# QitaoZhao/ContextAware-PoseFormer

Hardware: AMD Instinct MI355X
Metric: frames/sec (higher is better)
Workload: dtype f32; 1 GPU; configs[1]: batch 64/GPU hrnet_32 256x256 image + 17 kpts -> 17x3, PoseFormer lifter embed 128 levels 4, fp32 tensors, fp32 accumulation; 3x3 stride-1 convs from batch 5: each operand as two fp16 pieces under exact power-of-two block scales (to 2^-23), three piece products on the 16-bit matrix pipe -- same measured distance to fp64 as the direct fp32 MFMA kernel; Inf / NaN / |x| >= 1.5e23 give NaN; frames_per_gpu=64, parallelism=dp1 (independent frames, no collective), plan_flags=0

## Files before the change

contextaware-poseformer_amd/capf/lib.py:

```python
import ctypes
import os
from ctypes import POINTER, byref, c_char_p, c_double, c_float, c_int, c_int32, c_int64, c_size_t, c_void_p

LIB_PATH = os.environ.get("CAPF_LIB") or os.path.join(os.path.dirname(os.path.abspath(__file__)), "libcapf.so")
HRNET, CPN50 = 0, 1
F32, BF16 = 0, 1
PLAN_NO_FUSED_LIFTER, PLAN_NO_WINOGRAD, PLAN_NO_ROW_HALO, PLAN_WINOGRAD_F23_ONLY, PLAN_NO_PWCHAIN, PLAN_NO_WS, PLAN_LIFTER_FP32, PLAN_NO_F32X3, PLAN_F32X3_EXACT, PLAN_NO_F32H2_GEMM, PLAN_NO_UPADD, PLAN_H2_PLANES, PLAN_NO_BNECK, PLAN_NO_BATCHED_REDUCE = 1, 2, 4, 8, 16, 32, 64, 128, 256, 512, 1024, 2048, 4096, 8192
PLAN_BF16_F32_STREAM = 32768
ABI_VERSION = 9

EXPORTS = [
    "capf_create", "capf_destroy", "capf_last_error", "capf_version", "capf_num_params", "capf_param_info",
    "capf_set_param", "capf_params_changed", "capf_lifter_params_changed", "capf_workspace_bytes", "capf_set_workspace", "capf_forward",
    "capf_backbone_forward", "capf_lifter_forward", "capf_set_debug", "capf_set_lanes", "capf_op_conv_group", "capf_affine_from_center_scale", "capf_warp_affine", "capf_op_schedule", "capf_forward_profile_launches", "capf_forward_profile_variants", "capf_tensor", "capf_forward_stats",
    "capf_num_ops", "capf_op_info", "capf_forward_profile", "capf_op_pack_conv", "capf_op_conv", "capf_op_linear",
    "capf_preprocess", "capf_fliptest_fuse", "capf_op_pack_conv_bf16", "capf_op_conv_bf16", "capf_op_conv_bf16_rh_width", "capf_op_pack_conv_bf16_rh", "capf_op_conv_bf16_rh", "capf_op_conv_bf16_group", "capf_forward_train", "capf_backward", "capf_grad_elems", "capf_grad_info", "capf_train_h2_matrices", "capf_mpjpe", "capf_adamw_step",
    "capf_pose_errors", "capf_segment_sums", "capf_keypoints_loss", "capf_train_generation", "capf_max_batch", "capf_op_bytes", "capf_op_linear_bf16", "capf_op_pack_conv_wino", "capf_op_conv_wino", "capf_op_conv_wino_group",
    "capf_op_bilinear_corners", "capf_mpjpe_nd", "capf_op_executed_flops",
    "capf_forward_prefix", "capf_op_describe", "capf_op_tensor",
    "capf_op_conv_bf16_ws_pack_elems", "capf_op_pack_conv_bf16_ws", "capf_op_conv_bf16_ws_group",
    "capf_op_conv_f32x3_pack_elems", "capf_op_pack_conv_f32x3", "capf_op_conv_f32x3_group",
    "capf_op_conv_f32h2_pack_elems", "capf_op_pack_conv_f32h2", "capf_op_conv_f32h2_group",
    "capf_abi_version", "capf_op_describe_sized",
    "capf_jpeg_info", "capf_jpeg_coefficients", "capf_jpeg_decode",
    "capf_jpeg_batch_info", "capf_jpeg_decode_batch", "capf_jpeg_coefficients_subseq",
    "capf_op_f32h2_gemm_pack_elems", "capf_op_pack_f32h2_gemm", "capf_op_conv_f32h2g", "capf_op_conv_f32h2g_group", "capf_op_linear_f32h2g", "capf_op_linear_ln_f32h2g", "capf_op_wgrad", "capf_op_conv_f32h2_tiles", "capf_op_conv_f32h2_planes", "capf_op_h2_planes",
    "capf_fliptest_fuse_swap", "capf_pck_counts",
]


class CapfError(RuntimeError):
    pass


class CapfConfig(ctypes.Structure):
    _fields_ = [
        ("backbone", c_int32), ("hr_channels", c_int32 * 4), ("hr_modules", c_int32 * 3), ("hr_blocks", c_int32),
        ("base_dim", c_int32), ("embed_dim_ratio", c_int32), ("levels", c_int32), ("num_joints", c_int32),
        ("num_heads", c_int32), ("deform_heads", c_int32), ("deform_samples", c_int32), ("context_blocks", c_int32),
        ("compute_dtype", c_int32), ("max_batch", c_int32), ("height", c_int32), ("width", c_int32),
        ("training", c_int32), ("plan_flags", c_int32), ("depth", c_int32),
    ]


class OpDesc(ctypes.Structure):
    _fields_ = [(k, c_int32) for k in ("kind", "backbone", "conv", "Cin", "H", "W", "Cout", "Ho", "Wo", "ks", "stride", "pad", "act",
                                       "in_dtype", "out_dtype", "mfma_bf16", "n_in")] + [("shift", c_int32 * 4)] + \
               [(k, c_int32) for k in ("relu", "p_weight", "p_bn_weight", "has_residual", "checkpoint", "rows_per_frame", "p_bias",
                                       "p_ln_weight", "p_ln_bias")] + [("eps", c_float), ("attn", c_int32 * 4), ("maps", (c_int64 * 4) * 3),
                                                                         ("up_H", c_int32), ("up_W", c_int32)]


class ConvDesc(ctypes.Structure):
    _fields_ = [("x", ctypes.c_void_p), ("w_packed", ctypes.c_void_p), ("bias", ctypes.c_void_p),
                ("residual", ctypes.c_void_p), ("y", ctypes.c_void_p)] + \
               [(k, ctypes.c_int32) for k in ("B", "H", "W", "Cin", "Cout", "ks", "stride", "act")]


_lib = None


def load_library():
    global _lib
    if _lib is not None:
        return _lib
    import torch
    if not os.path.exists(LIB_PATH):
        raise CapfError(f"{LIB_PATH} is missing: build it with `python __graft_entry__.py` "
                        "(or make -C contextaware-poseformer_amd/csrc); there is no fallback path")
    lib = ctypes.CDLL(LIB_PATH)
    abi = lib.capf_abi_version() if hasattr(lib, "capf_abi_version") else None
    if abi != ABI_VERSION:
        raise CapfError(f"{LIB_PATH} implements ABI revision {abi}, this binding expects {ABI_VERSION}: rebuild the library")
    H = c_void_p
    lib.capf_create.argtypes = [POINTER(CapfConfig), c_int, POINTER(H)]
    lib.capf_create.restype = c_int
    lib.capf_destroy.argtypes = [H]
    lib.capf_destroy.restype = None
    lib.capf_last_error.argtypes = [H]
    lib.capf_last_error.restype = c_char_p
    lib.capf_version.restype = c_char_p
    lib.capf_num_params.argtypes = [H]
    lib.capf_param_info.argtypes = [H, c_int, POINTER(c_char_p), POINTER(c_int64), POINTER(c_int), POINTER(c_int)]
    lib.capf_set_param.argtypes = [H, c_char_p, c_void_p, POINTER(c_int64), c_int]
    lib.capf_params_changed.argtypes = [H, c_void_p]
    lib.capf_lifter_params_changed.argtypes = [H, c_void_p]
    lib.capf_workspace_bytes.argtypes = [H, c_int]
    lib.capf_workspace_bytes.restype = c_size_t
    lib.capf_set_workspace.argtypes = [H, c_void_p, c_size_t]
    lib.capf_forward.argtypes = [H, c_void_p, c_void_p, c_void_p, c_void_p, c_int, c_void_p]
    lib.capf_backbone_forward.argtypes = [H, c_void_p, c_void_p, c_int]
    lib.capf_lifter_forward.argtypes = [H, c_void_p, c_void_p, c_void_p, c_int, c_void_p]
    lib.capf_set_debug.argtypes = [H, c_int]
    lib.capf_set_lanes.argtypes = [H, c_int]
    lib.capf_tensor.argtypes = [H, c_char_p, POINTER(c_void_p), POINTER(c_int64), POINTER(c_int)]
    lib.capf_forward_stats.argtypes = [H, c_int, POINTER(c_int64), POINTER(c_double)]
    lib.capf_forward_profile_variants.argtypes = [H, POINTER(c_int32), c_int]
    lib.capf_num_ops.argtypes = [H]
    lib.capf_op_info.argtypes = [H, c_int, c_int, POINTER(c_char_p), POINTER(c_char_p), POINTER(c_double)]
    lib.capf_op_bytes.argtypes = [H, c_int, c_int, POINTER(c_double)]
    lib.capf_op_executed_flops.argtypes = [H, c_int, c_int, POINTER(c_double)]
    lib.capf_forward_prefix.argtypes = [H, c_void_p, c_void_p, c_void_p, c_void_p, c_int, c_void_p, c_int]
    lib.capf_op_describe.argtypes = [H, c_int, POINTER(OpDesc)]
    lib.capf_op_describe_sized.argtypes = [H, c_int, c_void_p, c_size_t]
    lib.capf_op_tensor.argtypes = [H, c_int, c_int, POINTER(c_void_p)]
    lib.capf_forward_profile.argtypes = [H, c_void_p, c_void_p, c_void_p, c_void_p, c_int, c_void_p,
                                         POINTER(c_float), c_int]
    lib.capf_forward_profile_launches.argtypes = [H, c_void_p, c_void_p, c_void_p, c_void_p, c_int, c_void_p,
                                                  POINTER(c_float), POINTER(c_int32), c_int]
    P = c_void_p
    lib.capf_forward_train.argtypes = [H, P, P, P, P, c_int, P, P]
    lib.capf_backward.argtypes = [H, P, P, c_int, P, P]
    lib.capf_train_generation.argtypes = [H]
    lib.capf_train_generation.restype = c_int64
    lib.capf_max_batch.argtypes = [H]
    lib.capf_grad_elems.argtypes = [H]
    lib.capf_grad_elems.restype = c_int64
    lib.capf_grad_info.argtypes = [H, c_int, POINTER(c_int64)]
    lib.capf_train_h2_matrices.argtypes = [H]
    lib.capf_train_h2_matrices.restype = c_int
    lib.capf_mpjpe.argtypes = [P, P, P, c_int, P, P, c_float]
    lib.capf_mpjpe_nd.argtypes = [P, P, P, c_int, c_int, P, P, c_float]
    lib.capf_adamw_step.argtypes = [P, P, P, P, P, c_int64] + [c_float] * 5 + [c_int, c_float]
    lib.capf_op_bilinear_corners.argtypes = [P, P, c_int, c_int, c_int, c_int, P, P]
    lib.capf_op_pack_conv.argtypes = [P, P, P, P, P, P, c_float, P, P, c_int, c_int, c_int]
    lib.capf_op_conv.argtypes = [P, P, P, P, P, P] + [c_int] * 8
    lib.capf_op_linear.argtypes = [P, P, P, P, P, P] + [c_int] * 4
    lib.capf_preprocess.argtypes = [P, P, c_int, c_int, c_int, POINTER(c_float), POINTER(c_float), c_int, P, P, P, P, P, P, P]
    lib.capf_fliptest_fuse.argtypes = [P, P, c_int, P]
    lib.capf_op_pack_conv_bf16.argtypes = [P, P, P, P, P, P, c_float, P, P, c_int, c_int, c_int]
    lib.capf_op_conv_bf16.argtypes = [P, P, P, P, P, P] + [c_int] * 8
    lib.capf_op_conv_bf16_rh_width.argtypes = [c_int]
    lib.capf_op_pack_conv_bf16_rh.argtypes = [P, P, P, P, P, P, c_float, P, P, c_int, c_int]
    lib.capf_op_conv_bf16_rh.argtypes = [P, P, P, P, P, P] + [c_int] * 6
    lib.capf_op_conv_bf16_ws_pack_elems.argtypes = [c_int, c_int]
    lib.capf_op_conv_bf16_ws_pack_elems.restype = c_int64
    lib.capf_op_pack_conv_bf16_ws.argtypes = [P, P, P, P, P, P, c_float, P, P, c_int, c_int]
    lib.capf_op_conv_f32x3_pack_elems.argtypes = [c_int, c_int]
    lib.capf_op_conv_f32x3_pack_elems.restype = c_int64
    lib.capf_op_pack_conv_f32x3.argtypes = [P, P, P, P, P, P, c_float, P, P, c_int, c_int]
    lib.capf_op_conv_f32h2_pack_elems.argtypes = [c_int, c_int]
    lib.capf_op_conv_f32h2_pack_elems.restype = c_int64
    lib.capf_op_pack_conv_f32h2.argtypes = [P, P, P, P, P, P, c_float, P, P, c_int, c_int]
    lib.capf_op_f32h2_gemm_pack_elems.argtypes = [c_int, c_int]
    lib.capf_op_f32h2_gemm_pack_elems.restype = c_int64
    lib.capf_op_pack_f32h2_gemm.argtypes = [P, P, P, P, P, P, c_float, P, P, c_int, c_int, c_int, c_int]
    lib.capf_op_conv_f32h2g.argtypes = [P, P, P, P, P, P] + [c_int] * 8
    lib.capf_op_linear_f32h2g.argtypes = [P, P, P, P, P, P] + [c_int] * 4
    lib.capf_op_linear_ln_f32h2g.argtypes = [P, P, P, P, c_float, P, P, P, P] + [c_int] * 4
    lib.capf_op_wgrad.argtypes = [P, P, P, c_int, c_int, c_int, P, c_int]
    lib.capf_op_pack_conv_wino.argtypes = [P, P, P, P, P, P, c_float, P, P, c_int, c_int, c_int]
    lib.capf_op_conv_wino.argtypes = [P, P, P, P, P, P] + [c_int] * 7
    lib.capf_op_linear_bf16.argtypes = [P, P, P, P, P, P] + [c_int] * 4
    D = POINTER(ConvDesc)
    for name in ("capf_op_conv_group", "capf_op_conv_bf16_ws_group", "capf_op_conv_f32x3_group", "capf_op_conv_f32h2_group",
                 "capf_op_conv_f32h2g_group"):
        getattr(lib, name).argtypes = [P, c_int, D]
    lib.capf_op_conv_wino_group.argtypes = [P, c_int, D, c_int]
    lib.capf_op_conv_bf16_group.argtypes = [P, c_int, D, POINTER(c_void_p), POINTER(c_int32)]
    lib.capf_op_conv_f32h2_planes.argtypes = [P, D, P, P]
    lib.capf_op_conv_f32h2_tiles.argtypes = [c_int, c_int, c_int, POINTER(c_int)]
    lib.capf_pose_errors.argtypes = [P, P, P, c_int, c_int, P, P]
    lib.capf_segment_sums.argtypes = [P, P, P, P, c_int, c_int, P, P]
    lib.capf_keypoints_loss.argtypes = [P, c_int, P, P, P, c_int, c_int, c_float, P, P]
    lib.capf_fliptest_fuse_swap.argtypes = [P, P, c_int, c_int, POINTER(c_int32), P]
    lib.capf_pck_counts.argtypes = [P, P, P, c_int, c_int, c_int, c_double, P, c_int, P, P, P]
    _lib = lib
    return lib


PARAM_KINDS = {0: "conv_w", 1: "bn_w", 2: "bn_b", 3: "bn_mean", 4: "bn_var", 5: "bn_nbt", 6: "lin_w", 7: "lin_b",
               8: "ln_w", 9: "ln_b", 10: "raw"}


class Engine:

    def __init__(self, cfg: CapfConfig, device=None):
        self.lib = load_library()
        self.cfg = cfg
        self.h = c_void_p()
        rc = self.lib.capf_create(byref(cfg), -1 if device is None else int(device), byref(self.h))
        if rc != 0:
            raise CapfError(f"capf_create failed ({rc}): {self.lib.capf_last_error(None).decode()}")
        self.device = device
        self._ws = None
        self._ws_batch = 0
        self._bound = {}

    def close(self):
        if getattr(self, "h", None):
            self.lib.capf_destroy(self.h)
            self.h = None

    __del__ = close

    def _check(self, rc, what):
        if rc < 0:
            raise CapfError(f"{what} failed ({rc}): {self.lib.capf_last_error(self.h).decode()}")
        return rc

    def schema(self):
        out = []
        name, shape, nd, kind = c_char_p(), (c_int64 * 4)(), c_int(), c_int()
        for i in range(self.lib.capf_num_params(self.h)):
            self._check(self.lib.capf_param_info(self.h, i, byref(name), shape, byref(nd), byref(kind)), "param_info")
            out.append((name.value.decode(), tuple(shape[j] for j in range(nd.value)), PARAM_KINDS[kind.value]))
        return out

    def bind_state(self, named_tensors, stream=0):
        import torch
        for name, shape, kind in self.schema():
            if kind == "bn_nbt":
                continue
            t = named_tensors[name]
            if t.dtype != torch.float32 or not t.is_cuda or not t.is_contiguous():
                raise CapfError(f"{name}: need a contiguous fp32 CUDA tensor, got {t.dtype} {t.device}")
            if self._bound.get(name) == t.data_ptr():
                continue
            shp = (c_int64 * 4)(*(list(t.shape) + [0] * (4 - t.dim())))
            self._check(self.lib.capf_set_param(self.h, name.encode(), c_void_p(t.data_ptr()), shp, t.dim()),
                        f"set_param({name})")
            self._bound[name] = t.data_ptr()
        self.params_changed(stream)

    def params_changed(self, stream=0):
        self._check(self.lib.capf_params_changed(self.h, c_void_p(stream)), "params_changed")

    def lifter_params_changed(self, stream=0):
        self._check(self.lib.capf_lifter_params_changed(self.h, c_void_p(stream)), "lifter_params_changed")

    def workspace_bytes(self, batch):
        return self.lib.capf_workspace_bytes(self.h, batch)

    def ensure_workspace(self, batch):
        import torch
        if self._ws is None or batch > self._ws_batch:
            nbytes = self.workspace_bytes(batch)
            self._ws = torch.empty(nbytes // 4 + 64, dtype=torch.float32, device=f"cuda:{self.device}")
            self._ws_batch = batch
            self._check(self.lib.capf_set_workspace(self.h, c_void_p(self._ws.data_ptr()), nbytes), "set_workspace")

    def forward(self, images, k2d, kcrop, out, stream):
        B = images.shape[0]
        self.ensure_workspace(B)
# ... 43 lines not shown
        self.ensure_workspace(B)
        self._check(self.lib.capf_backbone_forward(self.h, c_void_p(stream), c_void_p(images.data_ptr()), B),
                    "backbone_forward")

    def lifter_forward(self, k2d, kcrop, out, stream):
        B = k2d.shape[0]
        self.ensure_workspace(B)
        self._check(self.lib.capf_lifter_forward(self.h, c_void_p(stream), c_void_p(k2d.data_ptr()),
                                                 c_void_p(kcrop.data_ptr()), B, c_void_p(out.data_ptr())),
                    "lifter_forward")

    def set_lanes(self, on):
        self._check(self.lib.capf_set_lanes(self.h, int(on)), "set_lanes")

    def set_debug(self, on):
        self._check(self.lib.capf_set_debug(self.h, int(on)), "set_debug")

    def tensor(self, name):
        import torch
        ptr, shape, nd = c_void_p(), (c_int64 * 4)(), c_int()
        rc = self._check(self.lib.capf_tensor(self.h, name.encode(), byref(ptr), shape, byref(nd)), f"tensor({name})")
        shp = [shape[i] for i in range(nd.value)]
        n = 1
        for s in shp:
            n *= s
        off = (ptr.value - self._ws.data_ptr()) // 4
        if rc == 2:
            return self._ws[off:off + (n + 1) // 2].view(torch.bfloat16)[:n].view(*shp).clone()
        flat = self._ws[off:off + n]
        if rc == 1:
            flat = flat.view(torch.int32)
        return flat.view(*shp).clone()

    def op_table(self, batch):
        name, kern, fl = c_char_p(), c_char_p(), c_double()
        out = []
        for i in range(self.lib.capf_num_ops(self.h)):
            self._check(self.lib.capf_op_info(self.h, i, batch, byref(name), byref(kern), byref(fl)), "op_info")
            out.append((name.value.decode(), kern.value.decode(), fl.value))
        return out

    def op_bytes(self, batch):
        b, out = c_double(), []
        for i in range(self.lib.capf_num_ops(self.h)):
            self._check(self.lib.capf_op_bytes(self.h, i, batch, byref(b)), "op_bytes")
            out.append(b.value)
        return out

    def op_executed_flops(self, batch):
        f, out = c_double(), []
        for i in range(self.lib.capf_num_ops(self.h)):
            self._check(self.lib.capf_op_executed_flops(self.h, i, batch, byref(f)), "op_executed_flops")
            out.append(f.value)
        return out

    def forward_prefix(self, images, n_ops, stream, k2d=None, kcrop=None, out=None):
        B = images.shape[0]
        self.ensure_workspace(B)
        self._prefix_images = images
        P = lambda t: c_void_p(t.data_ptr()) if t is not None else c_void_p(0)
        self._check(self.lib.capf_forward_prefix(self.h, c_void_p(stream), P(images), P(k2d), P(kcrop), B, P(out), int(n_ops)),
                    "forward_prefix")

    def op_describe(self, index):
        d = OpDesc()
        self._check(self.lib.capf_op_describe_sized(self.h, index, byref(d), ctypes.sizeof(d)), "op_describe")
        return d

    def op_tensor(self, index, slot, shape, dtype_code):
        import torch
        ptr = c_void_p()
        self._check(self.lib.capf_op_tensor(self.h, index, slot, byref(ptr)), f"op_tensor({index}, {slot})")
        n = 1
        for v in shape:
            n *= v
        img = getattr(self, "_prefix_images", None)
        if img is not None and ptr.value == img.data_ptr():
            return img.view(*shape)
        off = (ptr.value - self._ws.data_ptr()) // 4
        if dtype_code == 2:
            return self._ws[off:off + (n + 1) // 2].view(torch.bfloat16)[:n].view(*shape)
        return self._ws[off:off + n].view(*shape)

    def op_h2_planes(self, index, batch):
        import torch
        ptr, tp = c_void_p(), c_int(0)
        self.lib.capf_op_h2_planes.argtypes = [c_void_p, c_int, c_int, POINTER(c_void_p), POINTER(c_int)]
        role = self.lib.capf_op_h2_planes(self.h, index, batch, byref(ptr), byref(tp))
        if role <= 0:
            return 0, None, 0
        d = self.op_describe(index)
        C = d.Cout if role == 1 else d.Cin
        tiles = self.lib.capf_op_conv_f32h2_tiles(batch, d.H, d.W, None)
        off = (ptr.value - self._ws.data_ptr()) // 4
        return role, self._ws[off:off + tiles * (C // 16)].view(torch.int32).view(tiles, C // 16), tp.value

    def op_tensor_fp32(self, index, slot, shape, dtype_code):
        t = self.op_tensor(index, slot, shape, dtype_code)
        role, exps, tp = self.op_h2_planes(index, shape[0])
        if (role == 1 and slot == 5) or (role == 2 and slot == 0):
            return planes_to_fp32(t, exps, tp)
        return t

    def forward_profile(self, images, k2d, kcrop, out, stream):
        B = images.shape[0]
        self.ensure_workspace(B)
        n = self.lib.capf_num_ops(self.h)
        ms = (c_float * n)()
        self._check(self.lib.capf_forward_profile(self.h, c_void_p(stream), c_void_p(images.data_ptr()),
                                                  c_void_p(k2d.data_ptr()), c_void_p(kcrop.data_ptr()), B,
                                                  c_void_p(out.data_ptr()), ms, n), "forward_profile")
        return list(ms)

    def op_schedule(self):
        self.lib.capf_op_schedule.argtypes = [c_void_p, c_int, POINTER(c_int32), POINTER(c_int32), POINTER(c_int32),
                                              POINTER(c_int32), POINTER(c_int32)]
        out = []
        for i in range(self.lib.capf_num_ops(self.h)):
            rg, lv, ln = c_int32(), c_int32(), c_int32()
            rd, wr = (c_int32 * 5)(), (c_int32 * 6)()
            self._check(self.lib.capf_op_schedule(self.h, i, byref(rg), byref(lv), byref(ln), rd, wr), "op_schedule")
            out.append((rg.value, lv.value, ln.value, [v for v in rd if v != -1], [v for v in wr if v != -1]))
        return out

    def forward_profile_launches(self, images, k2d, kcrop, out, stream):
        B = images.shape[0]
        self.ensure_workspace(B)
        n = self.lib.capf_num_ops(self.h)
        ms = (c_float * n)()
        leader = (c_int32 * n)()
        self._check(self.lib.capf_forward_profile_launches(self.h, c_void_p(stream), c_void_p(images.data_ptr()),
                                                           c_void_p(k2d.data_ptr()), c_void_p(kcrop.data_ptr()), B,
                                                           c_void_p(out.data_ptr()), ms, leader, n), "forward_profile_launches")
        return list(ms), list(leader)

    def profile_variants(self):
        n = self.lib.capf_num_ops(self.h)
        v = (c_int32 * n)()
        self._check(self.lib.capf_forward_profile_variants(self.h, v, n), "forward_profile_variants")
        return list(v)

    def stats(self, batch):
        n, f = c_int64(), c_double()
        self._check(self.lib.capf_forward_stats(self.h, batch, byref(n), byref(f)), "forward_stats")
        return n.value, f.value


def _p(t):
    return c_void_p(t.data_ptr()) if t is not None else c_void_p(0)


def _stream(t):
    import torch
    return c_void_p(torch.cuda.current_stream(t.device).cuda_stream)


def _call(entry, *args):
    rc = getattr(load_library(), entry)(*args)
    if rc:
        raise CapfError(f"{entry} failed ({rc})")


def _out_hw(H, W, ks, stride):
    pad = ks // 2
    return (H + 2 * pad - ks) // stride + 1, (W + 2 * pad - ks) // stride + 1

# ... 57 lines not shown
    descs, outs = _conv_descs([(x, wp, bias, res, wp.shape[0], 3, 1, act) for x, wp, bias, act, res in problems])
    x0, wp0 = problems[0][:2]
    _call("capf_op_conv_wino_group", _stream(x0), len(problems), descs, _wino_variant(wp0, x0.shape[3]))
    return outs


def conv_nhwc_group(problems):
    descs, outs = _conv_descs([(x, wp, bias, res, wp.shape[0], ks, stride, act) for x, wp, bias, ks, stride, act, res in problems])
    _call("capf_op_conv_group", _stream(problems[0][0]), len(problems), descs)
    return outs


def pack_conv_bf16(w, bn=None, eps=1e-5):
    import torch
    co, ci, ks, _ = w.shape
    return _pack("capf_op_pack_conv_bf16", w, bn, eps, (co, (ks * ks * ci + 63) // 64 * 64), torch.bfloat16, co, ci, ks)


def conv_nhwc_bf16(x, wp, bias, ks, stride=1, act=0, residual=None):
    d = ConvDesc()
    y = _conv_out(d, x, wp, bias, residual, wp.shape[0], ks, stride, act, bf16=True)
    _call("capf_op_conv_bf16", _stream(x), d.x, d.w_packed, d.bias, d.residual, d.y, d.B, d.H, d.W, d.Cin, d.Cout, ks, stride, act)
    return y


def pack_conv_bf16_rh(w, bn=None, eps=1e-5):
    import torch
    co, ci, ks, _ = w.shape
    cw = load_library().capf_op_conv_bf16_rh_width(ci)
    if ks != 3 or not cw:
        raise CapfError(f"row-halo conv needs a 3x3 kernel and Cin % 32 == 0 (got ks={ks}, Cin={ci})")
    return _pack("capf_op_pack_conv_bf16_rh", w, bn, eps, (co, 9 * ci), torch.bfloat16, co, ci) + (cw,)


def conv_nhwc_bf16_rh(x, wp, bias, act=0, residual=None):
    d = ConvDesc()
    y = _conv_out(d, x, wp, bias, residual, wp.shape[0], act=act, bf16=True)
    _call("capf_op_conv_bf16_rh", _stream(x), d.x, d.w_packed, d.bias, d.residual, d.y, d.B, d.H, d.W, d.Cin, d.Cout, act)
    return y


def pack_conv_bf16_ws(w, bn=None, eps=1e-5):
    import torch
    co, ci, ks, _ = w.shape
    n = load_library().capf_op_conv_bf16_ws_pack_elems(co, ci)
    if ks != 3 or n <= 0 or co % 8:
        raise CapfError(f"2-D halo conv needs a 3x3 kernel, Cin % 16 == 0 and Cout % 8 == 0 (got ks={ks}, Cin={ci}, Cout={co})")
    return _pack("capf_op_pack_conv_bf16_ws", w, bn, eps, n, torch.bfloat16, co, ci)


def conv_nhwc_bf16_ws_group(problems):
    descs, outs = _conv_descs([(x, wp, bias, res, co, 3, 1, act) for x, wp, bias, act, res, co in problems], bf16=True)
    _call("capf_op_conv_bf16_ws_group", _stream(problems[0][0]), len(problems), descs)
    return outs


def pack_conv_f32x3(w, bn=None, eps=1e-5):
    import torch
    co, ci, ks, _ = w.shape
    n = load_library().capf_op_conv_f32x3_pack_elems(co, ci)
    if ks != 3 or n <= 0 or co % 4:
        raise CapfError(f"split-fp32 conv needs a 3x3 kernel, Cin % 16 == 0 and Cout % 4 == 0 (got ks={ks}, Cin={ci}, Cout={co})")
    return _pack("capf_op_pack_conv_f32x3", w, bn, eps, n, torch.bfloat16, co, ci)


def conv_nhwc_f32x3_group(problems):
    descs, outs = _conv_descs([(x, wp, bias, res, co, 3, 1, act) for x, wp, bias, act, res, co in problems])
    _call("capf_op_conv_f32x3_group", _stream(problems[0][0]), len(problems), descs)
    return outs


def pack_conv_f32h2(w, bn=None, eps=1e-5):
    import torch
    co, ci, ks, _ = w.shape
    n = load_library().capf_op_conv_f32h2_pack_elems(co, ci)
    if ks != 3 or n <= 0 or co % 4:
        raise CapfError(f"split-fp32 conv needs a 3x3 kernel, Cin % 16 == 0 and Cout % 4 == 0 (got ks={ks}, Cin={ci}, Cout={co})")
    return _pack("capf_op_pack_conv_f32h2", w, bn, eps, n, torch.int16, co, ci)


def conv_nhwc_f32h2_group(problems):
    descs, outs = _conv_descs([(x, wp, bias, res, co, 3, 1, act) for x, wp, bias, act, res, co in problems])
    _call("capf_op_conv_f32h2_group", _stream(problems[0][0]), len(problems), descs)
    return outs


def conv_nhwc_f32h2_planes(x, wp, bias, act, residual, cout, exps_in=None, planes_out=False):
    import torch
    d = ConvDesc()
    y = _conv_out(d, x, wp, bias, residual, cout, act=act)
    tiles = load_library().capf_op_conv_f32h2_tiles(d.B, d.H, d.W, None)
    eo = torch.zeros(tiles, cout // 16, device=x.device, dtype=torch.int32) if planes_out else None
    _call("capf_op_conv_f32h2_planes", _stream(x), byref(d), _p(exps_in), _p(eo))
    return (y, eo) if planes_out else y


def f32h2_tile_pixels(B, H, W):
    px = c_int(0)
    if load_library().capf_op_conv_f32h2_tiles(B, H, W, byref(px)) <= 0:
        raise CapfError("geometry not eligible for the two-fp16-piece tile")
    return px.value


def planes_to_fp32(planes, exps, tile_pixels):
    import torch
    B, H, W, C = planes.shape
    h = planes.contiguous().view(torch.float16).view(B * H * W, C // 16, 2, 16).float()
    tile = torch.arange(B * H * W, device=planes.device) // tile_pixels
    scale = torch.exp2((127 - exps[tile].to(torch.float64))).to(torch.float32)
    v = (h[:, :, 0, :] + h[:, :, 1, :]) * scale[:, :, None]
    return v.reshape(B, H, W, C)


def pack_f32h2_gemm(w, bn=None, eps=1e-5):
    import torch
    if w.dim() == 4:
        n, ci, ks, _ = w.shape
        k = ks * ks * ci
    else:
        (n, k), ci, ks = w.shape, 0, 0
    elems = load_library().capf_op_f32h2_gemm_pack_elems(n, k)
    return _pack("capf_op_pack_f32h2_gemm", w, bn, eps, elems, torch.float32, n, ci, ks, k, bias="zeros" if w.dim() == 4 else None)


def conv_nhwc_f32h2g(x, wp, bias, ks, stride=1, act=0, residual=None, cout=None):
    d = ConvDesc()
    y = _conv_out(d, x, wp, bias, residual, cout if cout is not None else bias.numel(), ks, stride, act)
    _call("capf_op_conv_f32h2g", _stream(x), d.x, d.w_packed, d.bias, d.residual, d.y, d.B, d.H, d.W, d.Cin, d.Cout, ks, stride, act)
    return y


def conv_nhwc_f32h2g_group(problems):
    descs, outs = _conv_descs([(x, wp, bias, res, co, ks, stride, act) for x, wp, bias, ks, stride, act, res, co in problems])
    _call("capf_op_conv_f32h2g_group", _stream(problems[0][0]), len(problems), descs)
    return outs


def _rows_out(x, n, dtype=None):
    import torch
    return torch.empty(x.shape[0], n, device=x.device, dtype=dtype or torch.float32)


def linear_ln_f32h2g(x, gamma, beta, eps, wp, bias, n, act=0, residual=None):
    (M, K), y = x.shape, _rows_out(x, n)
    _call("capf_op_linear_ln_f32h2g", _stream(x), _p(x), _p(gamma), _p(beta), float(eps), _p(wp), _p(bias), _p(residual), _p(y), M, n, K, act)
    return y


def linear_f32h2g(x, wp, bias, n, act=0, residual=None):
    (M, K), y = x.shape, _rows_out(x, n)
    _call("capf_op_linear_f32h2g", _stream(x), _p(x), _p(wp), _p(bias), _p(residual), _p(y), M, n, K, act)
    return y


def wgrad(dy, x, two_piece=True):
    import torch
    (M, N), K = dy.shape, x.shape[1]
    out = torch.empty(N * K + N, device=x.device, dtype=torch.float32)
    _call("capf_op_wgrad", _stream(x), _p(dy), _p(x), M, N, K, _p(out), 1 if two_piece else 0)
    return out[:N * K].view(N, K), out[N * K:]


def conv_nhwc_bf16_group(problems):
    descs, outs = _conv_descs([(x, wp, bias, res, wp.shape[0], ks, stride, act) for x, wp, bias, ks, stride, act, res, _ in problems], bf16=True)
    rh = (c_void_p * len(problems))(*(p[7].data_ptr() if p[7] is not None else None for p in problems))
    variant = c_int32(-1)
# ... 290 lines not shown
```

contextaware-poseformer_amd/csrc/engine.cpp:

```cpp
#include <stdio.h>
#include <string.h>

#include <algorithm>
#include <vector>

#include "engine.h"

namespace capf {

#define HIP_TRY(expr)                                                                      \
    do {                                                                                   \
        hipError_t _e = (expr);                                                            \
        if (_e != hipSuccess) {                                                            \
            err = std::string(#expr) + ": " + hipGetErrorString(_e);                       \
            return CAPF_ERR_HIP;                                                           \
        }                                                                                  \
    } while (0)

Engine::ConvSrc Engine::conv_src(const Pack& pk) const {
    return {params[pk.w[0]].ptr, params[pk.bn.g].ptr, params[pk.bn.b].ptr, params[pk.bn.m].ptr, params[pk.bn.v].ptr, 1e-5f};
}

int Engine::repack(hipStream_t s, bool lifter_only) {
    for (const Param& p : params) {
// ... 20 lines not shown
        float* B = pack_arena + pk.b_off;
        if (pk.kind == CONV_BN) {
            if (lifter_only) continue;
            const ConvSrc c = conv_src(pk);
            if (pk.bf16) {
                HIP_TRY(launch_pack_conv_bf16(c.w, c.g, c.b, c.m, c.v, c.eps, W, B, pk.N, pk.Cin, pk.ks, pk.Kpad, s));
                if (pk.rh) HIP_TRY(launch_pack_conv_bf16_rh(c.w, c.g, c.b, c.m, c.v, c.eps, pack_arena + pk.rh_off, B, pk.N, pk.Cin, bf16_rh_width(pk.Cin), s));
                if (pk.ws) HIP_TRY(launch_pack_conv_bf16_ws(c.w, c.g, c.b, c.m, c.v, c.eps, pack_arena + pk.ws_off, B, pk.N, pk.Cin, s));
            } else if (pk.wino) {
                if (!pk.wino_skip) HIP_TRY(launch_pack_conv_wino(c.w, c.g, c.b, c.m, c.v, c.eps, W, B, pk.N, pk.Cin, s, pk.Kpad == 18 * pk.Cin ? 43 : 23));
                HIP_TRY(launch_pack_conv(c.w, c.g, c.b, c.m, c.v, c.eps, pack_arena + pk.direct_off, B, pk.N, pk.Cin, pk.ks, pk.direct_Kpad, s));
                if (pk.x3)
                    HIP_TRY((plan.x3_h2 ? launch_pack_conv_f32h2 : launch_pack_conv_f32x3)(c.w, c.g, c.b, c.m, c.v, c.eps, pack_arena + pk.x3_off, B, pk.N, pk.Cin, s));
            } else {
                HIP_TRY(launch_pack_conv(c.w, c.g, c.b, c.m, c.v, c.eps, W, B, pk.N, pk.Cin, pk.ks, pk.Kpad, s));
            }
            continue;
        }
        int n0 = 0;
        for (int i = 0; i < pk.n_lin; ++i) {
            const int n = (int)params[pk.w[i]].shape[0];
            const float* w = params[pk.w[i]].ptr;
            if (pk.bf16)
                HIP_TRY(launch_pack_conv_bf16(w, nullptr, nullptr, nullptr, nullptr, 0.f, reinterpret_cast<unsigned short*>(W) + (size_t)n0 * pk.Kpad,
                                              nullptr, n, pk.K, 1, pk.Kpad, s));
            else if (pk.quad) HIP_TRY(launch_pack_linear_quad(w, W, n, pk.K, n0, pk.N, s));
            else HIP_TRY(launch_pack_linear(w, W + (size_t)n0 * pk.Kpad, n, pk.K, pk.Kpad, s));
            jobs.push_back(CopySegment{params[pk.b[i]].ptr, B + n0, n, 0});
            n0 += n;
        }
    }
    if (!jobs.empty()) {
        CopySegment* tab_dev = reinterpret_cast<CopySegment*>(pack_arena + bias_tab_off);
        const bool same = bias_tab_on_device && bias_tab.size() == jobs.size() &&
                          memcmp(bias_tab.data(), jobs.data(), jobs.size() * sizeof(CopySegment)) == 0;
        if (!same) {
            HIP_TRY(hipStreamSynchronize(s));
            bias_tab = jobs;
            HIP_TRY(hipMemcpyAsync(tab_dev, bias_tab.data(), bias_tab.size() * sizeof(CopySegment), hipMemcpyHostToDevice, s));
            bias_tab_on_device = true;
        }
        HIP_TRY(launch_copy_segments(tab_dev, (int)jobs.size(), s));
    }
    packed = true;
    return CAPF_OK;
}

int Engine::ensure_h2g_lifter(hipStream_t s) {
    if (!h2g_lifter_dirty) return CAPF_OK;
    for (const Pack& pk : packs) {
        if (!pk.h2g || pk.kind != LINEAR) continue;
        int n0 = 0;
        for (int i = 0; i < pk.n_lin; ++i) {
            const int n = (int)params[pk.w[i]].shape[0];
            HIP_TRY(launch_pack_f32h2_gemm_rows(params[pk.w[i]].ptr, pack_arena + pk.h2g_off, n0, n, pk.N, pk.K, pk.h2g_Kpad, s));
            n0 += n;
        }
        if (pk.chain) HIP_TRY(launch_res_chain_repack(pack_arena + pk.h2g_off, pack_arena + pk.chain_off, pk.N, pk.h2g_Kpad, s));
    }
    h2g_lifter_dirty = false;
    return CAPF_OK;
}

GemmArgs Engine::gemm_args(const Op& op, int batch, bool planes) const {
    auto ptr = [&](int buf) -> float* { return (buf >= 0 && ws) ? bptr(buf, batch) : nullptr; };
    const Pack& pk = packs[op.pack];
    GemmArgs a{};
    a.A = op.in[0] == -2 ? images : ptr(op.in[0]);
    if (pk.in_place) {
        a.Wp = params[pk.w[0]].ptr;
        a.bias = params[pk.b[0]].ptr;
    } else {
        a.Wp = pack_arena + pk.w_off;
        a.bias = pack_arena + pk.b_off;
    }
    a.res = op.res_param >= 0 ? params[op.res_param].ptr : ptr(op.aux);
    a.out = ptr(op.out);
    a.M = (int)(op.rows_per_frame * batch);
    a.N = op.N; a.K = op.K; a.Kpad = pk.Kpad;
    if (pk.rh) a.Wp2 = pack_arena + pk.rh_off;
    if (pk.ws || pk.x3) a.Wp3 = pack_arena + (pk.ws ? pk.ws_off : pk.x3_off);
    a.x3_h2 = pk.x3 && plan.x3_h2;
    if (a.x3_h2 && op.h2_utab >= 0 && utab_on_device) a.h2_utab = reinterpret_cast<const unsigned*>(pack_arena + utab_off) + op.h2_utab;
    if (pk.h2g && batch >= H2G_MIN_BATCH && !op.bf16 && !op.pw_pair && !(op.wino && wino_now(op, batch))) a.Wh2 = pack_arena + pk.h2g_off;
    if (op.wino && !wino_now(op, batch)) {
        a.Wp = pack_arena + pk.direct_off;
        a.Kpad = pk.direct_Kpad;
    } else if (op.wino && pk.wino_skip) {
        a.Wp = nullptr;
    }
    a.conv = op.conv;
    a.Cin = op.Cin; a.H = op.H; a.W = op.W; a.Ho = op.Ho; a.Wo = op.Wo;
    a.ks = op.ks; a.stride = op.stride; a.pad = op.pad;
    a.amap = op.amap; a.omap = op.omap; a.rmap = op.rmap;
    a.act = op.act;
    a.out_bf16 = op.out_bf16;
    a.f32s = op.f32s;
    a.out_f32 = op.st_f32;
    a.out_sh = op.sh >= 0 ? ptr(op.sh) : nullptr;
    if (planes && op.h2_role && a.x3_h2 && a.Wp3 && wino_now(op, batch)) {
        const GemmArgs peer = gemm_args(ops[op.h2_peer], batch, false);
        GemmArgs me = a;
        me.conv = op.conv; me.Cin = op.Cin; me.H = op.H; me.W = op.W; me.Ho = op.Ho; me.Wo = op.Wo; me.ks = op.ks; me.stride = op.stride; me.pad = op.pad;
        me.omap = op.omap; me.rmap = op.rmap; me.act = op.act;
        if (peer.x3_h2 && peer.Wp3 && wino_now(ops[op.h2_peer], batch) && gemm_f32x3_wanted(me) && gemm_f32x3_wanted(peer)) {
            int* e = reinterpret_cast<int*>(ptr(op.h2_exps));
            if (op.h2_role == 1) a.h2_eout = e; else a.h2_ein = e;
        }
    }
    if (op.conv && op.up_in >= 0) {
        a.up = ptr(op.up_in);
        a.up_H = op.up_H; a.up_W = op.up_W;
        a.up_sh = op.Ho > 1 ? (float)(op.up_H - 1) / (float)(op.Ho - 1) : 0.f;
        a.up_sw = op.Wo > 1 ? (float)(op.up_W - 1) / (float)(op.Wo - 1) : 0.f;
    }
    static const bool splitk_on = [] { const char* e = diag_env("CAPF_SPLITK"); return !e || atoi(e) != 0; }();
    if ((op.conv || (op.kind == OP_GEMM && op.ln.w < 0 && op.res_param < 0)) && !op.bf16 && split_ws && lanes != 1 && splitk_on) {
        a.split_ws = on_side_chain ? split_ws_side : split_ws;
        a.split_cnt = on_side_chain ? split_cnt_side : split_cnt;
        a.split_ws_elems = SPLIT_WS_ELEMS; a.split_cnt_elems = SPLIT_CNT_ELEMS;
    }
    if (op.ln.w >= 0) {
        a.ln_g = params[op.ln.w].ptr;
        a.ln_b = params[op.ln.b].ptr;
        a.ln_eps = op.eps;
    }
    return a;
}

Engine::FusedLaunch Engine::fused_at(int i, int batch, int last_op, bool bneck_only) const {
    const int n_all = (int)ops.size();
    if (i < 0 || i >= n_all) return {};
    const Op& o = ops[i];
    if (o.kind == OP_FORK) {
        if (!plan.use_bneck || !bf16() || o.fork.lanes != 2 || o.region < 0) return {};
        const int j = regions[o.region].second;
        if (j != i + 4 || j + 1 >= last_op || j + 1 >= n_all) return {};
        int c1 = -1, c2 = -1, ds = -1;
        for (int k = i + 1; k < j; ++k) {
            const Op& g = ops[k];
            if (g.kind != OP_GEMM || !g.conv || g.bf16 != 1) return {};
            if (g.lane == 1) ds = k; else if (c1 < 0) c1 = k; else c2 = k;
        }
        const int c3 = j + 1;
        if (c1 < 0 || c2 < 0 || ds < 0 || ops[c3].kind != OP_GEMM || !ops[c3].conv || ops[c3].bf16 != 1) return {};
        if (ops[c2].in[0] != ops[c1].out || ops[ds].in[0] != ops[c1].in[0] || ops[c3].in[0] != ops[c2].out || ops[c3].aux != ops[ds].out) return {};
        if (ops[c1].rows_per_frame * batch < 65536) return {};
        if (!bneck0_bf16_ok(gemm_args(ops[c1], batch), gemm_args(ops[c2], batch), gemm_args(ops[ds], batch), gemm_args(ops[c3], batch))) return {};
        return {Fusion::BNECK0, 4, {c1, c2, ds, c3}};
    }
    if (o.kind != OP_GEMM) return {};
    if (plan.use_bneck && bf16() && i + 2 < last_op && i + 2 < n_all) {
        const Op &c2 = ops[i + 1], &c3 = ops[i + 2];
        bool ok = o.bneck_c3 == i + 2 && c2.in[0] == o.out && c3.in[0] == c2.out && c3.aux == o.in[0] && o.aux < 0 && c2.aux < 0 &&
                  o.rows_per_frame * batch >= 65536;
        for (const Op* g : {&o, &c2, &c3})
            ok = ok && g->kind == OP_GEMM && g->conv && g->bf16 == 1 && g->region == o.region && g->lane == o.lane && g->up_in < 0;
        if (ok && bneck1_bf16_ok(gemm_args(o, batch), gemm_args(c2, batch), gemm_args(c3, batch))) return {Fusion::BNECK1, 3, {i, i + 1, i + 2}};
    }
    if (bneck_only || !plan.use_pwchain || i + 1 >= last_op || i + 1 >= n_all) return {};
    const Op& b = ops[i + 1];
    if (!o.conv || b.kind != OP_GEMM || !b.conv || o.bf16 != b.bf16 || o.bf16 > 1 || b.in[0] != o.out || b.region != o.region || b.lane != o.lane) return {};
    if (o.bf16 && (fused_leader(i, batch, true).n || fused_at(i + 1, batch, last_op, true).n)) return {};
    const GemmArgs ga = gemm_args(o, batch), gb = gemm_args(b, batch);
    if (!(o.bf16 ? gemm_bf16_pwchain_ok(ga, gb) : gemm_f32_pwchain_ok(ga, gb))) return {};
    return {Fusion::PWCHAIN, 2, {i, i + 1}};
// ... 168 lines not shown
        case OP_HEAD:
            HIP_TRY(launch_head(ptr(op.in[0]), params[op.ln.w].ptr, params[op.ln.b].ptr, op.eps, params[op.head.w].ptr,
                                params[op.head.b].ptr, out, (int)(op.rows_per_frame * batch), op.C, op.head.N, s));
            break;
        default: break;
    }
    return CAPF_OK;
}

int Engine::run_region_grouped(hipStream_t s, int batch, int region, LaunchLog* log, unsigned lane_mask) {
    auto mine = [&](const Op& op) { return ((lane_mask >> op.lane) & 1u) != 0; };
    auto groupable = [&](const Op& op, const GemmArgs& a) {
        if (op.kind != OP_GEMM) return false;
        switch (gemm_family(op, batch)) {
            case Family::BF16: return gemm_bf16_groupable(a);
            case Family::WINO: return gemm_wino_ok(a);
            case Family::F32: return gemm_f32_groupable(a);
            default: return false;
        }
    };
    for (const std::vector<int>& level : region_levels[region]) {
        for (Family pass : {Family::F32, Family::BF16, Family::WINO}) {
            GemmArgs group[MAXG];
            int members[MAXG];
            int n = 0;
            auto flush = [&]() -> int {
                if (n == 0) return CAPF_OK;
                if (log) HIP_TRY(log->mark(s, members, n));
                if (pass == Family::F32) HIP_TRY(launch_gemm_f32_group(group, n, s));
                else if (pass == Family::BF16) {
                    int v = -1;
                    HIP_TRY(launch_gemm_bf16_group(group, n, s, &v));
                    if (log && !log->op_variant.empty()) log->op_variant[members[0]] = v;
                }
                else HIP_TRY(launch_gemm_wino_group(group, n, s));
                n = 0;
                return CAPF_OK;
            };
            for (int oi : level) {
                const Op& op = ops[oi];
                if (op.kind != OP_GEMM || !mine(op) || gemm_family(op, batch) != pass) continue;
                const GemmArgs a = gemm_args(op, batch);
                if (!groupable(op, a)) continue;
                group[n] = a;
                members[n++] = oi;
                if (n == MAXG) { int rc = flush(); if (rc) return rc; }
            }
            int rc = flush();
            if (rc) return rc;
        }
        {
            FuseSumArgs fg[4];
            int fm[4], nf = 0;
            for (int oi : level) {
                const Op& op = ops[oi];
                if (op.kind != OP_FUSE || skipped(op) || !mine(op)) continue;
                if (nf > 0 && (op.bf16 != ops[fm[0]].bf16 || (op.C % 8 == 0) != (ops[fm[0]].C % 8 == 0))) continue;
                if (nf == 4) break;
                fg[nf] = fuse_args(op, batch);
                fm[nf++] = oi;
            }
            if (nf < 2) nf = 0;
            if (nf) {
                if (log) HIP_TRY(log->mark(s, fm, nf));
                HIP_TRY(launch_fuse_sum_group(fg, nf, s));
            }
            for (int oi : level) {
                const Op& op = ops[oi];
                if (!mine(op)) continue;
                if (op.kind == OP_GEMM && groupable(op, gemm_args(op, batch))) continue;
                if (skipped(op)) continue;
                bool done = false;
                for (int k = 0; k < nf; ++k) done |= fm[k] == oi;
                if (done) continue;
                if (log) HIP_TRY(log->mark(s, &oi, 1));
                int rc = exec_op(op, s, batch);
                if (rc) return rc;
            }
        }
    }
    return CAPF_OK;
}

int Engine::run(hipStream_t s, int batch, int first_op, int last_op, hipEvent_t* ev, LaunchLog* log) {
    hipStream_t main_stream = s;
    if (plan.use_h2g && (batch >= H2G_MIN_BATCH || has_res_chain) && last_op > n_backbone_ops && !bf16()) {
        const int rc = ensure_h2g_lifter(s);
        if (rc) return rc;
    }
    const bool grouped = (lanes == 2 || lanes == 3) && !ev;
    const bool par = lanes == 1 && !ev && !log && side[0];
    for (int oi = first_op; oi < last_op; ++oi) {
        const Op& op = ops[oi];
        s = (par && op.lane > 0) ? side[op.lane - 1] : main_stream;
        if (ev) HIP_TRY(hipEventRecord(ev[oi], s));
        if (const FusedLaunch f = ev ? FusedLaunch{} : fused_at(oi, batch, last_op); f.n) {
            const bool tap = debug || last_op < (int)ops.size();
            GemmArgs m[4];
            for (int k = 0; k < f.n; ++k) m[k] = gemm_args(ops[f.m[k]], batch);
            if (log) HIP_TRY(log->mark(s, f.m, f.n));
            if (f.kind == Fusion::BNECK0) HIP_TRY(launch_bneck0_bf16(m[0], m[1], m[2], m[3], tap, s));
            else if (f.kind == Fusion::BNECK1) HIP_TRY(launch_bneck1_bf16(m[0], m[1], m[2], tap, s));
            else if (op.bf16) HIP_TRY(launch_gemm_bf16_pwchain(m[0], m[1], s));
            else HIP_TRY(launch_gemm_f32_pwchain(m[0], m[1], s));
            oi = f.m[f.n - 1];
            continue;
        }
        switch (op.kind) {
            case OP_FORK: {
                if (grouped && regions[op.region].second <= last_op) {
                    const bool two = lanes == 3 && !log && side[0] && op.fork.lanes >= 2 && batch >= 16 && batch <= 256;
                    if (two) {
                        HIP_TRY(hipEventRecord(events[op.fork.first_event], main_stream));
                        HIP_TRY(hipStreamWaitEvent(side[0], events[op.fork.first_event], 0));
                        on_side_chain = true;
                        int rc = run_region_grouped(side[0], batch, op.region, nullptr, 0x6u);
                        on_side_chain = false;
                        if (rc) return rc;
                        rc = run_region_grouped(main_stream, batch, op.region, nullptr, ~0x6u);
                        if (rc) return rc;
                        HIP_TRY(hipEventRecord(events[op.fork.first_event + 1], side[0]));
                        HIP_TRY(hipStreamWaitEvent(main_stream, events[op.fork.first_event + 1], 0));
                        oi = regions[op.region].second;
                        break;
                    }
                    int rc = run_region_grouped(main_stream, batch, op.region, log);
                    if (rc) return rc;
                    oi = regions[op.region].second;
                } else if (par) {
                    HIP_TRY(hipEventRecord(events[op.fork.first_event], main_stream));
                    for (int l = 1; l < op.fork.lanes; ++l) HIP_TRY(hipStreamWaitEvent(side[l - 1], events[op.fork.first_event], 0));
                }
                break;
            }
            case OP_JOIN:
                if (par) {
                    for (int l = 1; l < op.fork.lanes; ++l) {
                        HIP_TRY(hipEventRecord(events[op.fork.first_event + l], side[l - 1]));
                        HIP_TRY(hipStreamWaitEvent(main_stream, events[op.fork.first_event + l], 0));
                    }
                }
                break;
            default: {
                if (skipped(op)) break;
                if (log) HIP_TRY(log->mark(s, &oi, 1));
                int rc = exec_op(op, s, batch);
                if (rc) return rc;
            }
        }
    }
    if (ev) HIP_TRY(hipEventRecord(ev[last_op], main_stream));
    if (log) HIP_TRY(log->mark(main_stream, nullptr, 0));
    return CAPF_OK;
}

}

using capf::Engine;

static std::string g_create_error;

extern "C" {

const char* capf_version(void) { return "capf 0.9 (gfx950)"; }
int capf_abi_version(void) { return CAPF_ABI_VERSION; }

const char* capf_last_error(const capf_handle* h) { return h ? h->e.err.c_str() : g_create_error.c_str(); }

int capf_create(const capf_config* cfg, int device, capf_handle** out) {
    if (!cfg || !out) {
        g_create_error = "null argument";
        return CAPF_ERR_INVALID;
    }
    capf_handle* h = new capf_handle();
    Engine& e = h->e;
    e.cfg = *cfg;
    e.device = device;
    e.lanes = 2;
    if (cfg->compute_dtype != CAPF_F32 && cfg->compute_dtype != CAPF_BF16) {
        g_create_error = "compute_dtype must be CAPF_F32 or CAPF_BF16";
        delete h;
        return CAPF_ERR_UNSUPPORTED;
    }
    if (cfg->plan_flags & ~(16383 | CAPF_PLAN_BF16_F32_STREAM)) {
        g_create_error = "unknown capf_plan_flag bits";
        delete h;
        return CAPF_ERR_INVALID;
    }
    if (cfg->max_batch <= 0) {
        g_create_error = "max_batch must be positive";
        delete h;
        return CAPF_ERR_INVALID;
    }
    if (!e.build()) {
        g_create_error = e.err;
        delete h;
        return CAPF_ERR_UNSUPPORTED;
    }
    if (device >= 0) {
        hipError_t r = hipSetDevice(device);
        if (r == hipSuccess && e.pack_elems) r = hipMalloc(reinterpret_cast<void**>(&e.pack_arena), e.pack_elems * sizeof(float));
        if (r == hipSuccess) r = hipMalloc(reinterpret_cast<void**>(&e.split_ws), Engine::SPLIT_WS_ELEMS * sizeof(float));
        if (r == hipSuccess) r = hipMalloc(reinterpret_cast<void**>(&e.split_cnt), Engine::SPLIT_CNT_ELEMS * sizeof(int));
        if (r == hipSuccess) r = hipMemset(e.split_cnt, 0, Engine::SPLIT_CNT_ELEMS * sizeof(int));
        if (r == hipSuccess) r = hipMalloc(reinterpret_cast<void**>(&e.split_ws_side), Engine::SPLIT_WS_ELEMS * sizeof(float));
        if (r == hipSuccess) r = hipMalloc(reinterpret_cast<void**>(&e.split_cnt_side), Engine::SPLIT_CNT_ELEMS * sizeof(int));
        if (r == hipSuccess) r = hipMemset(e.split_cnt_side, 0, Engine::SPLIT_CNT_ELEMS * sizeof(int));
        for (int i = 0; i < 3 && r == hipSuccess; ++i) r = hipStreamCreateWithFlags(&e.side[i], hipStreamNonBlocking);
        e.events.resize(e.n_events);
        for (auto& x : e.events)
            if (r == hipSuccess) r = hipEventCreateWithFlags(&x, hipEventDisableTiming);
        if (r != hipSuccess) {
            g_create_error = std::string("hip: ") + hipGetErrorString(r);
            delete h;
            return CAPF_ERR_HIP;
        }
    }
    *out = h;
    return CAPF_OK;
}

void capf_destroy(capf_handle* h) {
    if (!h) return;
    if (h->e.pack_arena) (void)hipFree(h->e.pack_arena);
    if (h->e.split_ws) (void)hipFree(h->e.split_ws);
    if (h->e.split_cnt) (void)hipFree(h->e.split_cnt);
    if (h->e.split_ws_side) (void)hipFree(h->e.split_ws_side);
    if (h->e.split_cnt_side) (void)hipFree(h->e.split_cnt_side);
    for (auto& x : h->e.events)
        if (x) (void)hipEventDestroy(x);
    for (auto& st : h->e.side)
        if (st) (void)hipStreamDestroy(st);
    delete h;
}

int capf_max_batch(const capf_handle* h) { return h ? (h->e.batch_limit < h->e.cfg.max_batch ? h->e.batch_limit : h->e.cfg.max_batch) : CAPF_ERR_INVALID; }

int capf_num_params(const capf_handle* h) { return h ? (int)h->e.params.size() : CAPF_ERR_INVALID; }

int capf_param_info(const capf_handle* h, int index, const char** name, int64_t shape[4], int* ndim, int* kind) {
    if (!h || index < 0 || index >= (int)h->e.params.size()) return CAPF_ERR_INVALID;
    const capf::Param& p = h->e.params[index];
    if (name) *name = p.name.c_str();
    if (shape) memcpy(shape, p.shape, sizeof(p.shape));
    if (ndim) *ndim = p.ndim;
    if (kind) *kind = p.kind;
    return CAPF_OK;
}

int capf_set_param(capf_handle* h, const char* name, const void* dev_ptr, const int64_t* shape, int ndim) {
    if (!h || !name) return CAPF_ERR_INVALID;
    Engine& e = h->e;
    auto it = e.param_index.find(name);
    if (it == e.param_index.end()) {
        e.err = std::string("unknown parameter: ") + name;
        return CAPF_ERR_INVALID;
    }
    capf::Param& p = e.params[it->second];
    bool ok = (ndim == p.ndim);
    for (int i = 0; ok && i < ndim; ++i) ok = (shape[i] == p.shape[i]);
    if (!ok) {
        e.err = std::string("shape mismatch for ") + name;
        return CAPF_ERR_INVALID;
    }
    p.ptr = static_cast<const float*>(dev_ptr);
    e.packed = false;
    return CAPF_OK;
// ... 327 lines not shown
}

int capf_op_linear(void* stream, const float* x, const float* w, const float* bias, const float* residual, float* y,
                   int M, int N, int K, int act) {
    if (K % 32 != 0) return CAPF_ERR_UNSUPPORTED;
    return hip_rc(capf::launch_gemm_f32(rows_args(&capf::GemmArgs::Wp, x, w, bias, residual, y, M, N, K, act), static_cast<hipStream_t>(stream)));
}

int capf_op_bilinear_corners(void* stream, const float* grid, int n, int H, int W, int border, int32_t* idx, float* frac) {
    if (!grid || !idx || !frac || n <= 0 || H <= 0 || W <= 0) return CAPF_ERR_INVALID;
    return capf::launch_bilinear_corners(grid, n, H, W, border, idx, frac, static_cast<hipStream_t>(stream)) == hipSuccess
               ? CAPF_OK : CAPF_ERR_HIP;
}

int capf_op_pack_conv_bf16(void* stream, const float* w, const float* gamma, const float* beta, const float* mean,
                           const float* var, float eps, void* wp, float* bias, int Cout, int Cin, int ks) {
    const int Kpad = (ks * ks * Cin + 63) / 64 * 64;
    return hip_rc(capf::launch_pack_conv_bf16(w, gamma, beta, mean, var, eps, wp, bias, Cout, Cin, ks, Kpad, static_cast<hipStream_t>(stream)));
}

int capf_op_conv_bf16(void* stream, const void* x, const void* wp, const float* bias, const void* residual, void* y, int B,
                      int H, int W, int Cin, int Cout, int ks, int stride, int act) {
    const capf::GemmArgs a = conv_args(conv_desc(x, wp, bias, residual, y, B, H, W, Cin, Cout, ks, stride, act), &capf::GemmArgs::Wp, 64);
    return hip_rc(capf::launch_gemm_bf16(a, static_cast<hipStream_t>(stream)), CAPF_ERR_UNSUPPORTED);
}

int capf_op_conv_bf16_rh_width(int Cin) {
    return capf::gemm_bf16_rh_cw(conv_args(conv_desc(nullptr, nullptr, nullptr, nullptr, nullptr, 1, 8, 8, Cin, 8, 3, 1, 0), &capf::GemmArgs::Wp, 1));
}

int capf_op_pack_conv_bf16_rh(void* stream, const float* w, const float* gamma, const float* beta, const float* mean,
                              const float* var, float eps, void* wp, float* bias, int Cout, int Cin) {
    const int cw = capf_op_conv_bf16_rh_width(Cin);
    if (!cw) return CAPF_ERR_UNSUPPORTED;
    return hip_rc(capf::launch_pack_conv_bf16_rh(w, gamma, beta, mean, var, eps, wp, bias, Cout, Cin, cw, static_cast<hipStream_t>(stream)));
}

int capf_op_conv_bf16_rh(void* stream, const void* x, const void* wp, const float* bias, const void* residual, void* y, int B,
                         int H, int W, int Cin, int Cout, int act) {
    const capf::GemmArgs a = conv_args(conv_desc(x, wp, bias, residual, y, B, H, W, Cin, Cout, 3, 1, act), &capf::GemmArgs::Wp, 1);
    return hip_rc(capf::launch_gemm_bf16_rh(a, static_cast<hipStream_t>(stream)), CAPF_ERR_UNSUPPORTED);
}

int64_t capf_op_conv_bf16_ws_pack_elems(int Cout, int Cin) { return Cin % 16 == 0 && Cout > 0 ? capf::bf16_ws_pack_elems(Cout, Cin) : 0; }

int capf_op_pack_conv_bf16_ws(void* stream, const float* w, const float* gamma, const float* beta, const float* mean,
                              const float* var, float eps, void* wp, float* bias, int Cout, int Cin) {
    if (!w || !wp || Cin % 16 != 0 || Cout % 8 != 0) return CAPF_ERR_UNSUPPORTED;
    return hip_rc(capf::launch_pack_conv_bf16_ws(w, gamma, beta, mean, var, eps, wp, bias, Cout, Cin, static_cast<hipStream_t>(stream)));
}

int capf_op_conv_bf16_ws_group(void* stream, int n, const capf_conv_desc* d) {
    return conv_group(stream, n, d, [](const capf_conv_desc& c, int, capf::GemmArgs& a) { return wp3_build(c, a, capf::gemm_bf16_ws_ok, 0); },
                      capf::launch_gemm_bf16_ws_group);
}

int64_t capf_op_conv_f32x3_pack_elems(int Cout, int Cin) { return Cin % 16 == 0 && Cout > 0 ? capf::f32x3_pack_elems(Cout, Cin) : 0; }

int capf_op_pack_conv_f32x3(void* stream, const float* w, const float* gamma, const float* beta, const float* mean, const float* var,
                            float eps, void* wp, float* bias, int Cout, int Cin) {
    if (!w || !wp || Cin % 16 != 0 || Cout % 4 != 0) return CAPF_ERR_UNSUPPORTED;
    return hip_rc(capf::launch_pack_conv_f32x3(w, gamma, beta, mean, var, eps, wp, bias, Cout, Cin, static_cast<hipStream_t>(stream)));
}

int capf_op_conv_f32x3_group(void* stream, int n, const capf_conv_desc* d) {
    return conv_group(stream, n, d, [](const capf_conv_desc& c, int, capf::GemmArgs& a) { return wp3_build(c, a, capf::gemm_f32x3_ok, 0); },
                      capf::launch_gemm_f32x3_group);
}

int64_t capf_op_conv_f32h2_pack_elems(int Cout, int Cin) { return Cin % 16 == 0 && Cout > 0 ? capf::f32h2_pack_elems(Cout, Cin) : 0; }

int capf_op_pack_conv_f32h2(void* stream, const float* w, const float* gamma, const float* beta, const float* mean, const float* var,
                            float eps, void* wp, float* bias, int Cout, int Cin) {
    if (!w || !wp || Cin % 16 != 0 || Cout % 4 != 0) return CAPF_ERR_UNSUPPORTED;
    return hip_rc(capf::launch_pack_conv_f32h2(w, gamma, beta, mean, var, eps, wp, bias, Cout, Cin, static_cast<hipStream_t>(stream)));
}

int capf_op_conv_f32h2_group(void* stream, int n, const capf_conv_desc* d) {
    return conv_group(stream, n, d, [](const capf_conv_desc& c, int, capf::GemmArgs& a) { return wp3_build(c, a, capf::gemm_f32x3_ok, 1); },
                      capf::launch_gemm_f32h2_group);
}

int capf_op_conv_f32h2_tiles(int B, int H, int W, int* tile_pixels) { return capf::f32h2_tiles_m(B, H, W, tile_pixels); }

int capf_op_conv_f32h2_planes(void* stream, const capf_conv_desc* d, const int32_t* exps_in, int32_t* exps_out) {
    if (!d || !is_3x3_s1(*d) || (exps_in && exps_out)) return CAPF_ERR_UNSUPPORTED;
    capf::GemmArgs g = conv_args(*d, &capf::GemmArgs::Wp3, 1);
    g.x3_h2 = 1; g.h2_ein = exps_in; g.h2_eout = exps_out;
    if (!capf::gemm_f32x3_ok(g)) return CAPF_ERR_UNSUPPORTED;
    const hipError_t e = capf::launch_gemm_f32h2_group(&g, 1, static_cast<hipStream_t>(stream));
    return hip_rc(e, e == hipErrorInvalidValue ? CAPF_ERR_UNSUPPORTED : CAPF_ERR_HIP);
}

int capf_op_conv_bf16_group(void* stream, int n, const capf_conv_desc* d, const void* const* w_rh, int32_t* variant) {
    return conv_group(stream, n, d, [w_rh](const capf_conv_desc& c, int i, capf::GemmArgs& a) {
        a = conv_args(c, &capf::GemmArgs::Wp, 64);
        a.Wp2 = w_rh ? static_cast<const float*>(w_rh[i]) : nullptr;
        return capf::gemm_bf16_groupable(a) ? CAPF_OK : CAPF_ERR_UNSUPPORTED;
    }, [variant](const capf::GemmArgs* g, int n, hipStream_t s) {
        int v = -1;
        const hipError_t e = capf::launch_gemm_bf16_group(g, n, s, &v);
        if (variant) *variant = v;
        return e;
    });
}

int capf_op_linear_bf16(void* stream, const void* x_bf16, const void* w_bf16, const float* bias, const float* residual, void* y,
                        int M, int N, int K, int gelu_bf16_out) {
    if (!x_bf16 || !w_bf16 || !y || K % 64 != 0) return CAPF_ERR_INVALID;
    return capf::launch_gemm_bf16_rows(x_bf16, w_bf16, bias, M, N, K, K, static_cast<float*>(y), capf::row_ld(N), residual,
                                       capf::row_ld(N), gelu_bf16_out, static_cast<hipStream_t>(stream)) == hipSuccess
               ? CAPF_OK : CAPF_ERR_UNSUPPORTED;
}

int capf_preprocess(void* stream, const uint8_t* images_bgr, int batch, int height, int width, const float mean[3],
                    const float* std3, int mode, float* images_out, const float* gt_in, float* gt_out, const float* k2d_in,
                    float* k2d_out, const float* kcrop_in, float* kcrop_out) {
    if (!images_bgr || !images_out || !k2d_in || !k2d_out || !kcrop_in || !kcrop_out || !mean || batch <= 0 || mode < 0 ||
        mode > 2 || (gt_in && !gt_out))
        return CAPF_ERR_INVALID;
    return capf::launch_preprocess(images_bgr, batch, height, width, mean, std3, mode, images_out, gt_in, gt_out, k2d_in,
                                   k2d_out, kcrop_in, kcrop_out, static_cast<hipStream_t>(stream)) == hipSuccess
               ? CAPF_OK : CAPF_ERR_HIP;
}

int capf_fliptest_fuse(void* stream, const float* pred2, int batch, float* out) {
    if (!pred2 || !out || batch <= 0) return CAPF_ERR_INVALID;
    return capf::launch_fliptest_fuse(pred2, batch, out, static_cast<hipStream_t>(stream)) == hipSuccess ? CAPF_OK : CAPF_ERR_HIP;
}

int capf_fliptest_fuse_swap(void* stream, const float* pred2, int batch, int joints, const int32_t* swap, float* out) {
    if (!pred2 || !out || !swap || batch <= 0 || joints <= 0 || joints > capf::FLIP_MAX_JOINTS) return CAPF_ERR_INVALID;
    for (int j = 0; j < joints; ++j)
        if (swap[j] < 0 || swap[j] >= joints || swap[swap[j]] != j) return CAPF_ERR_INVALID;
    return capf::launch_fliptest_fuse_swap(pred2, batch, joints, swap, out, static_cast<hipStream_t>(stream)) == hipSuccess ? CAPF_OK
                                                                                                                       : CAPF_ERR_HIP;
}

int capf_affine_from_center_scale(const double center[2], const double scale[2], int out_w, int out_h, double m[6]) {
    if (!center || !scale || !m || out_w <= 1 || out_h <= 1) return CAPF_ERR_INVALID;
    return capf::affine_from_center_scale(center, scale, out_w, out_h, m) ? CAPF_OK : CAPF_ERR_INVALID;
}

int capf_warp_affine(void* stream, const uint8_t* const* frames, const int32_t* dims, const double* m, int batch, int out_h,
                     int out_w, uint8_t* out) {
    if (!frames || !dims || !m || !out || batch <= 0 || out_h <= 0 || out_w <= 0) return CAPF_ERR_INVALID;
    return capf::launch_warp_affine_u8(frames, dims, m, out, batch, out_h, out_w, static_cast<hipStream_t>(stream)) == hipSuccess
               ? CAPF_OK : CAPF_ERR_HIP;
}

int capf_pose_errors(void* stream, const float* pred, const float* gt, int n, int joints, const int32_t* prev, float* err) {
    if (!pred || !gt || !err || n <= 0 || joints <= 0) return CAPF_ERR_INVALID;
    hipError_t r = capf::launch_pose_errors(pred, gt, n, joints, prev, err, static_cast<hipStream_t>(stream));
    return r == hipSuccess ? CAPF_OK : (r == hipErrorInvalidValue ? CAPF_ERR_UNSUPPORTED : CAPF_ERR_HIP);
}

int capf_segment_sums(void* stream, const float* err, const int32_t* segment, const int32_t* prev, int n, int n_segments,
                      double* sums, int32_t* counts) {
    if (!err || !sums || !counts || n <= 0 || n_segments <= 0 || (n_segments > 1 && !segment)) return CAPF_ERR_INVALID;
    return capf::launch_segment_sums(err, segment, prev, n, n_segments, sums, counts, static_cast<hipStream_t>(stream)) == hipSuccess
               ? CAPF_OK : CAPF_ERR_HIP;
}

int capf_pck_counts(void* stream, const float* pred, const float* gt, int n, int joints, int root, double to_mm, const int32_t* segment,
                    int n_segments, int32_t* counts, double* mpjpe_sums, int32_t* frames) {
    if (!counts || !mpjpe_sums || !frames || n < 0 || (n > 0 && (!pred || !gt)) || joints <= 0 || joints > 32 || root < 0 ||
// ... 171 lines not shown
    }
    const int act_dt = e.bf16() ? 2 : 0;
    d->in_dtype = d->out_dtype = (d->backbone ? act_dt : 0);
    d->H = op.H; d->W = op.W; d->Ho = op.Ho; d->Wo = op.Wo;
    if (op.kind == capf::OP_GEMM) {
        const capf::Pack& pk = e.packs[op.pack];
        d->conv = op.conv; d->Cin = op.conv ? op.Cin : op.K; d->Cout = op.N;
        d->ks = op.ks; d->stride = op.stride; d->pad = op.pad; d->act = op.act;
        d->has_residual = op.aux >= 0 || op.res_param >= 0;
        if (op.conv && op.up_in >= 0) { d->up_H = op.up_H; d->up_W = op.up_W; }
        d->mfma_bf16 = (op.bf16 || op.out_bf16) ? 1 : 0;
        if (op.conv) {
            d->in_dtype = op.in[0] == -2 ? 0 : (op.bf16 ? 2 : 0);
            d->out_dtype = op.st_f32 ? 0 : (op.bf16 || op.out_bf16) ? 2 : 0;
            d->p_weight = pk.w[0]; d->p_bn_weight = pk.bn.g;
        } else {
            d->in_dtype = op.bf16 == 2 ? 2 : 0;
            d->out_dtype = op.out_bf16 ? 2 : 0;
            d->p_weight = pk.n_lin == 1 ? pk.w[0] : -1;
            d->p_bias = pk.n_lin == 1 ? pk.b[0] : -1;
            d->p_ln_weight = op.ln.w; d->p_ln_bias = op.ln.b;
        }
    } else if (op.kind == capf::OP_LAYERNORM) {
        d->Cin = d->Cout = op.C;
        d->in_dtype = 0; d->out_dtype = op.out_bf16 ? 2 : 0;
        d->has_residual = op.aux >= 0;
        d->p_ln_weight = op.ln.w; d->p_ln_bias = op.ln.b;
        d->maps[1][0] = 1; d->maps[1][1] = op.C; d->maps[1][2] = 0; d->maps[1][3] = 0;
    } else if (op.kind == capf::OP_ATTENTION) {
        const capf::Attn& at = op.attn;
        d->attn[0] = at.groups; d->attn[1] = at.tokens; d->attn[2] = at.heads; d->attn[3] = at.head_dim;
        d->rows_per_frame = at.groups * at.tokens;
        d->Cin = 3 * at.heads * at.head_dim; d->Cout = at.heads * at.head_dim;
        d->in_dtype = 0; d->out_dtype = op.out_bf16 ? 2 : 0;
        d->maps[0][0] = 1; d->maps[0][1] = d->Cin; d->maps[1][0] = 1; d->maps[1][1] = d->Cout;
    } else {
        d->Cin = d->Cout = op.C;
        d->n_in = op.n_in; d->relu = op.relu;
        d->has_residual = op.kind == capf::OP_RESIZE && op.aux >= 0;
        for (int i = 0; i < 4; ++i) d->shift[i] = op.shift[i];
        if (op.kind == capf::OP_FUSE) { d->Ho = op.H; d->Wo = op.W; }
        if (op.kind == capf::OP_FUSE && d->backbone) d->in_dtype = d->out_dtype = op.bf16 ? 2 : 0;
    }
    d->checkpoint = (op.bneck_c3 >= 0 ? op.bneck_c3 : op.region >= 0 ? e.regions[op.region].second : index) + 1;
    return CAPF_OK;
}

int capf_op_describe_sized(const capf_handle* h, int index, void* desc, size_t desc_bytes) {
    if (!desc || desc_bytes == 0) return CAPF_ERR_INVALID;
    capf_op_desc full;
    const int rc = capf_op_describe(h, index, &full);
    if (rc != CAPF_OK) return rc;
    memset(desc, 0, desc_bytes);
    memcpy(desc, &full, desc_bytes < sizeof(full) ? desc_bytes : sizeof(full));
    return CAPF_OK;
}

int capf_op_tensor(const capf_handle* h, int index, int slot, const void** dev_ptr) {
    if (!h || !dev_ptr || index < 0 || index >= (int)h->e.ops.size() || slot < 0 || slot > 6) return CAPF_ERR_INVALID;
    const Engine& e = h->e;
    const capf::Op& op = e.ops[index];
    const auto r = op.reads();
    const int buf = slot == 1 && r[5] >= 0 ? r[5] : slot < 5 ? r[slot] : slot == 5 ? op.out : op.sh;
    if (buf == -2) { *dev_ptr = e.images; return CAPF_OK; }
    if (buf < 0 || !e.ws || e.last_batch <= 0) return CAPF_ERR_INVALID;
    *dev_ptr = e.bptr(buf, e.last_batch);
    return CAPF_OK;
}

int capf_op_h2_planes(const capf_handle* h, int index, int batch, const void** exps, int32_t* tile_pixels) {
    if (!h || index < 0 || index >= (int)h->e.ops.size() || batch <= 0) return CAPF_ERR_INVALID;
    const Engine& e = h->e;
    const capf::Op& op = e.ops[index];
    if (!op.h2_role || !e.ws) return 0;
    const capf::GemmArgs a = e.gemm_args(op, batch);
    if (!a.h2_ein && !a.h2_eout) return 0;
    if (exps) *exps = a.h2_ein ? static_cast<const void*>(a.h2_ein) : static_cast<const void*>(a.h2_eout);
    int tp = 0;
    capf::f32h2_tiles_m(batch, op.H, op.W, &tp);
    if (tile_pixels) *tile_pixels = tp;
    return op.h2_role;
}

int capf_forward_profile(capf_handle* h, void* stream, const float* images_nhwc, const float* k2d, float* kcrop_inout,
                         int batch, float* out, float* op_ms, int n_ops) {
    if (!h || !images_nhwc || !k2d || !kcrop_inout || !out || !op_ms) return CAPF_ERR_INVALID;
    Engine& e = h->e;
    const int n = (int)e.ops.size();
    if (n_ops < n) return CAPF_ERR_INVALID;
    int rc = check_run(e, batch);
    if (rc) return rc;
    e.images = images_nhwc; e.k2d = k2d; e.kcrop = kcrop_inout; e.out = out;
    e.last_batch = batch;
    e.invalidate_train();
    std::vector<hipEvent_t> ev(n + 1);
    for (auto& x : ev)
        if (hipEventCreate(&x) != hipSuccess) return CAPF_ERR_HIP;
    hipStream_t s = static_cast<hipStream_t>(stream);
    rc = e.run(s, batch, 0, n, ev.data());
    if (rc == CAPF_OK && hipStreamSynchronize(s) != hipSuccess) rc = CAPF_ERR_HIP;
    for (int i = 0; i < n && rc == CAPF_OK; ++i)
        if (hipEventElapsedTime(&op_ms[i], ev[i], ev[i + 1]) != hipSuccess) rc = CAPF_ERR_HIP;
    for (auto& x : ev) (void)hipEventDestroy(x);
    return rc;
}

int capf_forward_profile_launches(capf_handle* h, void* stream, const float* images_nhwc, const float* k2d,
                                  float* kcrop_inout, int batch, float* out, float* op_ms, int32_t* op_leader, int n_ops) {
    if (!h || !images_nhwc || !k2d || !kcrop_inout || !out || !op_ms || !op_leader) return CAPF_ERR_INVALID;
    Engine& e = h->e;
    const int n = (int)e.ops.size();
    if (n_ops < n) return CAPF_ERR_INVALID;
    int rc = check_run(e, batch);
    if (rc) return rc;
    e.images = images_nhwc; e.k2d = k2d; e.kcrop = kcrop_inout; e.out = out;
    e.last_batch = batch;
    e.invalidate_train();
    capf::LaunchLog log;
    log.op_leader.assign(n, -1);
    log.op_variant.assign(n, -1);
    hipStream_t s = static_cast<hipStream_t>(stream);
    rc = e.run(s, batch, 0, n, nullptr, &log);
    e.last_variants = log.op_variant;
    if (rc == CAPF_OK && hipStreamSynchronize(s) != hipSuccess) rc = CAPF_ERR_HIP;
    for (int i = 0; i < n; ++i) { op_ms[i] = 0.f; op_leader[i] = log.op_leader[i]; }
    for (size_t k = 0; k < log.leader.size() && rc == CAPF_OK; ++k)
        if (hipEventElapsedTime(&op_ms[log.leader[k]], log.ev[k], log.ev[k + 1]) != hipSuccess) rc = CAPF_ERR_HIP;
    return rc;
}

int capf_forward_profile_variants(const capf_handle* h, int32_t* op_variant, int n_ops) {
    if (!h || !op_variant || n_ops < (int)h->e.last_variants.size()) return CAPF_ERR_INVALID;
    for (size_t i = 0; i < h->e.last_variants.size(); ++i) op_variant[i] = h->e.last_variants[i];
    return CAPF_OK;
}

int capf_forward_stats(const capf_handle* h, int batch, int64_t* launches, double* flops) {
    if (!h) return CAPF_ERR_INVALID;
    int64_t n = 0;
    double f = 0.0;
    for (const capf::Op& op : h->e.ops) {
        if (op.debug_only) continue;
        if (op.kind == capf::OP_FORK || op.kind == capf::OP_JOIN) continue;
        ++n;
        f += op.flops_per_frame * batch;
    }
    if (launches) *launches = n;
    if (flops) *flops = f;
    return CAPF_OK;
}

}
```

contextaware-poseformer_amd/csrc/engine.h:

```cpp
#pragma once
#include <hip/hip_runtime.h>
#include <stdint.h>

#include <array>
#include <map>
#include <string>
#include <vector>

#include "capf.h"
#include "kernels.h"

namespace capf {

struct Param {
    std::string name;
    int64_t shape[4] = {0, 0, 0, 0};
    int ndim = 0;
    int kind = 0;
    const float* ptr = nullptr;
    int64_t numel() const {
        int64_t n = 1;
        for (int i = 0; i < ndim; ++i) n *= shape[i];
        return n;
    }
};

struct Buffer {
    size_t elems = 0;
    size_t offset = 0;
    int def_op = -1;
    int last_op = -1;
    std::string tag;
};

struct Tensor {
    int buf = -1;
    int H = 0, W = 0, C = 0;
};

struct BnRef { int g = -1, b = -1, m = -1, v = -1; };

enum PackKind { CONV_BN = 0, LINEAR = 1 };
struct Pack {
    PackKind kind = CONV_BN;
    int w[4] = {-1, -1, -1, -1}, b[4] = {-1, -1, -1, -1};
    int n_lin = 0;
    BnRef bn;
    int N = 0, K = 0, Cin = 0, ks = 1;
    size_t w_off = 0, b_off = 0;
    int Kpad = 0;
    bool in_place = false;
    bool bf16 = false;
    bool quad = false;
    bool wino = false;
    bool wino_skip = false;
    size_t direct_off = 0; int direct_Kpad = 0;
    bool rh = false; size_t rh_off = 0; int rh_Kpad = 0;
    bool ws = false; size_t ws_off = 0;
    bool x3 = false; size_t x3_off = 0;
    bool h2g = false; size_t h2g_off = 0; int h2g_Kpad = 0;
    bool chain = false; size_t chain_off = 0;
};

struct LinearRef { int w = -1, b = -1, N = 0, K = 0; };
struct LnRef { int w = -1, b = -1; };
struct LifterMlp { LnRef norm2; LinearRef fc1, fc2; };
struct LifterAtt { LnRef norm1; LinearRef qkv, proj; LifterMlp mlp; };
struct LifterCtx {
    LnRef norm1;
    LinearRef aw, so, embed_proj[4];
    LifterMlp mlp;
    int ao_pack = -1;
    int tap_pos = -1, tap_idx = -1;
};
struct LifterSchema {
    int pos = -1;
    LinearRef coord, feat_embed[4];
    LifterAtt res[8], joint[8];
    LifterCtx ctx[4];
    LnRef head_ln;
    LinearRef head;
};

// ... 38 lines not shown
    int lvlH[4] = {0, 0, 0, 0}, lvlW[4] = {0, 0, 0, 0}, lvlC[4] = {0, 0, 0, 0};
    int idx_lvl[4] = {-1, -1, -1, -1};
    int tap_pos = -1, tap_idx = -1;
    int pq[4] = {-1, -1, -1, -1};
    int pb[4] = {-1, -1, -1, -1};
    double flops_per_frame = 0.0;
    int bf16 = 0;
    int wino = 0;
    int pw_pair = 0;
    int x3_lo = 0, x3_hi = -1;
    int out_bf16 = 0;
    int h2_exps = -1, h2_role = 0, h2_peer = -1;
    long h2_utab = -1;
    int f32s = 0, st_f32 = 0, sh = -1;
    int feat_bf16 = 0;
    int bneck_c3 = -1;
    int lane = 0;
    int region = -1;
};

struct NamedTensor {
    int buf;
    int64_t shape[4];
    int ndim;
    int is_int;
};

struct TrainLayout {
    struct Mlp { size_t xh2, rs2, y2, hp, hg; };
    struct Ctx { size_t xh1, rs1, y1, ao, U[4]; Mlp mlp; };
    struct Att { size_t xh1, rs1, y1, qkv, o; Mlp mlp; };
    size_t X, S[4];
    Ctx ctx[4];
    Att res[8], joint[8];
    size_t xhh, rsh, yh;
    size_t dX, gA, gB, gC, cat, dU[4], tA, tB, wT, slabs, red;
    size_t h2w, h2max;
    size_t wpad;
    size_t slabs_elems = 0, red_elems = 0;
    size_t red_cap = 0;
    size_t slab_cap = 0;
    size_t total;
};

struct LaunchLog {
    std::vector<hipEvent_t> ev;
    std::vector<int> leader;
    std::vector<int> op_leader;
    std::vector<int> op_variant;
    hipError_t mark(hipStream_t s, const int* members, int n) {
        hipEvent_t e;
        hipError_t r = hipEventCreate(&e);
        if (r != hipSuccess) return r;
        ev.push_back(e);
        if (n > 0) {
            leader.push_back(members[0]);
            for (int i = 0; i < n; ++i) op_leader[members[i]] = members[0];
        }
        return hipEventRecord(e, s);
    }
    ~LaunchLog() {
        for (hipEvent_t e : ev) (void)hipEventDestroy(e);
    }
};

struct Engine {
    capf_config cfg{};
    int device = -1;
    std::string err;

    struct PlanSwitches {
        bool fused_lifter = true;
        bool use_wino = true;
        bool wino_f43 = true;
        bool wino_f43_cpn = false;
        int wino_f43_min_hw = 0, wino_f43_max_hw = 1 << 30;
        int wino_min_batch = 24;
        bool use_rh = true;
        bool use_ws = true;
        bool use_x3 = true;
        bool x3_h2 = true;
        bool use_h2g = true;
        bool use_h2_planes = false;
        bool use_pwchain = true;
        bool use_bneck = true;
        bool use_upadd = true;
        bool batch_reduce = true;
        bool f32_stream = false;
    } plan;
    bool set_plan_switches();
    static constexpr int H2G_MIN_BATCH = 5;

    std::vector<Param> params;
    std::map<std::string, int> param_index;
    std::vector<Buffer> bufs;
    std::vector<Pack> packs;
    std::vector<Op> ops;
    int n_backbone_ops = 0;
    int cur_lane = 0, cur_region = -1, n_regions = 0, n_events = 0;
    std::vector<std::pair<int, int>> regions;
    std::vector<std::vector<std::vector<int>>> region_levels;
    std::map<std::string, NamedTensor> named;
    size_t ws_elems_per_frame = 0;
    size_t pack_elems = 0;
    size_t bias_tab_off = 0;
    bool has_res_chain = false;
    std::vector<unsigned> utab_host;
    size_t utab_off = 0;
    int batch_limit = 0;
    int feat_buf[4] = {-1, -1, -1, -1}, feat_H[4] = {0, 0, 0, 0}, feat_W[4] = {0, 0, 0, 0}, feat_C[4] = {0, 0, 0, 0};
    LifterSchema lifter;
    std::vector<long> grad_off;
    long grad_elems = 0;

    int add_param(const std::string& name, int kind, std::initializer_list<int64_t> shape);
    int new_buffer(size_t elems, const std::string& tag);
    Tensor conv_bn(const std::string& conv, const std::string& bn, const Tensor& x, int Cout, int ks, int stride,
                   int act, const Tensor* residual);
    void build_hrnet(Tensor img, Tensor feats[4]);
    void build_cpn(Tensor img, Tensor feats[4]);
    void build_lifter(const Tensor feats[4]);
    bool build();
    void assign_offsets();
    void schedule_regions();
    bool bf16() const { return cfg.compute_dtype == CAPF_BF16; }
    bool maps_bf16() const { return bf16() && !plan.f32_stream; }
    int depth() const { return cfg.depth > 0 ? cfg.depth : cfg.levels; }
    bool plan_f32_stream(const Tensor feats[4]);
    size_t act_elems(size_t n) const { return bf16() ? (n + 1) / 2 : n; }
    void use(int buf);
    void push(Op op);
    void fork(int n);
    void set_lane(int l) { cur_lane = l; }
    void join();

    float* pack_arena = nullptr;
    std::vector<CopySegment> bias_tab;
    bool bias_tab_on_device = false;
    bool utab_on_device = false;
    float* split_ws = nullptr;
    int* split_cnt = nullptr;
    float* split_ws_side = nullptr;
    int* split_cnt_side = nullptr;
    bool on_side_chain = false;
    static constexpr long SPLIT_WS_ELEMS = 4L << 20;
    static constexpr int SPLIT_CNT_ELEMS = 16384;
    float* ws = nullptr;
    size_t ws_bytes = 0;
    bool packed = false;
    bool h2g_lifter_dirty = true;
    bool debug = false;
    int lanes = 3;
    hipStream_t side[3] = {nullptr, nullptr, nullptr};
    std::vector<hipEvent_t> events;
    std::vector<int> last_variants;
    int last_batch = 0;
    const float* images = nullptr;
    const float* k2d = nullptr;
    float* kcrop = nullptr;
    float* out = nullptr;

    float* bptr(int buf, int batch) const { return ws + bufs[buf].offset * (size_t)batch; }
    struct ConvSrc { const float *w, *g, *b, *m, *v; float eps; };
    ConvSrc conv_src(const Pack& pk) const;
    int repack(hipStream_t s, bool lifter_only = false);
    int ensure_h2g_lifter(hipStream_t s);
    int run(hipStream_t s, int batch, int first_op, int last_op, hipEvent_t* ev = nullptr, LaunchLog* log = nullptr);
    int exec_op(const Op& op, hipStream_t s, int batch);
    bool skipped(const Op& op) const { return op.debug_only && !debug; }
    FuseSumArgs fuse_args(const Op& op, int batch) const;
    bool wino_now(const Op& op, int batch) const {
        return op.wino && ((batch >= op.x3_lo && batch <= op.x3_hi) || (batch >= plan.wino_min_batch && !packs[op.pack].wino_skip));
    }
    enum class Family { NONE = -1, F32, BF16, WINO, BF16_ROWS };
    struct OpRoute { Family family; const char* kernel; double flops; };
    Family gemm_family(const Op& op, int batch) const;
    OpRoute op_route(const Op& op, int batch) const;
    enum class Fusion { NONE, BNECK0, BNECK1, PWCHAIN };
    struct FusedLaunch { Fusion kind = Fusion::NONE; int n = 0; int m[4] = {-1, -1, -1, -1}; };
    FusedLaunch fused_at(int i, int batch, int last_op, bool bneck_only = false) const;
    FusedLaunch fused_leader(int i, int batch, bool bneck_only = false) const;
    int run_region_grouped(hipStream_t s, int batch, int region, LaunchLog* log, unsigned lane_mask = ~0u);
    GemmArgs gemm_args(const Op& op, int batch, bool planes = true) const;

    int train_batch = 0;
    int64_t train_generation = 0;
    void invalidate_train() { train_batch = 0; ++train_generation; t_h2_base = nullptr; }
    void train_layout(int B, TrainLayout& L) const;
    size_t train_elems(int B) const;
    int forward_train(hipStream_t s, int B, const float* masks);
    int backward(hipStream_t s, int B, const float* dOut, float* flat_grad, const float* masks);
    int t_gemm(hipStream_t s, const float* A, RowMap amap, int M, int N, int K, const float* W, int Kpad, const float* bias,
               float* out, RowMap omap, const float* res, RowMap rmap, int act, const float* rscale, int rs_div, const float* Wh2 = nullptr);
    struct H2TrainSpec { int param, pack; int N, K, ld; bool fwd, bwd; };
    std::vector<H2TrainSpec> t_h2_specs;
    std::vector<H2TrainW> t_h2_tab;
    std::map<const float*, int> t_h2_index;
    size_t t_h2_tab_off = 0;
    size_t t_h2_elems = 0, t_h2_max_elems = 0;
    int t_h2_tiles = 0;
    bool t_h2_on_device = false;
    SlabBatch t_slab_jobs{};
    size_t t_slab_cur = 0;
    float* t_slab_take(hipStream_t s, float* area, size_t cap, size_t elems, int* rc);
    int t_slab_defer(hipStream_t s, const float* slabs, int nslab, long n, float* dst);
    int t_slab_flush(hipStream_t s);
    ColFinalBatch t_col_jobs{};
    size_t t_col_cur = 0;
    int t_colreduce(hipStream_t s, const TrainLayout& L, float* tw, const float* A, RowMap amap, const float* Bm, RowMap bmap, int bmode,
                    int rows, int C, float* dst, long dst_stride, float* dst2, size_t cap_elems);
    int t_col_flush(hipStream_t s);
    float* t_h2_base = nullptr;
    void t_h2_plan();
    int t_h2_prepare(hipStream_t s, const TrainLayout& L, float* tw, int B);
    const float* t_h2_pack(const float* W, bool transposed) const;
    int t_linear_bwd(hipStream_t s, const TrainLayout& L, float* tw, const float* dY, RowMap dymap, int rows, int N, int K,
                     const float* Xin, RowMap xmap, const float* W, float* dX, RowMap dxmap, bool acc_dx, float* gW, float* gb);
};

}

struct capf_handle {
// ... 3 lines not shown
```

contextaware-poseformer_amd/csrc/igemm_f32h2_ws.hip:

```cpp
#include "igemm_f32h2_ws_tile.h"
#include "kernels.h"

namespace capf {

long f32h2_pack_elems(int Cout, int Cin) { return h2_pack_elems(Cout, Cin); }

static bool h2_from_args(const GemmArgs& a, H2Problem* q) {
    if (a.out_bf16 || !ws_args_ok(a, 3, 4.0, WS_MAX_P)) return false;
    if (!h2_plan(a.M / (a.H * a.W), a.H, a.W, a.Cin, a.N, 32, q)) return false;
    static const long wide_min = [] { const char* e = diag_env("CAPF_H2_WIDE_MIN_TILES"); return e ? atol(e) : 512L; }();
    if (a.N % 64 == 0 && (long)q->g.tiles_m * (a.N / 64) >= wide_min) { q->g.NS = 64; q->g.NSL = a.N / 64; }
    q->x = a.A;
    q->g.wp = reinterpret_cast<const unsigned short*>(a.Wp3);
    q->winv = reinterpret_cast<const float*>(q->g.wp + h2_piece_elems(a.N, a.Cin));
    q->g.bias = a.bias;
    q->res = a.res ? a.res + a.rmap.off : nullptr;
    q->y = a.out + a.omap.off;
    q->g.ldy = (int)a.omap.S1;
    q->g.ldr = a.res ? (int)a.rmap.S1 : (int)a.omap.S1;
    q->g.relu = a.act == ACT_RELU;
    q->ein = a.h2_ein;
    q->eout = a.h2_eout;
    q->utab = a.h2_utab;
    if (a.h2_eout && (a.res || a.N % 16 != 0 || a.omap.S1 != a.N)) return false;
    if (a.h2_ein && a.Cin % 16 != 0) return false;
    return true;
}

bool gemm_f32h2_ok(const GemmArgs& a) {
    H2Problem q;
    return h2_from_args(a, &q);
}
int f32h2_tiles_m(int B, int H, int W, int* tile_pixels) {
    H2Problem q;
    if (!h2_plan(B, H, W, 16, 16, 32, &q)) return 0;
    if (tile_pixels) *tile_pixels = q.g.P;
    return q.g.tiles_m;
}
bool f32h2_unit_table(int H, int W, int Cin, unsigned* out) { return h2_unit_table(H, W, Cin, out); }
bool f32h2_shape_ok(int B, int H, int W, int Cin, int Cout) {
    H2Problem q;
    return h2_plan(B, H, W, Cin, Cout, 32, &q);
}

struct H2GroupArgs {
    H2Problem g[MAXG];
    GroupLayout lay;
    int n;
};
static_assert(sizeof(H2GroupArgs) == MAXG * sizeof(H2Problem) + (2 * MAXG + 2) * sizeof(int), "kernel argument layout");

template <int TN, bool PIN = false, bool POUT = false>
__global__ __launch_bounds__(256, TN == 1 ? 3 : 2) void igemm_f32h2_group_ws_kernel(H2GroupArgs ga) {
#if defined(__HIP_DEVICE_COMPILE__)
    extern __shared__ __attribute__((aligned(16))) unsigned char h2_lds[];
    const GroupSlot t = group_slot(ga.lay, ga.n, blockIdx.x);
    if (!t.live) return;
    igemm_f32h2_ws_tile<TN, PIN, POUT>(ga.g[t.pi], t.bid, h2_lds);
#endif
}

template <int TN, bool PIN = false, bool POUT = false>
static hipError_t h2_launch(const H2Problem* list, int n, hipStream_t s) {
    int tiles[MAXG], order[MAXG];
    double cost[MAXG];
    for (int i = 0; i < n; ++i) { tiles[i] = list[i].g.tiles_m * list[i].g.NSL; cost[i] = list[i].g.C; }
    H2GroupArgs ga{};
    ga.n = n;
    const int start = group_layout(ga.lay, n, tiles, cost, order);
    for (int i = 0; i < n; ++i) ga.g[i] = list[order[i]];
    static DynLdsAttr attr;
    const hipError_t e = attr.ensure(reinterpret_cast<const void*>(&igemm_f32h2_group_ws_kernel<TN, PIN, POUT>), h2_lds_bytes(32 * TN));
    if (e != hipSuccess) return e;
    hipLaunchKernelGGL((igemm_f32h2_group_ws_kernel<TN, PIN, POUT>), dim3(start), dim3(256), h2_lds_bytes(32 * TN), s, ga);
    return hipGetLastError();
}

hipError_t launch_gemm_f32h2_group(const GemmArgs* list, int n, hipStream_t s) {
    if (n <= 0) return hipSuccess;
    if (n > MAXG) return hipErrorInvalidValue;
    H2Problem cls[2][3][MAXG];
    int cnt[2][3] = {{0, 0, 0}, {0, 0, 0}};
    for (int i = 0; i < n; ++i) {
        H2Problem q;
        if (!list[i].Wp3 || !list[i].x3_h2 || !h2_from_args(list[i], &q)) return hipErrorInvalidValue;
        if (q.ein && q.eout) return hipErrorInvalidValue;
        const int w = q.g.NS == 64 ? 1 : 0, k = q.ein ? 1 : (q.eout ? 2 : 0);
        cls[w][k][cnt[w][k]++] = q;
    }
    hipError_t e = hipSuccess;
    if (cnt[1][0] && e == hipSuccess) e = h2_launch<2>(cls[1][0], cnt[1][0], s);
    if (cnt[1][1] && e == hipSuccess) e = h2_launch<2, true, false>(cls[1][1], cnt[1][1], s);
    if (cnt[1][2] && e == hipSuccess) e = h2_launch<2, false, true>(cls[1][2], cnt[1][2], s);
    if (cnt[0][0] && e == hipSuccess) e = h2_launch<1>(cls[0][0], cnt[0][0], s);
    if (cnt[0][1] && e == hipSuccess) e = h2_launch<1, true, false>(cls[0][1], cnt[0][1], s);
    if (cnt[0][2] && e == hipSuccess) e = h2_launch<1, false, true>(cls[0][2], cnt[0][2], s);
    return e;
}

const char* gemm_f32h2_kernel_name(const GemmArgs&) { return "igemm_f32h2_group_ws"; }

__global__ void pack_conv_f32h2_kernel(const float* __restrict__ w, const float* __restrict__ gamma, const float* __restrict__ beta,
                                       const float* __restrict__ mean, const float* __restrict__ var, float eps,
                                       unsigned short* __restrict__ Wp, const float* __restrict__ winv, float* __restrict__ bias,
                                       int Cout, int Cin, long total) {
    const int ncc = Cin / 16;
    for (long i = blockIdx.x * (long)blockDim.x + threadIdx.x; i < total; i += (long)gridDim.x * blockDim.x) {
        const WsPackIdx d = ws_pack_decode(i, 32, ncc);
        float v = bn_fold_w3x3(w, gamma, beta, mean, var, eps, bias, Cout, Cin, d.ng, d.c, d.tap, d.first);
        if (d.ng < Cout) v *= __uint_as_float(0x7F000000u - __float_as_uint(winv[d.ng]));
        const long piece = 9L * 32 * 16;
        const long base = ((long)(d.sl * ncc + d.cc) * 2) * piece + ((long)d.tap * 32 + d.n) * 16 + d.qp * 8 + d.e;
        const _Float16 p0 = (_Float16)v;
        const _Float16 p1 = (_Float16)(v - (float)p0);
        Wp[base] = __builtin_bit_cast(unsigned short, p0);
        Wp[base + piece] = __builtin_bit_cast(unsigned short, p1);
    }
}

hipError_t launch_pack_conv_f32h2(const float* w, const float* gamma, const float* beta, const float* mean, const float* var, float eps,
                                  void* Wp_f16, float* bias, int Cout, int Cin, hipStream_t s) {
    if (Cin % 16 != 0 || Cout <= 0) return hipErrorInvalidValue;
    unsigned short* Wp = static_cast<unsigned short*>(Wp_f16);
    float* winv = reinterpret_cast<float*>(Wp + h2_piece_elems(Cout, Cin));
    const int npad = ((Cout + 31) / 32) * 32;
    const hipError_t e = launch_f32h2_wscale(w, gamma, var, eps, winv, npad, Cout, Cin * 9, s);
    if (e != hipSuccess) return e;
    const long total = h2_piece_elems(Cout, Cin) / 2;
    hipLaunchKernelGGL(pack_conv_f32h2_kernel, dim3(grid_1d(total)), dim3(256), 0, s, w, gamma, beta, mean, var, eps, Wp,
                       winv, bias, Cout, Cin, total);
    return hipGetLastError();
}

}
```

contextaware-poseformer_amd/csrc/igemm_f32h2_ws_tile.h:

```cpp
#pragma once
#ifndef H2_EXPERIMENT
#define H2_EXPERIMENT 0
#endif
#include <algorithm>

#include "igemm_bf16_ws_tile.h"

namespace capf {

static constexpr int H2_HP = WS_MAX_PP * 16 + 64;
static constexpr int H2_A_BYTES = 4 * H2_HP;
static constexpr int H2_AUX_BYTES = 16 + 2 * 64 * 4 + 4 * 64 * 4 + 16;
inline constexpr int h2_w_bytes(int NS) { return 2 * 9 * NS * 32; }
inline constexpr int h2_lds_bytes(int NS) { return H2_A_BYTES + h2_w_bytes(NS) + H2_AUX_BYTES; }

struct H2Problem {
    WsProblem g;
    const float* x;
    const float* res;
    float* y;
    const float* winv;
    const int* ein;
    int* eout;
    const unsigned* utab;
};
static constexpr int H2_NAU = 7;

inline long h2_piece_elems(int N, int C) { return (long)((N + 31) / 32) * (C / 16) * 2 * 9 * 32 * 16; }
inline long h2_pack_elems(int N, int C) { return h2_piece_elems(N, C) + 2L * ((N + 31) / 32) * 32; }

inline bool h2_plan(int B, int H, int W, int C, int N, int NS, H2Problem* q) {
    if (B <= 0 || H <= 0 || W <= 0 || N % 4 != 0 || (NS != 32 && NS != 64)) return false;
    if ((double)H * W * C * 4.0 * (WS_MAX_P / (H * W) + 2) >= 2.0e9 || (double)WS_MAX_P * N * 4.0 >= 2.0e9) return false;
    if (!ws_plan(B, H, W, C, (N + 7) & ~7, &q->g, true)) return false;
    q->g.N = N;
    q->g.ldy = q->g.ldr = N;
    q->g.NS = NS;
    q->g.NSL = (N + NS - 1) / NS;
    q->utab = nullptr;
    return true;
}

inline bool h2_unit_table(int H, int W, int C, unsigned* out) {
    H2Problem q;
    if (!h2_plan(1, H, W, C, 32, 32, &q)) return false;
    const WsProblem& p = q.g;
    if (p.G != 1 && p.RGPI != 1) return false;
    const int n_units = 4 * p.PP;
    for (int j = 0; j < H2_NAU; ++j)
        for (int tid = 0; tid < 256; ++tid) {
            const int qi = std::min(j * 256 + tid, n_units - 1);
            const int px = qi >> 2, qt = qi & 3;
            const int g = px / p.SEGP, rem = px - g * p.SEGP;
            const int rr = rem / p.PW, ww = rem - rr * p.PW;
            const int col = ww - 1;
            const long off = ((((long)g * p.H + rr - 1) * p.W + col) * p.C + qt * 4) * 4;
            if (off >= (1L << 31) || off < -(1L << 31)) return false;
            out[j * 256 + tid] = ((unsigned)(int)off & ~15u) | (col >= 0 && col < p.W ? 1u : 0u) | (rr == 0 ? 2u : 0u) | (rr == p.RH + 1 ? 4u : 0u);
        }
    return true;
}

inline __host__ __device__ int h2_scale_exp(int mbits) {
    const int sb = 268 - (mbits >> 23);
    return sb < 64 ? 64 : (sb > 190 ? 190 : sb);
}

#if defined(__HIP_DEVICE_COMPILE__)

typedef _Float16 ws_f16x8 __attribute__((ext_vector_type(8)));
typedef unsigned ws_u32x2 __attribute__((ext_vector_type(2)));

__device__ __forceinline__ void h2_split2(float x, float y, float s, unsigned& p1, unsigned& p2) {
    typedef _Float16 h2_t __attribute__((ext_vector_type(2)));
    typedef float f2_t __attribute__((ext_vector_type(2)));
    const f2_t v = f2_t{x, y} * s;
    const h2_t a = __builtin_convertvector(v, h2_t);
    const f2_t r = v - __builtin_convertvector(a, f2_t);
    const h2_t b = __builtin_convertvector(r, h2_t);
    p1 = __builtin_bit_cast(unsigned, a);
    p2 = __builtin_bit_cast(unsigned, b);
}

__device__ __forceinline__ unsigned h2_pk_mul(unsigned a, unsigned b) {
    typedef _Float16 h2_t __attribute__((ext_vector_type(2)));
    const h2_t r = __builtin_bit_cast(h2_t, a) * __builtin_bit_cast(h2_t, b);
    return __builtin_bit_cast(unsigned, r);
}

__device__ __forceinline__ int h2_wave_max(float v) {
    int x = __float_as_int(v);
    x = max(x, __builtin_amdgcn_update_dpp(0, x, 0xB1, 0xF, 0xF, true));
    x = max(x, __builtin_amdgcn_update_dpp(0, x, 0x4E, 0xF, 0xF, true));
    x = max(x, __builtin_amdgcn_update_dpp(0, x, 0x141, 0xF, 0xF, true));
    x = max(x, __builtin_amdgcn_update_dpp(0, x, 0x140, 0xF, 0xF, true));
    return max(max(__builtin_amdgcn_readlane(x, 0), __builtin_amdgcn_readlane(x, 16)),
               max(__builtin_amdgcn_readlane(x, 32), __builtin_amdgcn_readlane(x, 48)));
}

template <int TN, bool PIN = false, bool POUT = false>
__device__ __forceinline__ void igemm_f32h2_ws_tile(const H2Problem& q, const int bid, unsigned char* __restrict__ lds) {
    constexpr int NS = 32 * TN;
    constexpr int WP_BYTES = 9 * 32 * 32;
    constexpr int WS_BYTES = 2 * WP_BYTES;
    constexpr int W2_BYTES = TN * WS_BYTES;
    constexpr int NWI = W2_BYTES / 1024;
    constexpr int NWS = (NWI + 3) / 4;
    constexpr int NAU = H2_NAU;
    constexpr unsigned OOB = 0x80000000u;
    const WsProblem& p = q.g;
    const int tid = threadIdx.x, lane = tid & 63;
    const int wave = __builtin_amdgcn_readfirstlane(tid >> 6);
    const int frow = lane & 31, fhalf = lane >> 5;
    const int NCC = p.C >> 4;
    const int tm = bid / p.NSL, slice = bid - tm * p.NSL;

    const int b_first = ws_div(tm * p.G, p.d_rgpi);
    const ws_rsrc_t rs_x = __builtin_amdgcn_make_buffer_rsrc((void*)(q.x + (size_t)b_first * p.H * p.W * p.C), 0, 0x7FFFFF00u, 0x00020000);
    constexpr int HP = H2_HP;
    unsigned a_voff[NAU], a_lds[NAU];
    [[maybe_unused]] unsigned a_cls = 0;
    const int n_units = 4 * p.PP;
    const bool tab_ok = !(H2_EXPERIMENT & 128) && !PIN && q.utab != nullptr && (p.G == 1 || (p.RGPI == 1 && (tm + 1) * p.G <= p.RG));
    if (tab_ok) {
        const int k = tm * p.G - b_first * p.RGPI;
        const unsigned kill = (k == 0 ? 2u : 0u) | (k == p.RGPI - 1 ? 4u : 0u);
        const int base = k * p.RH * p.W * p.C * 4;
#pragma unroll
        for (int j = 0; j < NAU; ++j) {
            const unsigned t = q.utab[j * 256 + tid];
            const int qi = min(j * 256 + tid, n_units - 1);
            const int px = qi >> 2, qt = qi & 3;
            a_lds[j] = (unsigned)((qt >> 1) * HP + px * 16 + (qt & 1) * 8);
            a_voff[j] = ((t & 1u) && !(t & kill)) ? (unsigned)((int)(t & ~15u) + base) : OOB;
        }
    } else {
        const int q0 = tm * p.G;
#pragma unroll
        for (int j = 0; j < NAU; ++j) {
            const int qi = min(j * 256 + tid, n_units - 1);
            const int px = qi >> 2, qt = qi & 3;
            a_lds[j] = PIN ? (unsigned)((2 * (qt >> 1) + (qt & 1)) * HP + px * 16)
                           : (unsigned)((qt >> 1) * HP + px * 16 + (qt & 1) * 8);
#if (H2_EXPERIMENT & 64)
            a_voff[j] = (unsigned)(qi * 16 + q0);
            continue;
#endif
            const int g = ws_div(px, p.d_segp), rem = px - g * p.SEGP;
            const int rr = ws_div(rem, p.d_pw), ww = rem - rr * p.PW;
            if (PIN) a_cls |= (rr == 0 ? 1u : (rr == p.RH + 1 ? 2u : 0u)) << (2 * j);
            const int sg = q0 + g;
            const int b = ws_div(sg, p.d_rgpi);
            const int h = (sg - b * p.RGPI) * p.RH + rr - 1, col = ww - 1;
            const bool ok = sg < p.RG && h >= 0 && h < p.H && col >= 0 && col < p.W;
            a_voff[j] = ok ? (unsigned)(((((b - b_first) * p.H + h) * p.W + col) * p.C + qt * 4) * 4) : OOB;
        }
    }
    ws_f32x4 ar[NAU];
    auto load_a = [&](int cc) {
#pragma unroll
        for (int j = 0; j < NAU; ++j)
            ar[j] = __builtin_bit_cast(ws_f32x4, __builtin_amdgcn_raw_buffer_load_b128(rs_x, a_voff[j], (unsigned)cc * 64u, 0));
    };
    int* const aux = reinterpret_cast<int*>(lds + H2_A_BYTES + W2_BYTES);
    float* const aux_w = reinterpret_cast<float*>(aux + 4);
    float* const aux_b = aux_w + 64;
    int* const aux_px = reinterpret_cast<int*>(aux_b + 64) + wave * 64;
    [[maybe_unused]] int* const aux_o = reinterpret_cast<int*>(aux_b + 64) + 4 * 64;
    [[maybe_unused]] int e_nb[3] = {190, 190, 190};
    [[maybe_unused]] const int* e_row[3] = {nullptr, nullptr, nullptr};
    if constexpr (PIN) {
        e_row[0] = q.ein + (size_t)tm * NCC;
        if (p.G == 1 && p.RH < p.H) {
            const int k = tm - ws_div(tm, p.d_rgpi) * p.RGPI;
            if (k > 0) e_row[1] = q.ein + (size_t)(tm - 1) * NCC;
            if (k + 1 < p.RGPI) e_row[2] = q.ein + (size_t)(tm + 1) * NCC;
        }
    }
    [[maybe_unused]] int e_raw[3] = {190, 190, 190};
    auto load_e = [&](int cc) {
        if constexpr (PIN) {
#pragma unroll
            for (int k = 0; k < 3; ++k) e_raw[k] = e_row[k] ? e_row[k][cc] : 190;
        }
    };
    auto use_e = [&]() {
        if constexpr (PIN) {
#pragma unroll
            for (int k = 0; k < 3; ++k) e_nb[k] = __builtin_amdgcn_readfirstlane(e_raw[k]);
        }
    };
    [[maybe_unused]] unsigned has_cls[3] = {0, 0, 0};
    if constexpr (PIN) {
#pragma unroll
        for (int j = 0; j < NAU; ++j) {
            const unsigned c = (a_cls >> (2 * j)) & 3;
#pragma unroll
            for (int k = 0; k < 3; ++k) has_cls[k] |= (__builtin_amdgcn_ballot_w64(c == (unsigned)k) != 0 ? 1u : 0u) << j;
        }
    }
    auto store_planes = [&](int sn) {
        const unsigned moved = (e_nb[0] != sn ? has_cls[0] : 0u) | ((e_nb[1] != sn && e_nb[1] != 190) ? has_cls[1] : 0u) |
                               ((e_nb[2] != sn && e_nb[2] != 190) ? has_cls[2] : 0u);
#pragma unroll
        for (int j = 0; j < NAU; ++j) {
            const ws_u32x4 src = __builtin_bit_cast(ws_u32x4, ar[j]);
            unsigned w0 = src[0], w1 = src[1], w2 = src[2], w3 = src[3];
            if ((moved >> j) & 1) {
                const int cls = (a_cls >> (2 * j)) & 3;
                const int en = cls == 0 ? e_nb[0] : (cls == 1 ? e_nb[1] : e_nb[2]);
                const int r = en == 190 ? 0 : sn - en;
                const int r1 = r >= -14 ? r : -14, r2 = r - r1;
                const unsigned hb = (unsigned)(15 + r1) << 10, mb = hb | (hb << 16);
                w0 = h2_pk_mul(w0, mb); w1 = h2_pk_mul(w1, mb); w2 = h2_pk_mul(w2, mb); w3 = h2_pk_mul(w3, mb);
                if (__builtin_amdgcn_ballot_w64(r2 < 0)) {
                    const unsigned gb = r2 >= -14 ? (unsigned)(15 + r2) << 10 : (r2 >= -24 ? 1u << (24 + r2) : 0u), nb = gb | (gb << 16);
                    w0 = h2_pk_mul(w0, nb); w1 = h2_pk_mul(w1, nb); w2 = h2_pk_mul(w2, nb); w3 = h2_pk_mul(w3, nb);
                }
            }
            *reinterpret_cast<ws_u32x4*>(lds + a_lds[j]) = ws_u32x4{w0, w1, w2, w3};
        }
    };
    auto publish_max = [&]() {
        if constexpr (PIN) return;
#if (H2_EXPERIMENT & 1)
        return;
#endif
        float m = 0.f;
#pragma unroll
        for (int j = 0; j < NAU; ++j)
#pragma unroll
            for (int e = 0; e < 4; ++e) m = fmaxf(m, fabsf(ar[j][e]));
        const int wm = h2_wave_max(m);
        if (lane == 0) aux[wave] = wm;
    };
    auto block_scale_exp = [&]() -> int {
        if constexpr (PIN) return min(e_nb[0], min(e_nb[1], e_nb[2]));
#if (H2_EXPERIMENT & 1)
        return 127;
#endif
        const ws_u32x4 v = *reinterpret_cast<const ws_u32x4*>(aux);
        const int m = max(max((int)v[0], (int)v[1]), max((int)v[2], (int)v[3]));
        return __builtin_amdgcn_readfirstlane(h2_scale_exp(m));
    };
    auto split_a = [&](float s) {
        if constexpr (PIN) { store_planes(__float_as_int(s) >> 23); return; }
#pragma unroll
        for (int j = 0; j < NAU; ++j) {
            ws_u32x2 u1, u2;
#if (H2_EXPERIMENT & 1)
            u1[0] = __float_as_uint(ar[j][0]); u1[1] = __float_as_uint(ar[j][1]); u2[0] = __float_as_uint(ar[j][2]); u2[1] = __float_as_uint(ar[j][3]);
            *reinterpret_cast<ws_u32x2*>(lds + a_lds[j]) = u1;
            *reinterpret_cast<ws_u32x2*>(lds + 2 * HP + a_lds[j]) = u2;
            continue;
#endif
#pragma unroll
            for (int k = 0; k < 2; ++k) {
                unsigned s1, s2;
                h2_split2(ar[j][2 * k], ar[j][2 * k + 1], s, s1, s2);
                u1[k] = s1; u2[k] = s2;
            }
            *reinterpret_cast<ws_u32x2*>(lds + a_lds[j]) = u1;
            *reinterpret_cast<ws_u32x2*>(lds + 2 * HP + a_lds[j]) = u2;
        }
    };
    const unsigned w_voff = (unsigned)lane * 16u;
    const int nsl32 = (p.N + 31) >> 5;
    const ws_rsrc_t rs_w = __builtin_amdgcn_make_buffer_rsrc((void*)(p.wp + (size_t)slice * TN * NCC * (WS_BYTES / 2)), 0,
                                                             (unsigned)(nsl32 - slice * TN) * (unsigned)NCC * (unsigned)WS_BYTES, 0x00020000);
    auto fire_w = [&](int cc) {
#pragma unroll
        for (int i = 0; i < NWS; ++i) {
            const int k = min(i * 4 + wave, NWI - 1);
            const int j = k / 18, rem = k - j * 18;
            __builtin_amdgcn_raw_ptr_buffer_load_lds(rs_w, (ws_lptr_t)(lds + H2_A_BYTES + k * 1024), 16, w_voff,
                                                     (unsigned)(j * NCC + cc) * (unsigned)WS_BYTES + (unsigned)rem * 1024u, 0, 0);
        }
    };
    load_a(0);
    load_e(0);
    if (POUT && tid < 4) aux_o[tid] = 0;
    if (tid < NS) {
        const int n = slice * NS + tid;
        aux_w[tid] = n < ((p.N + 31) & ~31) ? q.winv[n] : 1.f;
        aux_b[tid] = (p.bias && n < p.N) ? p.bias[n] : 0.f;
    }

    int pl_i[2];
    {
        const int in_g1 = (frow >= 4 && frow < 12) || (frow >= 16 && frow < 20) || frow >= 28;
        const int pos = in_g1 ? (frow < 12 ? frow - 4 : (frow < 20 ? frow - 8 : frow - 16))
                              : (frow < 4 ? frow : (frow < 16 ? frow - 8 : frow - 12));
        if ((p.W & 15) == 0) {
#pragma unroll
            for (int i = 0; i < 2; ++i) pl_i[i] = ((2 * wave + i) * 2 + in_g1) * 16 + pos;
        } else {
            unsigned short* tab = reinterpret_cast<unsigned short*>(lds);
            unsigned short* ovf = tab + 256;
            int* cnt = reinterpret_cast<int*>(lds + 1024);
            if (tid < 18) cnt[tid] = 0;
            asm volatile("s_waitcnt lgkmcnt(0)" ::: "memory");
            __builtin_amdgcn_s_barrier();
            if (tid < p.P) {
                const int g = ws_div(tid, p.d_rhw), rem = tid - g * p.RHW;
                const int r = ws_div(rem, p.d_w), w = rem - r * p.W;
                const int c = ((g * (p.RH + 2) + r) * p.PW + w) & 15;
                const int rank = atomicAdd(&cnt[c], 1);
                if (rank < 16) tab[rank * 16 + c] = (unsigned short)tid;
                else ovf[atomicAdd(&cnt[16], 1)] = (unsigned short)tid;
            }
            asm volatile("s_waitcnt lgkmcnt(0)" ::: "memory");
            __builtin_amdgcn_s_barrier();
            if ((tid >> 4) >= cnt[tid & 15]) {
                const int e = atomicAdd(&cnt[17], 1);
                tab[tid] = e < cnt[16] ? ovf[e] : (unsigned short)0xFFFFu;
            }
            asm volatile("s_waitcnt lgkmcnt(0)" ::: "memory");
            __builtin_amdgcn_s_barrier();
#pragma unroll
            for (int i = 0; i < 2; ++i) pl_i[i] = tab[((2 * wave + i) * 2 + in_g1) * 16 + pos];
            asm volatile("s_waitcnt lgkmcnt(0)" ::: "memory");
            __builtin_amdgcn_s_barrier();
        }
    }
    fire_w(0);
    unsigned a_addr[2][3];
#pragma unroll
    for (int i = 0; i < 2; ++i) {
        int pl = pl_i[i];
        if (pl >= p.P) { pl = 0; pl_i[i] = 0x7FFF; }
        const int g = ws_div(pl, p.d_rhw), rem = pl - g * p.RHW;
        const int r = ws_div(rem, p.d_w), w = rem - r * p.W;
        const int pix0 = (g * (p.RH + 2) + r) * p.PW + w;
#pragma unroll
        for (int kh = 0; kh < 3; ++kh) a_addr[i][kh] = (unsigned)((pix0 + kh * p.PW) * 16 + fhalf * HP);
    }
    const unsigned b_addr = (unsigned)(H2_A_BYTES + frow * 32 + ((fhalf ^ ((frow >> 3) & 1)) << 4));
    if (fhalf == 0) { aux_px[frow] = pl_i[0]; aux_px[32 + frow] = pl_i[1]; }

    const int Mi = (int)p.M;
    const int gp0 = tm * p.G * p.RHW;
    const ws_rsrc_t rs_res = __builtin_amdgcn_make_buffer_rsrc(q.res ? (void*)(q.res + (size_t)gp0 * p.ldr) : (void*)q.y, 0, q.res ? 0x7FFFFF00u : 0u,
                                                               0x00020000);
    const ws_rsrc_t rs_out = __builtin_amdgcn_make_buffer_rsrc((void*)(q.y + (size_t)gp0 * p.ldy), 0, 0x7FFFFF00u, 0x00020000);
    constexpr int PW_[3] = {0, 1, 0};
    constexpr int PA_[3] = {1, 0, 0};

    publish_max();
    asm volatile("s_waitcnt lgkmcnt(0)" ::: "memory");
    __builtin_amdgcn_s_barrier();
    use_e();
    int sb = block_scale_exp();
    int smin = sb;
    split_a(__int_as_float(sb << 23));

    ws_f32x16 acc[2][TN];
#pragma unroll
    for (int i = 0; i < 2; ++i)
#pragma unroll
        for (int j = 0; j < TN; ++j)
#pragma unroll
            for (int e = 0; e < 16; ++e) acc[i][j][e] = 0.f;
    asm volatile("s_waitcnt vmcnt(0) lgkmcnt(0)" ::: "memory");
    if (NCC > 1) { load_a(1); load_e(1); }
    __builtin_amdgcn_s_barrier();

    const int er = lane >> 2, ec = (lane & 3) * 8;
    auto row_off = [&](int pl, int j, int q, int ld) -> unsigned {
        const int n = slice * NS + j * 32 + ec + 4 * q;
        const int gp = gp0 + pl;
        return (pl < p.P && gp < Mi && n < p.N) ? (unsigned)(pl * ld + n) * 4u : OOB;
    };
    ws_f32x4 rr[2][TN][4];
    ws_f16x8 af[2][2][2], bfr[2][2][TN];
    for (int cc = 0; cc < NCC; ++cc) {
        if (cc == NCC - 1 && !(H2_EXPERIMENT & 32) && !POUT) {
#pragma unroll
            for (int i = 0; i < 2; ++i)
#pragma unroll
                for (int h = 0; h < 2; ++h) {
                    const int pl = aux_px[i * 32 + h * 16 + er];
#pragma unroll
                    for (int j = 0; j < TN; ++j)
#pragma unroll
                        for (int q = 0; q < 2; ++q)
                            rr[i][j][h * 2 + q] = __builtin_bit_cast(ws_f32x4, __builtin_amdgcn_raw_buffer_load_b128(rs_res, row_off(pl, j, q, p.ldr), 0, 0));
                }
        }
        auto read_frags = [&](int t, int buf) {
            if ((H2_EXPERIMENT & 16) && (t > 0 || cc > 0)) return;
#pragma unroll
            for (int o = 0; o < 2; ++o) {
                const int pw = PW_[o], pa = PA_[o];
#pragma unroll
                for (int j = 0; j < TN; ++j)
                    bfr[buf][pw][j] = __builtin_bit_cast(ws_f16x8, *reinterpret_cast<const ws_f32x4*>(lds + b_addr + j * WS_BYTES + pw * WP_BYTES + t * 1024));
#pragma unroll
                for (int i = 0; i < 2; ++i)
                    af[buf][pa][i] = __builtin_bit_cast(ws_f16x8, *reinterpret_cast<const ws_f32x4*>(lds + pa * 2 * HP + (t % 3) * 16 + a_addr[i][t / 3]));
            }
        };
        read_frags(0, 0);
        __builtin_amdgcn_sched_barrier(0);
#pragma unroll
        for (int t = 0; t < 9; ++t) {
            if (t < 8) read_frags(t + 1, (t + 1) & 1);
#pragma unroll
            for (int k = 0; k < 3; ++k)
#pragma unroll
                for (int j = 0; j < TN; ++j)
#pragma unroll
                    for (int i = 0; i < 2; ++i)
                        if (!(H2_EXPERIMENT & 8)) acc[i][j] = __builtin_amdgcn_mfma_f32_32x32x16_f16(bfr[t & 1][PW_[k]][j], af[t & 1][PA_[k]][i], acc[i][j], 0, 0, 0);
                        else acc[i][j][0] += (float)bfr[t & 1][PW_[k]][j][0] + (float)af[t & 1][PA_[k]][i][0];
            if (t < 8) {
#pragma unroll
                for (int x = 0; x < 4 + 2 * TN; ++x) {
                    __builtin_amdgcn_sched_group_barrier(0x008, 1, 0);
                    __builtin_amdgcn_sched_group_barrier(0x100, 1, 0);
                }
                if (6 * TN > 4 + 2 * TN) __builtin_amdgcn_sched_group_barrier(0x008, 6 * TN - (4 + 2 * TN), 0);
            }
            __builtin_amdgcn_sched_barrier(0);
        }
        if (cc + 1 < NCC) {
            publish_max();
            asm volatile("s_waitcnt lgkmcnt(0)" ::: "memory");
            __builtin_amdgcn_s_barrier();
            if (!(H2_EXPERIMENT & 2)) fire_w(cc + 1);
            use_e();
            const int sn = min(block_scale_exp(), smin + 80);
            smin = min(smin, sn);
            if (sn != sb) {
                const float f = __int_as_float((127 + sn - sb) << 23);
#pragma unroll
                for (int i = 0; i < 2; ++i)
#pragma unroll
                    for (int j = 0; j < TN; ++j)
#pragma unroll
                        for (int e = 0; e < 16; ++e) acc[i][j][e] *= f;
                sb = sn;
            }
            split_a(__int_as_float(sb << 23));
            asm volatile("s_waitcnt vmcnt(0) lgkmcnt(0)" ::: "memory");
            if (cc + 2 < NCC && !(H2_EXPERIMENT & 4)) { load_a(cc + 2); load_e(cc + 2); }
            __builtin_amdgcn_s_barrier();
        }
    }

    if (H2_EXPERIMENT & 32) {
        float t = 0.f;
#pragma unroll
        for (int i = 0; i < 2; ++i)
#pragma unroll
            for (int j = 0; j < TN; ++j)
#pragma unroll
                for (int e = 0; e < 16; ++e) t += acc[i][j][e];
        if (t == 1234.5678f) q.y[tid] = t;
        return;
    }
    const float inv_s = __int_as_float((254 - sb) << 23);
    if constexpr (POUT) {
#pragma unroll
        for (int j = 0; j < TN; ++j) {
            float m[2] = {0.f, 0.f};
#pragma unroll
            for (int g = 0; g < 4; ++g) {
                const ws_f32x4 wv = *reinterpret_cast<const ws_f32x4*>(aux_w + j * 32 + 8 * g + 4 * fhalf);
                const ws_f32x4 bv = *reinterpret_cast<const ws_f32x4*>(aux_b + j * 32 + 8 * g + 4 * fhalf);
#pragma unroll
                for (int i = 0; i < 2; ++i)
#pragma unroll
                    for (int e = 0; e < 4; ++e) {
                        const float t = fmaf(acc[i][j][4 * g + e], wv[e] * inv_s, bv[e]);
                        m[g >> 1] = fmaxf(m[g >> 1], p.relu ? fmaxf(t, 0.f) : fabsf(t));
                    }
            }
            const int w0 = h2_wave_max(m[0]), w1 = h2_wave_max(m[1]);
            if (lane == 0) { atomicMax(&aux_o[2 * j], w0); atomicMax(&aux_o[2 * j + 1], w1); }
        }
    }
    asm volatile("s_waitcnt lgkmcnt(0)" ::: "memory");
    __builtin_amdgcn_s_barrier();
    constexpr int EPS = 36;
    float* ep = reinterpret_cast<float*>(lds) + wave * (32 * EPS);
    [[maybe_unused]] const int hi_chunk = (lane >> 1) & 1;
    if constexpr (POUT) {
        const int nck = p.N >> 4;
        if (tid < 2 * TN && slice * 2 * TN + tid < nck) q.eout[(size_t)tm * nck + slice * 2 * TN + tid] = h2_scale_exp(aux_o[tid]);
    }
#pragma unroll
    for (int j = 0; j < TN; ++j) {
        ws_f32x4 wv[2], bv[2];
#pragma unroll
        for (int q = 0; q < 2; ++q) {
            wv[q] = *reinterpret_cast<const ws_f32x4*>(aux_w + j * 32 + ec + 4 * q);
            bv[q] = *reinterpret_cast<const ws_f32x4*>(aux_b + j * 32 + ec + 4 * q);
#pragma unroll
            for (int e = 0; e < 4; ++e) wv[q][e] *= inv_s;
        }
#pragma unroll
        for (int i = 0; i < 2; ++i) {
            __builtin_amdgcn_wave_barrier();
#pragma unroll
            for (int g = 0; g < 4; ++g)
                *reinterpret_cast<ws_f32x4*>(&ep[frow * EPS + 8 * g + 4 * fhalf]) =
                    ws_f32x4{acc[i][j][4 * g], acc[i][j][4 * g + 1], acc[i][j][4 * g + 2], acc[i][j][4 * g + 3]};
            __builtin_amdgcn_wave_barrier();
#pragma unroll
            for (int h = 0; h < 2; ++h) {
                const int row = h * 16 + er;
                const int pl = aux_px[i * 32 + row];
                [[maybe_unused]] ws_f32x4 ov[2];
#pragma unroll
                for (int q = 0; q < 2; ++q) {
                    const ws_f32x4 x = *reinterpret_cast<const ws_f32x4*>(&ep[row * EPS + ec + 4 * q]);
                    ws_f32x4 o;
#pragma unroll
                    for (int e = 0; e < 4; ++e) {
                        const float t = POUT ? fmaf(x[e], wv[q][e], bv[q][e]) : fmaf(x[e], wv[q][e], bv[q][e] + rr[i][j][h * 2 + q][e]);
                        o[e] = p.relu ? fmaxf(t, 0.f) : t;
                    }
                    if constexpr (POUT) ov[q] = o;
                    else __builtin_amdgcn_raw_buffer_store_b128(__builtin_bit_cast(ws_u32x4, o), rs_out, row_off(pl, j, q, p.ldy), 0, 0);
                }
                if constexpr (POUT) {
                    const float sc = __int_as_float(h2_scale_exp(aux_o[2 * j + hi_chunk]) << 23);
                    ws_u32x4 p0, p1;
#pragma unroll
                    for (int qq = 0; qq < 2; ++qq)
#pragma unroll
                        for (int k = 0; k < 2; ++k) {
                            unsigned s1, s2;
                            h2_split2(ov[qq][2 * k], ov[qq][2 * k + 1], sc, s1, s2);
                            p0[2 * qq + k] = s1; p1[2 * qq + k] = s2;
                        }
                    const int n = slice * NS + j * 32 + ec;
                    const bool ok = pl < p.P && gp0 + pl < Mi && n < p.N;
                    const unsigned off = ok ? (unsigned)(pl * p.ldy + (n & ~15)) * 4u + (unsigned)(n & 15) * 2u : OOB;
                    __builtin_amdgcn_raw_buffer_store_b128(p0, rs_out, off, 0, 0);
                    __builtin_amdgcn_raw_buffer_store_b128(p1, rs_out, ok ? off + 32u : OOB, 0, 0);
                }
            }
        }
    }
}

#endif

}
```

contextaware-poseformer_amd/csrc/kernels.h:

```cpp
#pragma once
#include <hip/hip_runtime.h>
#include <stdint.h>

#include <stdlib.h>

namespace capf {

inline const char* diag_env(const char* name) {
#ifdef CAPF_DIAG
    return getenv(name);
#else
    (void)name;
    return nullptr;
#endif
}

__host__ __device__ __forceinline__ unsigned pack_bf16x2(float lo, float hi) {
#if defined(__HIP_DEVICE_COMPILE__)
    typedef __bf16 bf16x2_t __attribute__((ext_vector_type(2)));
    typedef float f32x2_t __attribute__((ext_vector_type(2)));
    return __builtin_bit_cast(unsigned, __builtin_convertvector(f32x2_t{lo, hi}, bf16x2_t));
#else
    (void)lo; (void)hi;
    return 0u;
#endif
}
__host__ __device__ __forceinline__ unsigned short to_bf16(float f) { return (unsigned short)(pack_bf16x2(f, 0.f) & 0xFFFFu); }

struct BilinearCorner {
    int x0, y0;
    float wx1, wy1;
};
#if defined(__HIPCC__)
template <bool BORDER>
__device__ __forceinline__ BilinearCorner bilinear_corner(float gx, float gy, int H, int W) {
    float x = ((gx + 1.0f) / 2.0f) * (float)(W - 1);
    float y = ((gy + 1.0f) / 2.0f) * (float)(H - 1);
    if (BORDER) {
        x = fminf((float)(W - 1), fmaxf(x, 0.0f));
        y = fminf((float)(H - 1), fmaxf(y, 0.0f));
    }
    const float xf = floorf(x), yf = floorf(y);
    BilinearCorner c;
    c.x0 = (int)xf;
    c.y0 = (int)yf;
    c.wx1 = x - xf;
    c.wy1 = y - yf;
    return c;
}
#endif

struct RowMap {
    int G;
    long S1, S2, off;
};
inline RowMap row_ld(long ld, long off = 0) { return RowMap{1, ld, 0, off}; }

enum Act { ACT_NONE = 0, ACT_RELU = 1, ACT_GELU = 2 };

struct FastDiv {
    unsigned mul, shift;
};
FastDiv make_fastdiv(unsigned d);

struct DynLdsAttr {
    unsigned long long seen = 0;
    hipError_t ensure(const void* kernel, int bytes) {
        int dev = 0;
        hipError_t e = hipGetDevice(&dev);
        if (e != hipSuccess) return e;
        if (dev >= 0 && dev < 64 && ((seen >> dev) & 1ull)) return hipSuccess;
        e = hipFuncSetAttribute(kernel, hipFuncAttributeMaxDynamicSharedMemorySize, bytes);
        if (e == hipSuccess && dev >= 0 && dev < 64) seen |= 1ull << dev;
        return e;
    }
};

struct GemmArgs {
    const float* A;
    const float* Wp;
    const float* Wp2;
    const float* Wp3;
    int x3_h2;
    const float* Wh2;
    const float* bias;
    const float* res;
    float* out;
    int M, N, K, Kpad;
    int conv;
    int Cin, H, W, Ho, Wo, ks, stride, pad;
    RowMap amap, omap, rmap;
    int act;
    FastDiv fd_hw, fd_wo;
    unsigned long long spread;
    const float* rscale;
    int rs_div;
    int splits, cps;
    long split_stride;
    int out_bf16;
    float* split_ws;
    int* split_cnt;
    long split_ws_elems;
    int split_cnt_elems;
    const float* ln_g;
    const float* ln_b;
    float ln_eps;
    const void* up;
    int up_H, up_W;
    float up_sh, up_sw;
    const int* h2_ein;
    int* h2_eout;
    const unsigned* h2_utab;
    int f32s;
    int out_f32;
    void* out_sh;
};

struct ResBlockW {
    const float *ln1_g, *ln1_b, *wqkv, *bqkv, *wproj, *bproj, *ln2_g, *ln2_b, *wfc1, *bfc1, *wfc2, *bfc2;
};
bool res_chain_ok(int dim, int tokens, int heads, int nblk);
hipError_t launch_res_chain_repack(const float* h2g_pack, float* chain_pack, int N, int K, hipStream_t s);
hipError_t launch_res_chain(float* X, int rows, int tokens, int heads, float eps, const ResBlockW* blk, int nblk, hipStream_t s);
hipError_t launch_mlp_chain(float* X, RowMap rows_map, int rows, float eps, const ResBlockW& blk, hipStream_t s);

inline int grid_1d(long total, int cap = 4096) {
    const long want = (total + 255) / 256;
    return (int)(want < cap ? want : cap);
}

#if defined(__HIPCC__)
__device__ __forceinline__ float bn_scale(const float* __restrict__ gamma, const float* __restrict__ var, float eps, int n) {
    return gamma ? gamma[n] / sqrtf(var[n] + eps) : 1.f;
}
__device__ __forceinline__ float bn_bias(const float* __restrict__ gamma, const float* __restrict__ beta, const float* __restrict__ mean, float sc, int n) {
    return gamma ? beta[n] - mean[n] * sc : 0.f;
}
__device__ __forceinline__ float bn_fold_w3x3(const float* __restrict__ w, const float* __restrict__ gamma, const float* __restrict__ beta,
                                              const float* __restrict__ mean, const float* __restrict__ var, float eps, float* __restrict__ bias,
                                              int Cout, int Cin, int ng, int c, int tap, bool first) {
    if (ng >= Cout) return 0.f;
    const float sc = bn_scale(gamma, var, eps, ng);
    if (bias && first) bias[ng] = bn_bias(gamma, beta, mean, sc, ng);
    return w[(((long)ng * Cin + c) * 3 + tap / 3) * 3 + tap % 3] * sc;
}
#endif

hipError_t launch_gemm_f32(const GemmArgs& a, hipStream_t s);
static constexpr int MAXG = 8;

struct GroupLayout {
    int start[MAXG + 1];
    int tiles[MAXG];
};
inline void group_order(int n, const double* cost, int* order) {
    for (int i = 0; i < n; ++i) {
        int j = i;
        for (; j > 0 && cost[i] > cost[order[j - 1]]; --j) order[j] = order[j - 1];
        order[j] = i;
    }
}
inline int group_fill(GroupLayout& lay, int n, const int* tiles) {
    int start = 0;
    for (int i = 0; i < MAXG; ++i) {
        lay.start[i] = start;
        lay.tiles[i] = i < n ? tiles[i] : 0;
        start += (lay.tiles[i] + 7) & ~7;
    }
    lay.start[MAXG] = start;
    return start;
}
inline int group_layout(GroupLayout& lay, int n, const int* tiles, const double* cost, int* order) {
    group_order(n, cost, order);
    int sorted[MAXG];
    for (int i = 0; i < n; ++i) sorted[i] = tiles[order[i]];
    return group_fill(lay, n, sorted);
}
#if defined(__HIPCC__)
struct GroupSlot { int pi, bid; bool live; };
__device__ __forceinline__ GroupSlot group_slot(const GroupLayout& lay, int n, int b) {
    int pi = 0;
    while (pi + 1 < n && b >= lay.start[pi + 1]) ++pi;
    const int l = b - lay.start[pi];
    const int per_xcd = (lay.start[pi + 1] - lay.start[pi]) >> 3;
    const int bid = (l & 7) * per_xcd + (l >> 3);
    return GroupSlot{pi, bid, bid < lay.tiles[pi]};
}
#endif

inline bool ws_args_ok(const GemmArgs& a, int align_mask, double elem_bytes, long rows) {
    if (!a.conv || a.ks != 3 || a.stride != 1 || a.pad != 1 || a.Ho != a.H || a.Wo != a.W || a.act == ACT_GELU || a.rscale ||
        a.omap.G != 1 || (a.res && a.rmap.G != 1) || a.M <= 0 || a.H <= 0 || a.W <= 0 || a.M % (a.H * a.W) != 0)
        return false;
    if ((a.omap.S1 & align_mask) || (a.omap.off & align_mask) || (a.res && ((a.rmap.S1 & align_mask) || (a.rmap.off & align_mask)))) return false;
    return (double)rows * (double)a.omap.S1 * elem_bytes < 2.0e9 && (!a.res || (double)rows * (double)a.rmap.S1 * elem_bytes < 2.0e9);
}
bool gemm_f32_groupable(const GemmArgs& a);
bool gemm_f32_rows_splitk(const GemmArgs& a);
hipError_t launch_gemm_f32_group(const GemmArgs* list, int n, hipStream_t s);
enum class F32Path { PW, H2G, SPLITK_GROUP, ROWS_SPLITK, STEM_BF16, STEM_STREAM, SMALLC, TILE };
struct F32Route { F32Path path; int tile; };
F32Route gemm_f32_route(const GemmArgs& a);
const char* gemm_f32_kernel_name(const GemmArgs& a);
bool gemm_f32_pw_ok(const GemmArgs& a);
hipError_t launch_gemm_f32_pw(const GemmArgs& a, hipStream_t s);
const char* gemm_f32_pw_kernel_name();
bool gemm_f32_pwchain_ok(const GemmArgs& a, const GemmArgs& b);
hipError_t launch_gemm_f32_pwchain(const GemmArgs& a, const GemmArgs& b, hipStream_t s);
const char* gemm_f32_pwchain_kernel_name();
bool bneck0_bf16_ok(const GemmArgs& c1, const GemmArgs& c2, const GemmArgs& ds, const GemmArgs& c3);
hipError_t launch_bneck0_bf16(const GemmArgs& c1, const GemmArgs& c2, const GemmArgs& ds, const GemmArgs& c3, bool tap, hipStream_t s);
const char* bneck0_bf16_kernel_name();
bool bneck1_bf16_ok(const GemmArgs& c1, const GemmArgs& c2, const GemmArgs& c3);
hipError_t launch_bneck1_bf16(const GemmArgs& c1, const GemmArgs& c2, const GemmArgs& c3, bool tap, hipStream_t s);
const char* bneck1_bf16_kernel_name();
bool gemm_bf16_pwchain_ok(const GemmArgs& a, const GemmArgs& b);
hipError_t launch_gemm_bf16_pwchain(const GemmArgs& a, const GemmArgs& b, hipStream_t s);
const char* gemm_bf16_pwchain_kernel_name();

bool gemm_wino_ok(const GemmArgs& a);
hipError_t launch_gemm_wino(const GemmArgs& a, hipStream_t s);
hipError_t launch_gemm_wino_group(const GemmArgs* list, int n, hipStream_t s);
enum class WinoPath { X3, F43_GROUP, WINO };
WinoPath gemm_wino_route(const GemmArgs& a);
const char* gemm_wino_kernel_name(const GemmArgs& a);
hipError_t launch_pack_conv_wino(const float* w, const float* gamma, const float* beta, const float* mean, const float* var,
                                 float eps, float* Wp, float* bias, int Cout, int Cin, hipStream_t s, int variant = 23);

hipError_t launch_pack_conv(const float* w, const float* gamma, const float* beta, const float* mean,
                            const float* var, float eps, float* Wp, float* bias, int Cout, int Cin,
                            int ks, int Kpad, hipStream_t s);
hipError_t launch_pack_conv_bf16(const float* w, const float* gamma, const float* beta, const float* mean,
                                 const float* var, float eps, void* Wp_bf16, float* bias, int Cout, int Cin, int ks,
                                 int Kpad, hipStream_t s);
hipError_t launch_gemm_bf16(const GemmArgs& a, hipStream_t s);
int f32h2_tiles_m(int B, int H, int W, int* tile_pixels = nullptr);
bool gemm_bf16_groupable(const GemmArgs& a);
bool gemm_bf16_upadd_ok(const GemmArgs& a);
hipError_t launch_gemm_bf16_group(const GemmArgs* list, int n, hipStream_t s, int* variant = nullptr);
enum class Bf16Path { WS, RH, T128x32, T128x64, T64x64, T128x128 };
struct Bf16Route { Bf16Path path; bool pp; };
Bf16Route gemm_bf16_route(const GemmArgs& a);
const char* gemm_bf16_kernel_name(const GemmArgs& a);
int bf16_rh_width(int Cin);
int gemm_bf16_rh_cw(const GemmArgs& a);
hipError_t launch_gemm_bf16_rh(const GemmArgs& a, hipStream_t s);
hipError_t launch_pack_conv_bf16_rh(const float* w, const float* gamma, const float* beta, const float* mean, const float* var,
                                    float eps, void* Wp_bf16, float* bias, int Cout, int Cin, int CW, hipStream_t s);
bool gemm_bf16_ws_ok(const GemmArgs& a);
int gemm_bf16_ws_tiles(const GemmArgs& a);
bool gemm_bf16_ws_wanted(const GemmArgs& a);
long bf16_ws_pack_elems(int Cout, int Cin);
hipError_t launch_gemm_bf16_ws(const GemmArgs& a, hipStream_t s);
hipError_t launch_gemm_bf16_ws_group(const GemmArgs* list, int n, hipStream_t s);
const char* gemm_bf16_ws_kernel_name(const GemmArgs& a);
hipError_t launch_pack_conv_bf16_ws(const float* w, const float* gamma, const float* beta, const float* mean, const float* var,
                                    float eps, void* Wp_bf16, float* bias, int Cout, int Cin, hipStream_t s);

bool gemm_f32x3_ok(const GemmArgs& a);
bool gemm_f32x3_wanted(const GemmArgs& a);
bool f32x3_takes(int B, int H, int W, int Cin, int Cout, bool h2);
long f32x3_pack_elems(int Cout, int Cin);
hipError_t launch_gemm_f32x3(const GemmArgs& a, hipStream_t s);
hipError_t launch_gemm_f32x3_group(const GemmArgs* list, int n, hipStream_t s);
const char* gemm_f32x3_kernel_name(const GemmArgs& a);
hipError_t launch_pack_conv_f32x3(const float* w, const float* gamma, const float* beta, const float* mean, const float* var, float eps,
                                  void* Wp_bf16, float* bias, int Cout, int Cin, hipStream_t s);
long f32h2_pack_elems(int Cout, int Cin);
hipError_t launch_gemm_f32h2_group(const GemmArgs* list, int n, hipStream_t s);
bool gemm_f32h2_ok(const GemmArgs& a);
static constexpr int F32H2_UNIT_TABLE_WORDS = 7 * 256;
bool f32h2_unit_table(int H, int W, int Cin, unsigned* out);
bool f32h2_shape_ok(int B, int H, int W, int Cin, int Cout);
const char* gemm_f32h2_kernel_name(const GemmArgs& a);
hipError_t launch_pack_conv_f32h2(const float* w, const float* gamma, const float* beta, const float* mean, const float* var, float eps,
                                  void* Wp_f16, float* bias, int Cout, int Cin, hipStream_t s);
long f32h2_gemm_pack_elems(int N, int Kpad);
hipError_t launch_f32h2_wscale(const float* w, const float* gamma, const float* var, float eps, float* winv, int rows, int N, int K, hipStream_t s);
bool gemm_f32h2g_ok(const GemmArgs& a);
hipError_t launch_gemm_f32h2g(const GemmArgs& a, hipStream_t s);
hipError_t launch_gemm_f32h2g_group(const GemmArgs* list, int n, hipStream_t s);
const char* gemm_f32h2g_kernel_name(const GemmArgs& a, bool grouped);
hipError_t launch_pack_f32h2_gemm(const float* w, const float* gamma, const float* beta, const float* mean, const float* var, float eps,
                                  float* Wp, float* bias, int N, int Cin, int ks, int K, int Kpad, hipStream_t s);
hipError_t launch_pack_f32h2_gemm_rows(const float* w, float* Wp, int n0, int n, int Ntot, int K, int Kpad, hipStream_t s);
struct H2TrainW {
    const float* w;
    long fwd_off, bwd_off;
    int N, K, ld, tile_start, max_off, pad_;
};
hipError_t launch_pack_f32h2_train(const H2TrainW* tab_dev, int n, int tiles, float* base, int* maxima, long maxima_elems, hipStream_t s);
bool gemm_bf16_smallc_ok(const GemmArgs& a);
hipError_t launch_gemm_bf16_smallc(const GemmArgs& a, hipStream_t s);
const char* gemm_bf16_smallc_kernel_name(const GemmArgs& a);
hipError_t launch_pack_linear(const float* w, float* Wp, int N, int K, int Kpad, hipStream_t s);
hipError_t launch_pack_linear_quad(const float* w, float* Wq, int N, int K, int n0, int Ntot, hipStream_t s);
hipError_t launch_gemm_bf16_rows(const void* A_bf16, const void* W_bf16, const float* bias, int M, int N, int K, int Kpad,
                                 float* out, RowMap omap, const float* res, RowMap rmap, int gelu_bf16_out, hipStream_t s);
const char* gemm_bf16_rows_kernel_name(int M, int N);

struct FuseSumArgs {
    const float* in[4];
    int shift[4];
    int n_in;
    float* out;
    int B, H, W, C;
    int relu;
    int bf16;
    void* out_sh;
};
hipError_t launch_fuse_sum(const FuseSumArgs& a, hipStream_t s);
hipError_t launch_fuse_sum_group(const FuseSumArgs* a, int n, hipStream_t s);

hipError_t launch_maxpool3x3s2(const float* in, float* out, int B, int H, int W, int C, int Ho, int Wo,
                               hipStream_t s, int bf16 = 0);
hipError_t launch_bilinear_resize(const float* in, float* out, int B, int H, int W, int C, int Ho, int Wo,
                                  hipStream_t s, int bf16 = 0, const float* add = nullptr);

struct CopySegment {
    const float* src;
    float* dst;
    int n, pad;
};
hipError_t launch_copy_segments(const CopySegment* table_dev, int n, hipStream_t s);

hipError_t launch_prep_embed(float* kcrop, const float* k2d, const float* w, const float* bias,
                             const float* pos, float* X, int B, int J, int L1, int C, hipStream_t s);
hipError_t launch_sample_ref(const float* feat, const float* ref, float* S, int* idx, int B, int J, int H,
                             int W, int C, hipStream_t s, int feat_bf16 = 0);
hipError_t launch_layernorm(const float* in, RowMap imap, const float* add, RowMap amap, const float* g,
                            const float* b, float eps, float* out, int rows, int C, hipStream_t s, int out_bf16 = 0);
struct DeformArgs {
    const float* feat[4];
    int H[4], W[4], C[4];
    float* U[4];
    const float* AO;
    const float* ref;
    int B, J, L, NH, NS;
    int feat_bf16;
    int ld_ao;
    const float* dU[4];
    float* cpos;
    int* cidx;
};
hipError_t launch_deform_sample(const DeformArgs& a, hipStream_t s);
hipError_t launch_bilinear_corners(const float* grid, int n, int H, int W, int border, int* idx, float* frac, hipStream_t s);
struct EmbedArgs {
    float* kcrop;
    const float* k2d;
    const float* cw; const float* cb;
    const float* pos;
    const float* feat[4]; int H[4], W[4], Cl[4];
    const float* fw[4]; const float* fb[4];
    float* sampled[4];
    int* idx[4];
    float* X;
// ... 95 lines not shown
```

contextaware-poseformer_amd/csrc/plan.cpp:

```cpp
#include <limits.h>
#include <stdlib.h>

#include <algorithm>
#include <map>
#include <tuple>

#include "engine.h"

namespace capf {

static const int EXT_IMAGES = -2;

static size_t round64(size_t n) { return (n + 63) / 64 * 64; }
static int round32(int n) { return (n + 31) / 32 * 32; }
static int round64(int n) { return (n + 63) / 64 * 64; }

int Engine::add_param(const std::string& name, int kind, std::initializer_list<int64_t> shape) {
    auto it = param_index.find(name);
    if (it != param_index.end()) return it->second;
    Param p;
    p.name = name;
    p.kind = kind;
    p.ndim = (int)shape.size();
    int i = 0;
// ... 867 lines not shown
void Engine::assign_offsets() {
    struct Live { size_t off, size; int last; };
    std::vector<int> order(bufs.size());
    for (size_t i = 0; i < bufs.size(); ++i) order[i] = (int)i;
    std::stable_sort(order.begin(), order.end(), [&](int a, int b) { return bufs[a].def_op < bufs[b].def_op; });
    for (Buffer& b : bufs)
        for (const auto& rg : regions) {
            const bool touches = b.def_op <= rg.second && b.last_op >= rg.first;
            if (touches && b.last_op < rg.second) b.last_op = rg.second;
            if (touches && b.def_op > rg.first) b.def_op = rg.first;
        }
    std::stable_sort(order.begin(), order.end(), [&](int a, int b) { return bufs[a].def_op < bufs[b].def_op; });
    std::vector<Live> live;
    size_t top = 0;
    for (int id : order) {
        Buffer& b = bufs[id];
        live.erase(std::remove_if(live.begin(), live.end(), [&](const Live& l) { return l.last < b.def_op; }), live.end());
        std::sort(live.begin(), live.end(), [](const Live& x, const Live& y) { return x.off < y.off; });
        size_t off = 0;
        for (const Live& l : live) {
            if (off + b.elems <= l.off) break;
            off = std::max(off, l.off + l.size);
        }
        b.offset = off;
        live.push_back(Live{off, b.elems, b.last_op});
        top = std::max(top, off + b.elems);
    }
    ws_elems_per_frame = top;
}

void Engine::schedule_regions() {
    region_levels.assign(regions.size(), {});
    for (size_t r = 0; r < regions.size(); ++r) {
        const int lo = regions[r].first + 1, hi = regions[r].second;
        std::vector<int> level(hi - lo, 0);
        auto has = [](const auto& slots, int b) { return std::find(slots.begin(), slots.end(), b) != slots.end(); };
        auto reads = [&](const Op& o, int b) { return has(o.reads(), b); };
        auto writes = [&](const Op& o, int b) { return has(o.writes(), b); };
        auto touched = [&](const Op& o) {
            std::vector<int> v;
            for (int b : o.reads()) if (b >= 0) v.push_back(b);
            for (int b : o.writes()) if (b >= 0) v.push_back(b);
            return v;
        };
        int max_level = 0;
        for (int i = lo; i < hi; ++i) {
            const Op& oi = ops[i];
            for (int j = lo; j < i; ++j) {
                const Op& oj = ops[j];
                bool dep = false;
                for (int b : touched(oi))
                    if ((writes(oj, b)) || (reads(oj, b) && writes(oi, b))) { dep = true; break; }
                if (dep) level[i - lo] = std::max(level[i - lo], level[j - lo] + 1);
            }
            max_level = std::max(max_level, level[i - lo]);
        }
        for (int i = lo; i < hi; ++i) {
            const Op& oi = ops[i];
            if (oi.kind != OP_FUSE || oi.debug_only) continue;
            bool sink = true;
            for (int j = i + 1; j < hi && sink; ++j) {
                const Op& oj = ops[j];
                for (int b : touched(oj))
                    if (writes(oi, b) || (reads(oi, b) && writes(oj, b))) { sink = false; break; }
            }
            if (sink) level[i - lo] = max_level;
        }
        region_levels[r].assign(max_level + 1, {});
        for (int i = lo; i < hi; ++i) region_levels[r][level[i - lo]].push_back(i);
    }
}

bool Engine::set_plan_switches() {
    PlanSwitches& p = plan;
    if (cfg.plan_flags & CAPF_PLAN_NO_FUSED_LIFTER) p.fused_lifter = false;
    if (cfg.plan_flags & CAPF_PLAN_NO_WINOGRAD) p.use_wino = false;
    if (cfg.plan_flags & CAPF_PLAN_NO_ROW_HALO) p.use_rh = false;
    if (cfg.plan_flags & CAPF_PLAN_WINOGRAD_F23_ONLY) p.wino_f43 = false;
    if (cfg.plan_flags & CAPF_PLAN_NO_PWCHAIN) p.use_pwchain = false;
    if (cfg.plan_flags & CAPF_PLAN_NO_UPADD) p.use_upadd = false;
    if (cfg.plan_flags & CAPF_PLAN_NO_BNECK) p.use_bneck = false;
    if (cfg.plan_flags & CAPF_PLAN_NO_BATCHED_REDUCE) p.batch_reduce = false;
    if (cfg.plan_flags & CAPF_PLAN_H2_PLANES) p.use_h2_planes = true;
    if (cfg.plan_flags & CAPF_PLAN_NO_WS) p.use_ws = false;
    if (cfg.plan_flags & CAPF_PLAN_NO_F32X3) p.use_x3 = false;
    if (cfg.plan_flags & CAPF_PLAN_F32X3_EXACT) p.x3_h2 = false;
    if (cfg.plan_flags & CAPF_PLAN_NO_F32H2_GEMM) p.use_h2g = false;
    if (cfg.plan_flags & CAPF_PLAN_BF16_F32_STREAM) {
        if (!bf16()) { err = "CAPF_PLAN_BF16_F32_STREAM needs compute_dtype = CAPF_BF16"; return false; }
        if (cfg.backbone != CAPF_HRNET) { err = "CAPF_PLAN_BF16_F32_STREAM is an HRNet plan (CPN50 is not supported)"; return false; }
        if (cfg.plan_flags != CAPF_PLAN_BF16_F32_STREAM) { err = "CAPF_PLAN_BF16_F32_STREAM cannot be combined with other plan flags"; return false; }
        p.f32_stream = true;
        p.use_bneck = false;
        p.use_pwchain = false;
    }
    if (const char* fz = diag_env("CAPF_LIFTER_FUSED")) p.fused_lifter = atoi(fz) != 0;
    if (const char* wz = diag_env("CAPF_WINO")) p.use_wino = atoi(wz) != 0;
    if (const char* rz = diag_env("CAPF_BF16_RH")) p.use_rh = atoi(rz) != 0;
    if (const char* wb = diag_env("CAPF_WINO_MIN_BATCH")) p.wino_min_batch = atoi(wb);
    if (const char* wf = diag_env("CAPF_WINO_F43")) p.wino_f43 = atoi(wf) != 0;
    if (const char* wf = diag_env("CAPF_WINO_F43_MINHW")) p.wino_f43_min_hw = atoi(wf);
    if (const char* wf = diag_env("CAPF_WINO_F43_CPN")) p.wino_f43_cpn = atoi(wf) != 0;
    if (const char* wf = diag_env("CAPF_WINO_F43_MAXHW")) p.wino_f43_max_hw = atoi(wf);
    if (cfg.embed_dim_ratio > 256) p.fused_lifter = false;
    if (cfg.backbone == CAPF_HRNET && cfg.hr_channels[3] > 512) p.fused_lifter = false;
    return true;
}

bool Engine::build() {
    if (cfg.height % 32 != 0 || cfg.width % 32 != 0) {
        err = "height and width must be multiples of 32";
        return false;
    }
    if (cfg.levels != 4 || cfg.num_joints <= 0 || cfg.embed_dim_ratio % (4 * cfg.num_heads) != 0 ||
        cfg.embed_dim_ratio % (4 * cfg.deform_heads) != 0 || cfg.deform_samples != 4 || cfg.deform_heads != 4) {
        err = "unsupported lifter configuration (levels must be 4, 4x4 deformable sampling, embed_dim_ratio % 32 == 0)";
        return false;
    }
    if (cfg.depth != 0 && cfg.depth != cfg.levels) {
        const bool mpi_width = (cfg.base_dim == 32 && cfg.embed_dim_ratio == 64) || (cfg.base_dim == 48 && cfg.embed_dim_ratio == 96);
        if (cfg.depth < 1 || cfg.depth > 8 || cfg.context_blocks || (cfg.training && !mpi_width)) {
            err = cfg.context_blocks ? "depth != levels: 1..8 blocks per group, only for the variant without context blocks (ContextPose_mpi) and only for "
                                       "inference plans"
                  : (cfg.depth < 1 || cfg.depth > 8) ? "depth != levels: 1..8 blocks per group (the variant without context blocks, ContextPose_mpi)"
                  : "depth != levels with training = 1: only at the ContextPose_mpi widths (embed_dim_ratio 64 over base_dim 32, 96 over 48); "
                    "other widths train at depth == levels";
            return false;
        }
    }
    if (!set_plan_switches()) return false;
    Tensor img{EXT_IMAGES, cfg.height, cfg.width, 3};
    Tensor feats[4];
    if (cfg.backbone == CAPF_HRNET) {
        for (int i = 0; i < 4; ++i)
            if (cfg.hr_channels[i] <= 0 || cfg.hr_channels[i] % 4 != 0) {
                err = "HRNet branch widths must be positive multiples of 4";
                return false;
            }
        build_hrnet(img, feats);
        if (plan.f32_stream && !plan_f32_stream(feats)) return false;
    } else if (cfg.backbone == CAPF_CPN50) {
        build_cpn(img, feats);
    } else {
        err = "unknown backbone";
        return false;
    }
    for (int l = 0; l < 4; ++l) {
        name_tensor(*this, "feat" + std::to_string(l), feats[l].buf, {-1, feats[l].H, feats[l].W, feats[l].C}, maps_bf16() ? 2 : 0);
        const int expect = cfg.backbone == CAPF_CPN50 ? cfg.base_dim : cfg.base_dim << l;
        if (feats[l].C != expect) {
            err = "poseformer.base_dim does not match the backbone's context-map widths";
            return false;
        }
    }
    n_backbone_ops = (int)ops.size();
    for (int l = 0; l < 4; ++l) {
        feat_buf[l] = feats[l].buf; feat_H[l] = feats[l].H; feat_W[l] = feats[l].W; feat_C[l] = feats[l].C;
    }
    build_lifter(feats);
    grad_off.assign(params.size(), -1);
    grad_elems = 0;
    for (size_t i = 0; i < params.size(); ++i)
        if (params[i].name.rfind("volume_net.", 0) == 0) {
            grad_off[i] = grad_elems;
            grad_elems += params[i].numel();
        }
// ... 15 lines not shown
        if (a.kind != OP_GEMM || b.kind != OP_GEMM || !a.conv || !b.conv || a.bf16 || b.bf16) continue;
        if (a.ks != 1 || b.ks != 1 || a.stride != 1 || b.stride != 1 || a.Cin != 64 || a.N != 256 || b.Cin != 256 || b.N != 64) continue;
        if (b.in[0] != a.out || b.region != a.region || b.lane != a.lane || a.aux < 0 || b.aux >= 0) continue;
        a.pw_pair = b.pw_pair = 1;
    }
    for (Op& op : ops) {
        if (op.kind != OP_GEMM || !op.wino || !packs[op.pack].x3) continue;
        const double cap = plan.x3_h2 ? 2.0e9 / ((double)op.H * op.W) : 2.0e9 / ((double)op.H * op.W * (double)std::max(op.Cin, op.N) * 4.0);
        int hi = (int)std::min(1.0e6, cap);
        while (hi >= 1 && hi > (int)cap - 4 && !f32x3_takes(hi, op.H, op.W, op.Cin, op.N, plan.x3_h2)) --hi;
        if (hi < 1 || !f32x3_takes(hi, op.H, op.W, op.Cin, op.N, plan.x3_h2)) continue;
        int lo = 1, top = hi;
        while (lo < top) {
            const int mid = lo + (top - lo) / 2;
            if (f32x3_takes(mid, op.H, op.W, op.Cin, op.N, plan.x3_h2)) top = mid; else lo = mid + 1;
        }
        op.x3_lo = lo; op.x3_hi = hi;
        if (lo <= plan.wino_min_batch && hi >= cfg.max_batch) packs[op.pack].wino_skip = true;
    }
    utab_host.clear();
    if (plan.x3_h2 && plan.use_x3) {
        std::map<std::tuple<int, int, int>, long> seen;
        for (Op& op : ops) {
            if (op.kind != OP_GEMM || !op.wino || !packs[op.pack].x3 || op.x3_hi < op.x3_lo) continue;
            const auto key = std::make_tuple(op.H, op.W, op.Cin);
            auto it = seen.find(key);
            if (it == seen.end()) {
                std::vector<unsigned> t(F32H2_UNIT_TABLE_WORDS);
                long at = -1;
                if (f32h2_unit_table(op.H, op.W, op.Cin, t.data())) {
                    at = (long)utab_host.size();
                    utab_host.insert(utab_host.end(), t.begin(), t.end());
                }
                it = seen.emplace(key, at).first;
            }
            op.h2_utab = it->second;
        }
    }
    size_t off = 0;
    for (Pack& pk : packs) {
        if (pk.in_place) continue;
        pk.w_off = off;
        off += pk.wino_skip ? 64 : round64(pk.bf16 ? ((size_t)pk.N * pk.Kpad + 1) / 2 : (size_t)pk.N * pk.Kpad);
        if (pk.wino) {
            pk.direct_off = off;
            off += round64((size_t)pk.N * pk.direct_Kpad);
        }
        if (pk.rh) {
            pk.rh_off = off;
            off += round64(((size_t)pk.N * pk.rh_Kpad + 1) / 2);
        }
        if (pk.ws) {
            pk.ws_off = off;
            off += round64(((size_t)bf16_ws_pack_elems(pk.N, pk.Cin) + 1) / 2);
        }
        if (pk.x3) {
            pk.x3_off = off;
            off += round64(((size_t)(plan.x3_h2 ? f32h2_pack_elems(pk.N, pk.Cin) : f32x3_pack_elems(pk.N, pk.Cin)) + 1) / 2);
        }
        pk.b_off = off;
        off += round64((size_t)pk.N);
    }
    for (Pack& pk : packs)
        if (pk.h2g) {
            pk.h2g_off = off;
            off += round64((size_t)f32h2_gemm_pack_elems(pk.N, pk.h2g_Kpad));
            if (pk.chain) {
                pk.chain_off = off;
                off += round64((size_t)f32h2_gemm_pack_elems(pk.N, pk.h2g_Kpad));
            }
        }
    {
        size_t nseg = 0;
        for (const Pack& pk : packs)
            if (pk.kind == LINEAR && !pk.in_place) nseg += (size_t)pk.n_lin;
        bias_tab_off = off;
        off += round64(nseg * (sizeof(CopySegment) / sizeof(float)));
    }
    t_h2_plan();
    t_h2_tab_off = off;
    off += round64(t_h2_specs.size() * (sizeof(H2TrainW) / sizeof(float)) + 16);
    utab_off = off;
    off += round64(utab_host.size() + 16);
    pack_elems = off;
    return true;
}

}
```

include/capf.h:

```cpp
#ifndef CAPF_H
#define CAPF_H

#include <stddef.h>
#include <stdint.h>

#ifdef __cplusplus
extern "C" {
#endif
#pragma GCC visibility push(default)

typedef struct capf_handle capf_handle;

enum capf_status {
    CAPF_OK = 0,
    CAPF_ERR_INVALID = -1,
    CAPF_ERR_UNSUPPORTED = -2,
    CAPF_ERR_HIP = -3,
    CAPF_ERR_STATE = -4
};

enum capf_backbone { CAPF_HRNET = 0, CAPF_CPN50 = 1 };
enum capf_dtype { CAPF_F32 = 0, CAPF_BF16 = 1 };

enum capf_param_kind {
    CAPF_P_CONV_W = 0,
    CAPF_P_BN_W = 1, CAPF_P_BN_B = 2, CAPF_P_BN_MEAN = 3, CAPF_P_BN_VAR = 4, CAPF_P_BN_NBT = 5,
    CAPF_P_LIN_W = 6, CAPF_P_LIN_B = 7,
    CAPF_P_LN_W = 8, CAPF_P_LN_B = 9,
    CAPF_P_RAW = 10
};

typedef struct capf_config {
    int32_t backbone;
    int32_t hr_channels[4];
    int32_t hr_modules[3];
    int32_t hr_blocks;
    int32_t base_dim;
    int32_t embed_dim_ratio;
    int32_t levels;
    int32_t num_joints;
    int32_t num_heads;
    int32_t deform_heads;
    int32_t deform_samples;
    int32_t context_blocks;
    int32_t compute_dtype;
    int32_t max_batch;
    int32_t height, width;
    int32_t training;
    int32_t plan_flags;
    int32_t depth;
} capf_config;

enum capf_plan_flag {
    CAPF_PLAN_NO_FUSED_LIFTER = 1,
    CAPF_PLAN_NO_WINOGRAD = 2,
    CAPF_PLAN_NO_ROW_HALO = 4,
    CAPF_PLAN_WINOGRAD_F23_ONLY = 8,
    CAPF_PLAN_NO_PWCHAIN = 16,
    CAPF_PLAN_NO_WS = 32,
    CAPF_PLAN_LIFTER_FP32 = 64,
    CAPF_PLAN_NO_F32X3 = 128,
    CAPF_PLAN_NO_F32H2_GEMM = 512,
    CAPF_PLAN_NO_UPADD = 1024,
    CAPF_PLAN_H2_PLANES = 2048,
    CAPF_PLAN_NO_BNECK = 4096,
    CAPF_PLAN_NO_BATCHED_REDUCE = 8192,
    CAPF_PLAN_BF16_F32_STREAM = 32768,
    CAPF_PLAN_F32X3_EXACT = 256
};

int capf_create(const capf_config* cfg, int device, capf_handle** out);
void capf_destroy(capf_handle* h);
int capf_max_batch(const capf_handle* h);
const char* capf_last_error(const capf_handle* h);
const char* capf_version(void);
#define CAPF_ABI_VERSION 9
int capf_abi_version(void);

int capf_num_params(const capf_handle* h);
int capf_param_info(const capf_handle* h, int index, const char** name, int64_t shape[4],
                    int* ndim, int* kind);

int capf_set_param(capf_handle* h, const char* name, const void* dev_ptr, const int64_t* shape,
                   int ndim);

int capf_params_changed(capf_handle* h, void* stream);

int capf_lifter_params_changed(capf_handle* h, void* stream);

size_t capf_workspace_bytes(const capf_handle* h, int batch);
int capf_set_workspace(capf_handle* h, void* dev_ptr, size_t bytes);

int capf_forward(capf_handle* h, void* stream, const float* images_nhwc, const float* k2d,
                 float* kcrop_inout, int batch, float* out);

int capf_backbone_forward(capf_handle* h, void* stream, const float* images_nhwc, int batch);

int capf_forward_train(capf_handle* h, void* stream, const float* images_nhwc, const float* k2d,
                       float* kcrop_inout, int batch, float* out, const float* drop_masks);
int capf_backward(capf_handle* h, void* stream, const float* grad_out, int batch, float* flat_grad,
                  const float* drop_masks);
int64_t capf_train_generation(const capf_handle* h);
int64_t capf_grad_elems(const capf_handle* h);
int capf_grad_info(const capf_handle* h, int param_index, int64_t* offset);
int capf_train_h2_matrices(const capf_handle* h);
int capf_mpjpe(void* stream, const float* pred, const float* gt, int rows, float* loss, float* dpred,
               float grad_scale);
int capf_mpjpe_nd(void* stream, const float* pred, const float* gt, int rows, int dim, float* loss, float* dpred,
                  float grad_scale);
int capf_adamw_step(void* stream, float* params, const float* grads, float* exp_avg, float* exp_avg_sq,
                    int64_t n, float lr, float beta1, float beta2, float eps, float weight_decay, int step,
                    float grad_scale);

int capf_lifter_forward(capf_handle* h, void* stream, const float* k2d, float* kcrop_inout, int batch,
                        float* out);

int capf_set_lanes(capf_handle* h, int on);

int capf_set_debug(capf_handle* h, int on);

int capf_tensor(const capf_handle* h, const char* name, const void** dev_ptr, int64_t shape[4],
                int* ndim);

int capf_forward_profile_variants(const capf_handle* h, int32_t* op_variant, int n_ops);
int capf_forward_stats(const capf_handle* h, int batch, int64_t* launches, double* flops);

int capf_op_pack_conv(void* stream, const float* w_oihw, const float* gamma, const float* beta,
                      const float* mean, const float* var, float eps, float* w_packed, float* bias,
                      int Cout, int Cin, int ks);
int capf_op_conv(void* stream, const float* x_nhwc, const float* w_packed, const float* bias,
                 const float* residual, float* y_nhwc, int B, int H, int W, int Cin, int Cout, int ks,
                 int stride, int act);
typedef struct capf_conv_desc {
    const float* x;
    const float* w_packed;
    const float* bias;
    const float* residual;
    float* y;
    int32_t B, H, W, Cin, Cout, ks, stride, act;
} capf_conv_desc;
int capf_op_conv_group(void* stream, int n, const capf_conv_desc* convs);
int capf_op_pack_conv_wino(void* stream, const float* w, const float* gamma, const float* beta, const float* mean,
                           const float* var, float eps, float* wp, float* bias, int Cout, int Cin, int variant);
int capf_op_conv_wino(void* stream, const float* x, const float* wp, const float* bias, const float* residual, float* y, int B,
                      int H, int W, int Cin, int Cout, int act, int variant);
int capf_op_conv_wino_group(void* stream, int n, const capf_conv_desc* d, int variant);
int capf_op_linear(void* stream, const float* x, const float* w, const float* bias, const float* residual,
                   float* y, int M, int N, int K, int act);
int capf_op_bilinear_corners(void* stream, const float* grid, int n, int H, int W, int border, int32_t* idx, float* frac);
int capf_op_pack_conv_bf16(void* stream, const float* w_oihw, const float* gamma, const float* beta,
                           const float* mean, const float* var, float eps, void* w_packed_bf16, float* bias,
                           int Cout, int Cin, int ks);
int capf_op_conv_bf16(void* stream, const void* x_nhwc_bf16, const void* w_packed_bf16, const float* bias,
                      const void* residual_bf16, void* y_nhwc_bf16, int B, int H, int W, int Cin, int Cout,
                      int ks, int stride, int act);

int capf_op_conv_bf16_rh_width(int Cin);
int capf_op_pack_conv_bf16_rh(void* stream, const float* w_oihw, const float* gamma, const float* beta, const float* mean,
                              const float* var, float eps, void* w_packed_bf16, float* bias, int Cout, int Cin);
int capf_op_conv_bf16_rh(void* stream, const void* x_nhwc_bf16, const void* w_packed_bf16, const float* bias,
                         const void* residual_bf16, void* y_nhwc_bf16, int B, int H, int W, int Cin, int Cout, int act);

int64_t capf_op_conv_bf16_ws_pack_elems(int Cout, int Cin);
int capf_op_pack_conv_bf16_ws(void* stream, const float* w_oihw, const float* gamma, const float* beta, const float* mean,
                              const float* var, float eps, void* w_packed_bf16, float* bias, int Cout, int Cin);
int capf_op_conv_bf16_ws_group(void* stream, int n, const capf_conv_desc* convs);

int64_t capf_op_conv_f32x3_pack_elems(int Cout, int Cin);
int capf_op_pack_conv_f32x3(void* stream, const float* w_oihw, const float* gamma, const float* beta, const float* mean,
                            const float* var, float eps, void* w_packed_bf16, float* bias, int Cout, int Cin);
int capf_op_conv_f32x3_group(void* stream, int n, const capf_conv_desc* convs);

int64_t capf_op_conv_f32h2_pack_elems(int Cout, int Cin);
int capf_op_pack_conv_f32h2(void* stream, const float* w_oihw, const float* gamma, const float* beta, const float* mean,
                            const float* var, float eps, void* w_packed_f16, float* bias, int Cout, int Cin);
int capf_op_conv_f32h2_group(void* stream, int n, const capf_conv_desc* convs);

int capf_op_conv_f32h2_tiles(int B, int H, int W, int* tile_pixels);
int capf_op_conv_f32h2_planes(void* stream, const capf_conv_desc* conv, const int32_t* exps_in, int32_t* exps_out);

int64_t capf_op_f32h2_gemm_pack_elems(int N, int K);
int capf_op_pack_f32h2_gemm(void* stream, const float* w, const float* gamma, const float* beta, const float* mean, const float* var,
                            float eps, float* w_packed, float* bias, int N, int Cin, int ks, int K);
int capf_op_conv_f32h2g(void* stream, const float* x_nhwc, const float* w_packed, const float* bias, const float* residual, float* y,
                        int B, int H, int W, int Cin, int Cout, int ks, int stride, int act);
int capf_op_conv_f32h2g_group(void* stream, int n, const capf_conv_desc* convs);
int capf_op_linear_f32h2g(void* stream, const float* x, const float* w_packed, const float* bias, const float* residual, float* y,
                          int M, int N, int K, int act);
int capf_op_wgrad(void* stream, const float* dY, const float* X, int M, int N, int K, float* dw_db, int two_piece);
int capf_op_linear_ln_f32h2g(void* stream, const float* x, const float* ln_gamma, const float* ln_beta, float eps, const float* w_packed,
                             const float* bias, const float* residual, float* y, int M, int N, int K, int act);

int capf_op_conv_bf16_group(void* stream, int n, const capf_conv_desc* convs, const void* const* w_row_halo, int32_t* variant);

int capf_op_linear_bf16(void* stream, const void* x_bf16, const void* w_bf16, const float* bias, const float* residual, void* y,
                        int M, int N, int K, int gelu_bf16_out);

int capf_preprocess(void* stream, const uint8_t* images_bgr, int batch, int height, int width, const float mean[3],
                    const float* std3, int mode, float* images_out, const float* gt_in, float* gt_out,
                    const float* k2d_in, float* k2d_out, const float* kcrop_in, float* kcrop_out);
int capf_fliptest_fuse(void* stream, const float* pred2, int batch, float* out);
int capf_fliptest_fuse_swap(void* stream, const float* pred2, int batch, int joints, const int32_t* swap, float* out);

int capf_pose_errors(void* stream, const float* pred, const float* gt, int n, int joints, const int32_t* prev, float* err);
int capf_segment_sums(void* stream, const float* err, const int32_t* segment, const int32_t* prev, int n, int n_segments,
                      double* sums, int32_t* counts);
int capf_keypoints_loss(void* stream, int mode, const float* pred, const float* gt, const float* validity, int rows, int dim,
                        float threshold, float* loss, float* dpred);
int capf_pck_counts(void* stream, const float* pred, const float* gt, int n, int joints, int root, double to_mm, const int32_t* segment,
                    int n_segments, int32_t* counts, double* mpjpe_sums, int32_t* frames);

int capf_jpeg_info(const uint8_t* data, size_t n_bytes, int32_t* width, int32_t* height, int32_t* components, int32_t* h_samp,
                   int32_t* v_samp, size_t* scratch_bytes);
int capf_jpeg_coefficients(const uint8_t* data, size_t n_bytes, int16_t* coef, size_t coef_elems);
int capf_jpeg_decode(void* stream, const uint8_t* data, size_t n_bytes, uint8_t* out_bgr, size_t out_pitch_bytes, void* scratch,
                     size_t scratch_bytes);
int capf_jpeg_batch_info(int n, const uint8_t* const* data, const size_t* n_bytes, int subseq_bytes, int32_t* info, size_t* scratch_bytes);
int capf_jpeg_decode_batch(void* stream, int n, const uint8_t* const* data, const size_t* n_bytes, uint8_t* const* out_bgr,
                           const size_t* out_pitch_bytes, int16_t* coef_out, void* scratch, size_t scratch_bytes, int32_t* status,
                           int subseq_bytes);
int capf_jpeg_coefficients_subseq(const uint8_t* data, size_t n_bytes, int16_t* coef, size_t coef_elems, int subseq_bytes);
int capf_affine_from_center_scale(const double center[2], const double scale[2], int out_w, int out_h, double m[6]);
int capf_warp_affine(void* stream, const uint8_t* const* frames, const int32_t* dims, const double* m, int batch,
                     int out_h, int out_w, uint8_t* out);

int capf_num_ops(const capf_handle* h);
int capf_op_info(const capf_handle* h, int index, int batch, const char** name, const char** kernel,
                 double* flops);
int capf_op_executed_flops(const capf_handle* h, int index, int batch, double* flops);
int capf_op_bytes(const capf_handle* h, int index, int batch, double* bytes);
int capf_op_schedule(const capf_handle* h, int index, int32_t* region, int32_t* level, int32_t* lane,
                     int32_t reads[5], int32_t writes[6]);
typedef struct capf_op_desc {
    int32_t kind;
    int32_t backbone;
    int32_t conv;
    int32_t Cin, H, W, Cout, Ho, Wo, ks, stride, pad, act;
    int32_t in_dtype, out_dtype;
    int32_t mfma_bf16;
    int32_t n_in, shift[4], relu;
    int32_t p_weight, p_bn_weight;
    int32_t has_residual;
    int32_t checkpoint;
    int32_t rows_per_frame;
    int32_t p_bias, p_ln_weight, p_ln_bias;
    float eps;
    int32_t attn[4];
    int64_t maps[3][4];
    int32_t up_H, up_W;
} capf_op_desc;
int capf_forward_prefix(capf_handle* h, void* stream, const float* images_nhwc, const float* k2d, float* kcrop_inout,
                        int batch, float* out, int n_ops);
int capf_op_describe(const capf_handle* h, int index, capf_op_desc* desc);
int capf_op_describe_sized(const capf_handle* h, int index, void* desc, size_t desc_bytes);
int capf_op_tensor(const capf_handle* h, int index, int slot, const void** dev_ptr);
int capf_op_h2_planes(const capf_handle* h, int index, int batch, const void** exps, int32_t* tile_pixels);

int capf_forward_profile(capf_handle* h, void* stream, const float* images_nhwc, const float* k2d,
                         float* kcrop_inout, int batch, float* out, float* op_ms, int n_ops);
int capf_forward_profile_launches(capf_handle* h, void* stream, const float* images_nhwc, const float* k2d,
                                  float* kcrop_inout, int batch, float* out, float* op_ms, int32_t* op_leader,
                                  int n_ops);

#pragma GCC visibility pop
#ifdef __cplusplus
}
#endif
#endif
```

Baseline: 9855 frames/s.

## Run grouped fp16-split 3x3 convs as persistent workgroups walking precomputed tile lists

Grouped split-fp16 3x3 conv launches on 32-channel tiles now use a persistent walking kernel by default. Each workgroup reads a host-built, per-batch list of (problem, tile) entries from the pack arena. While it writes the current tile's epilogue, it prefetches the next tile's weights and activations, so the loads overlap and the per-tile workgroup startup cost goes away. In exchange it adds host-side list planning, cached per batch size and copied to the device once, plus a more complex kernel control flow, with a plan flag to fall back to one workgroup per tile.

```diff
diff --git a/contextaware-poseformer_amd/capf/lib.py b/contextaware-poseformer_amd/capf/lib.py
--- a/contextaware-poseformer_amd/capf/lib.py
+++ b/contextaware-poseformer_amd/capf/lib.py
@@ -7,6 +7,7 @@
 F32, BF16 = 0, 1
 PLAN_NO_FUSED_LIFTER, PLAN_NO_WINOGRAD, PLAN_NO_ROW_HALO, PLAN_WINOGRAD_F23_ONLY, PLAN_NO_PWCHAIN, PLAN_NO_WS, PLAN_LIFTER_FP32, PLAN_NO_F32X3, PLAN_F32X3_EXACT, PLAN_NO_F32H2_GEMM, PLAN_NO_UPADD, PLAN_H2_PLANES, PLAN_NO_BNECK, PLAN_NO_BATCHED_REDUCE = 1, 2, 4, 8, 16, 32, 64, 128, 256, 512, 1024, 2048, 4096, 8192
 PLAN_BF16_F32_STREAM = 32768
+PLAN_H2_PER_TILE_GRID = 65536
 ABI_VERSION = 9
 
 EXPORTS = [
@@ -25,6 +26,7 @@
     "capf_jpeg_info", "capf_jpeg_coefficients", "capf_jpeg_decode",
     "capf_jpeg_batch_info", "capf_jpeg_decode_batch", "capf_jpeg_coefficients_subseq",
     "capf_op_f32h2_gemm_pack_elems", "capf_op_pack_f32h2_gemm", "capf_op_conv_f32h2g", "capf_op_conv_f32h2g_group", "capf_op_linear_f32h2g", "capf_op_linear_ln_f32h2g", "capf_op_wgrad", "capf_op_conv_f32h2_tiles", "capf_op_conv_f32h2_planes", "capf_op_h2_planes",
+    "capf_op_conv_f32h2_walk_lists", "capf_op_conv_f32h2_walk_group", "capf_op_h2_walk",
     "capf_fliptest_fuse_swap", "capf_pck_counts",
 ]
 
@@ -160,6 +162,9 @@
     lib.capf_op_conv_bf16_group.argtypes = [P, c_int, D, POINTER(c_void_p), POINTER(c_int32)]
     lib.capf_op_conv_f32h2_planes.argtypes = [P, D, P, P]
     lib.capf_op_conv_f32h2_tiles.argtypes = [c_int, c_int, c_int, POINTER(c_int)]
+    lib.capf_op_conv_f32h2_walk_lists.argtypes = [c_int, D, P, c_int64, POINTER(c_int32)]
+    lib.capf_op_conv_f32h2_walk_lists.restype = c_int64
+    lib.capf_op_conv_f32h2_walk_group.argtypes = [P, c_int, D, P, c_int64]
     lib.capf_pose_errors.argtypes = [P, P, P, c_int, c_int, P, P]
     lib.capf_segment_sums.argtypes = [P, P, P, P, c_int, c_int, P, P]
     lib.capf_keypoints_loss.argtypes = [P, c_int, P, P, P, c_int, c_int, c_float, P, P]
@@ -369,6 +374,10 @@
             return self._ws[off:off + (n + 1) // 2].view(torch.bfloat16)[:n].view(*shape)
         return self._ws[off:off + n].view(*shape)
 
+    def op_h2_walk(self, index, batch):
+        self.lib.capf_op_h2_walk.argtypes = [c_void_p, c_int, c_int]
+        return self.lib.capf_op_h2_walk(self.h, index, batch)
+
     def op_h2_planes(self, index, batch):
         import torch
         ptr, tp = c_void_p(), c_int(0)
@@ -592,6 +601,31 @@
 def conv_nhwc_f32h2_group(problems):
     descs, outs = _conv_descs([(x, wp, bias, res, co, 3, 1, act) for x, wp, bias, act, res, co in problems])
     _call("capf_op_conv_f32h2_group", _stream(problems[0][0]), len(problems), descs)
+    return outs
+
+
+def f32h2_walk_lists(descs, n):
+    import numpy as np
+    lib = load_library()
+    blocks = c_int32(0)
+    words = lib.capf_op_conv_f32h2_walk_lists(n, descs, None, 0, byref(blocks))
+    if words < 0:
+        raise CapfError(f"capf_op_conv_f32h2_walk_lists failed ({words})")
+    if words == 0:
+        return None, 0
+    img = np.zeros(words, dtype=np.int32)
+    lib.capf_op_conv_f32h2_walk_lists(n, descs, img.ctypes.data, words, byref(blocks))
+    return img, blocks.value
+
+
+def conv_nhwc_f32h2_walk_group(problems):
+    import torch
+    descs, outs = _conv_descs([(x, wp, bias, res, co, 3, 1, act) for x, wp, bias, act, res, co in problems])
+    img, _ = f32h2_walk_lists(descs, len(problems))
+    if img is None:
+        raise CapfError("no conv of the launch runs on 32-channel tiles: no walking form")
+    lists = torch.from_numpy(img).to(problems[0][0].device)
+    _call("capf_op_conv_f32h2_walk_group", _stream(problems[0][0]), len(problems), descs, _p(lists), img.size)
     return outs
 
 
diff --git a/contextaware-poseformer_amd/csrc/engine.cpp b/contextaware-poseformer_amd/csrc/engine.cpp
--- a/contextaware-poseformer_amd/csrc/engine.cpp
+++ b/contextaware-poseformer_amd/csrc/engine.cpp
@@ -126,6 +126,15 @@
     if (pk.ws || pk.x3) a.Wp3 = pack_arena + (pk.ws ? pk.ws_off : pk.x3_off);
     a.x3_h2 = pk.x3 && plan.x3_h2;
     if (a.x3_h2 && op.h2_utab >= 0 && utab_on_device) a.h2_utab = reinterpret_cast<const unsigned*>(pack_arena + utab_off) + op.h2_utab;
+    if (a.x3_h2 && pack_arena) {
+        const long oi = &op - ops.data();
+        const WalkRef* r = oi >= 0 && oi < (long)ops.size() ? walk_ref((int)oi, batch) : nullptr;
+        if (r && r->at >= 0) {
+            a.h2_walk = reinterpret_cast<const int*>(pack_arena + walk_off) + r->at;
+            a.h2_walk_words = r->words;
+            a.h2_walk_sig = r->sig;
+        }
+    }
     if (pk.h2g && batch >= H2G_MIN_BATCH && !op.bf16 && !op.pw_pair && !(op.wino && wino_now(op, batch))) a.Wh2 = pack_arena + pk.h2g_off;
     if (op.wino && !wino_now(op, batch)) {
         a.Wp = pack_arena + pk.direct_off;
@@ -460,8 +469,29 @@
     return CAPF_OK;
 }
 
+int Engine::ensure_walk(int batch) {
+    if (!plan.h2_walk || !pack_arena || walk_ref(0, batch)) return CAPF_OK;
+    const int n = walk_n.load(std::memory_order_relaxed);
+    if (n == WALK_BATCHES) return CAPF_OK;
+    std::vector<int> img;
+    WalkBatch& wb = walk_batches[n];
+    walk_plan(batch, img, wb.refs);
+    if (walk_used + img.size() > WALK_WORDS) {
+        for (WalkRef& r : wb.refs) r = WalkRef{};
+        img.clear();
+    }
+    if (!img.empty()) HIP_TRY(hipMemcpy(pack_arena + walk_off + walk_used, img.data(), img.size() * sizeof(int), hipMemcpyHostToDevice));
+    for (WalkRef& r : wb.refs)
+        if (r.at >= 0) r.at += (long)walk_used;
+    walk_used += img.size();
+    wb.batch = batch;
+    walk_n.store(n + 1, std::memory_order_release);
+    return CAPF_OK;
+}
+
 int Engine::run(hipStream_t s, int batch, int first_op, int last_op, hipEvent_t* ev, LaunchLog* log) {
     hipStream_t main_stream = s;
+    if (const int rc = ensure_walk(batch)) return rc;
     if (plan.use_h2g && (batch >= H2G_MIN_BATCH || has_res_chain) && last_op > n_backbone_ops && !bf16()) {
         const int rc = ensure_h2g_lifter(s);
         if (rc) return rc;
@@ -560,7 +590,7 @@
         delete h;
         return CAPF_ERR_UNSUPPORTED;
     }
-    if (cfg->plan_flags & ~(16383 | CAPF_PLAN_BF16_F32_STREAM)) {
+    if (cfg->plan_flags & ~(16383 | CAPF_PLAN_BF16_F32_STREAM | CAPF_PLAN_H2_PER_TILE_GRID)) {
         g_create_error = "unknown capf_plan_flag bits";
         delete h;
         return CAPF_ERR_INVALID;
@@ -1054,6 +1084,37 @@
 }
 
 int capf_op_conv_f32h2_tiles(int B, int H, int W, int* tile_pixels) { return capf::f32h2_tiles_m(B, H, W, tile_pixels); }
+
+static unsigned walk_lists_of(int n, const capf_conv_desc* d, std::vector<int>* img, int* blocks) {
+    int geo[capf::MAXG][5];
+    for (int i = 0; i < n; ++i) {
+        const int g[5] = {d[i].B, d[i].H, d[i].W, d[i].Cin, d[i].Cout};
+        for (int k = 0; k < 5; ++k) geo[i][k] = g[k];
+    }
+    return capf::f32h2_walk_lists(geo, n, img, blocks, nullptr);
+}
+
+int64_t capf_op_conv_f32h2_walk_lists(int n, const capf_conv_desc* d, int32_t* out, int64_t capacity, int32_t* blocks) {
+    if (n <= 0 || n > capf::MAXG || !d) return CAPF_ERR_INVALID;
+    std::vector<int> img;
+    int wgs = 0;
+    if (!walk_lists_of(n, d, &img, &wgs)) return 0;
+    if (blocks) *blocks = wgs;
+    if (out && capacity >= (int64_t)img.size()) memcpy(out, img.data(), img.size() * sizeof(int));
+    return (int64_t)img.size();
+}
+
+int capf_op_conv_f32h2_walk_group(void* stream, int n, const capf_conv_desc* d, const int32_t* lists_dev, int64_t words) {
+    if (!lists_dev || words <= 0 || words > 0x7FFFFFFF) return CAPF_ERR_INVALID;
+    if (n <= 0 || n > capf::MAXG || !d) return CAPF_ERR_INVALID;
+    const unsigned sig = walk_lists_of(n, d, nullptr, nullptr);
+    if (!sig) return CAPF_ERR_UNSUPPORTED;
+    return conv_group(stream, n, d, [&](const capf_conv_desc& c, int, capf::GemmArgs& a) {
+        const int rc = wp3_build(c, a, capf::gemm_f32x3_ok, 1);
+        a.h2_walk = lists_dev; a.h2_walk_words = (int)words; a.h2_walk_sig = sig;
+        return rc;
+    }, capf::launch_gemm_f32h2_group);
+}
 
 int capf_op_conv_f32h2_planes(void* stream, const capf_conv_desc* d, const int32_t* exps_in, int32_t* exps_out) {
     if (!d || !is_3x3_s1(*d) || (exps_in && exps_out)) return CAPF_ERR_UNSUPPORTED;
@@ -1391,6 +1452,14 @@
     return op.h2_role;
 }
 
+int capf_op_h2_walk(const capf_handle* h, int index, int batch) {
+    if (!h || index < 0 || index >= (int)h->e.ops.size() || batch <= 0) return CAPF_ERR_INVALID;
+    std::vector<int> img;
+    std::vector<Engine::WalkRef> refs;
+    h->e.walk_plan(batch, img, refs);
+    return refs[index].at >= 0 ? refs[index].words : 0;
+}
+
 int capf_forward_profile(capf_handle* h, void* stream, const float* images_nhwc, const float* k2d, float* kcrop_inout,
                          int batch, float* out, float* op_ms, int n_ops) {
     if (!h || !images_nhwc || !k2d || !kcrop_inout || !out || !op_ms) return CAPF_ERR_INVALID;
diff --git a/contextaware-poseformer_amd/csrc/engine.h b/contextaware-poseformer_amd/csrc/engine.h
--- a/contextaware-poseformer_amd/csrc/engine.h
+++ b/contextaware-poseformer_amd/csrc/engine.h
@@ -1,4 +1,5 @@
 #pragma once
+#include <atomic>
 #include <hip/hip_runtime.h>
 #include <stdint.h>
 
@@ -203,6 +204,7 @@
         bool x3_h2 = true;
         bool use_h2g = true;
         bool use_h2_planes = false;
+        bool h2_walk = true;
         bool use_pwchain = true;
         bool use_bneck = true;
         bool use_upadd = true;
@@ -228,6 +230,12 @@
     bool has_res_chain = false;
     std::vector<unsigned> utab_host;
     size_t utab_off = 0;
+    struct WalkRef { long at = -1; int words = 0; unsigned sig = 0; };
+    struct WalkBatch { int batch = 0; std::vector<WalkRef> refs; };
+    static constexpr int WALK_BATCHES = 16;
+    static constexpr size_t WALK_WORDS = 1u << 17;
+    size_t walk_off = 0;
+    void walk_plan(int batch, std::vector<int>& img, std::vector<WalkRef>& refs) const;
     int batch_limit = 0;
     int feat_buf[4] = {-1, -1, -1, -1}, feat_H[4] = {0, 0, 0, 0}, feat_W[4] = {0, 0, 0, 0}, feat_C[4] = {0, 0, 0, 0};
     LifterSchema lifter;
@@ -259,6 +267,16 @@
     std::vector<CopySegment> bias_tab;
     bool bias_tab_on_device = false;
     bool utab_on_device = false;
+    WalkBatch walk_batches[WALK_BATCHES];
+    std::atomic<int> walk_n{0};
+    size_t walk_used = 0;
+    int ensure_walk(int batch);
+    const WalkRef* walk_ref(int op_index, int batch) const {
+        const int n = walk_n.load(std::memory_order_acquire);
+        for (int i = 0; i < n; ++i)
+            if (walk_batches[i].batch == batch) return &walk_batches[i].refs[op_index];
+        return nullptr;
+    }
     float* split_ws = nullptr;
     int* split_cnt = nullptr;
     float* split_ws_side = nullptr;
diff --git a/contextaware-poseformer_amd/csrc/igemm_f32h2_ws.hip b/contextaware-poseformer_amd/csrc/igemm_f32h2_ws.hip
--- a/contextaware-poseformer_amd/csrc/igemm_f32h2_ws.hip
+++ b/contextaware-poseformer_amd/csrc/igemm_f32h2_ws.hip
@@ -1,3 +1,5 @@
+#include <vector>
+
 #include "igemm_f32h2_ws_tile.h"
 #include "kernels.h"
 
@@ -5,11 +7,14 @@
 
 long f32h2_pack_elems(int Cout, int Cin) { return h2_pack_elems(Cout, Cin); }
 
+static bool h2_wide(const H2Problem& q, int N) {
+    static const long wide_min = [] { const char* e = diag_env("CAPF_H2_WIDE_MIN_TILES"); return e ? atol(e) : 512L; }();
+    return N % 64 == 0 && (long)q.g.tiles_m * (N / 64) >= wide_min;
+}
 static bool h2_from_args(const GemmArgs& a, H2Problem* q) {
     if (a.out_bf16 || !ws_args_ok(a, 3, 4.0, WS_MAX_P)) return false;
     if (!h2_plan(a.M / (a.H * a.W), a.H, a.W, a.Cin, a.N, 32, q)) return false;
-    static const long wide_min = [] { const char* e = diag_env("CAPF_H2_WIDE_MIN_TILES"); return e ? atol(e) : 512L; }();
-    if (a.N % 64 == 0 && (long)q->g.tiles_m * (a.N / 64) >= wide_min) { q->g.NS = 64; q->g.NSL = a.N / 64; }
+    if (h2_wide(*q, a.N)) { q->g.NS = 64; q->g.NSL = a.N / 64; }
     q->x = a.A;
     q->g.wp = reinterpret_cast<const unsigned short*>(a.Wp3);
     q->winv = reinterpret_cast<const float*>(q->g.wp + h2_piece_elems(a.N, a.Cin));
@@ -47,8 +52,11 @@
     H2Problem g[MAXG];
     GroupLayout lay;
     int n;
+    int walk_words;
+    int walk_pad;
+    const int* walk;
 };
-static_assert(sizeof(H2GroupArgs) == MAXG * sizeof(H2Problem) + (2 * MAXG + 2) * sizeof(int), "kernel argument layout");
+static_assert(sizeof(H2GroupArgs) == MAXG * sizeof(H2Problem) + (2 * MAXG + 4) * sizeof(int) + sizeof(const int*), "kernel argument layout");
 
 template <int TN, bool PIN = false, bool POUT = false>
 __global__ __launch_bounds__(256, TN == 1 ? 3 : 2) void igemm_f32h2_group_ws_kernel(H2GroupArgs ga) {
@@ -60,8 +68,54 @@
 #endif
 }
 
+#if defined(__HIP_DEVICE_COMPILE__)
+struct H2WalkNext {
+    static constexpr bool walk = true;
+    const H2GroupArgs& ga;
+    int pos, end;
+    __device__ __forceinline__ bool operator()(int& pi, int& bid) {
+        while (pos < end) {
+            const unsigned e = (unsigned)__builtin_amdgcn_readfirstlane(ga.walk[pos++]);
+            const int i = (int)(e >> 28), b = (int)(e & 0x0FFFFFFFu);
+            if (i < ga.n && b < ga.lay.tiles[i]) { pi = i; bid = b; return true; }
+        }
+        return false;
+    }
+    __device__ __forceinline__ const H2Problem& problem(int pi) const { return ga.g[pi]; }
+};
+#endif
+__global__ __launch_bounds__(256, 3) void igemm_f32h2_group_walk_kernel(H2GroupArgs ga) {
+#if defined(__HIP_DEVICE_COMPILE__)
+    extern __shared__ __attribute__((aligned(16))) unsigned char h2_lds[];
+    const int b = blockIdx.x;
+    int pos = __builtin_amdgcn_readfirstlane(ga.walk[b]), end = __builtin_amdgcn_readfirstlane(ga.walk[b + 1]);
+    pos = max(pos, (int)gridDim.x + 1);
+    end = min(end, ga.walk_words);
+    H2WalkNext next{ga, pos, end};
+    int pi, bid;
+    if (!next(pi, bid)) return;
+    igemm_f32h2_ws_tiles<1, false, false, H2WalkNext>(pi, bid, h2_lds, next);
+#endif
+}
+
+unsigned f32h2_walk_lists(const int (*geo)[5], int n, std::vector<int>* out, int* wgs, int* total_tiles) {
+    int tiles[MAXG], ncc[MAXG], order[MAXG], st[MAXG], sn[MAXG], m = 0, total = 0;
+    double cost[MAXG];
+    for (int i = 0; i < n && m < MAXG; ++i) {
+        H2Problem q;
+        if (!h2_plan(geo[i][0], geo[i][1], geo[i][2], geo[i][3], geo[i][4], 32, &q) || h2_wide(q, geo[i][4])) continue;
+        tiles[m] = q.g.tiles_m * q.g.NSL; ncc[m] = geo[i][3] / 16; cost[m] = geo[i][3];
+        ++m;
+    }
+    if (m == 0) return 0;
+    group_order(m, cost, order);
+    for (int i = 0; i < m; ++i) { st[i] = tiles[order[i]]; sn[i] = ncc[order[i]]; total += st[i]; }
+    if (total_tiles) *total_tiles = total;
+    return h2_walk_build(st, sn, m, H2_WALK_SLOTS, out, wgs);
+}
+
 template <int TN, bool PIN = false, bool POUT = false>
-static hipError_t h2_launch(const H2Problem* list, int n, hipStream_t s) {
+static hipError_t h2_launch(const H2Problem* list, int n, hipStream_t s, const GemmArgs* walk = nullptr) {
     int tiles[MAXG], order[MAXG];
     double cost[MAXG];
     for (int i = 0; i < n; ++i) { tiles[i] = list[i].g.tiles_m * list[i].g.NSL; cost[i] = list[i].g.C; }
@@ -69,6 +123,21 @@
     ga.n = n;
     const int start = group_layout(ga.lay, n, tiles, cost, order);
     for (int i = 0; i < n; ++i) ga.g[i] = list[order[i]];
+    if constexpr (TN == 1 && !PIN && !POUT) {
+        if (walk && walk->h2_walk) {
+            int st[MAXG], sn[MAXG], wgs = 0;
+            for (int i = 0; i < n; ++i) { st[i] = tiles[order[i]]; sn[i] = ga.g[i].g.C >> 4; }
+            if (h2_walk_build(st, sn, n, H2_WALK_SLOTS, nullptr, &wgs) == walk->h2_walk_sig && wgs > 0 && walk->h2_walk_words > wgs) {
+                ga.walk = walk->h2_walk;
+                ga.walk_words = walk->h2_walk_words;
+                static DynLdsAttr wattr;
+                const hipError_t we = wattr.ensure(reinterpret_cast<const void*>(&igemm_f32h2_group_walk_kernel), h2_lds_bytes(32));
+                if (we != hipSuccess) return we;
+                hipLaunchKernelGGL(igemm_f32h2_group_walk_kernel, dim3(wgs), dim3(256), h2_lds_bytes(32), s, ga);
+                return hipGetLastError();
+            }
+        }
+    }
     static DynLdsAttr attr;
     const hipError_t e = attr.ensure(reinterpret_cast<const void*>(&igemm_f32h2_group_ws_kernel<TN, PIN, POUT>), h2_lds_bytes(32 * TN));
     if (e != hipSuccess) return e;
@@ -81,6 +150,9 @@
     if (n > MAXG) return hipErrorInvalidValue;
     H2Problem cls[2][3][MAXG];
     int cnt[2][3] = {{0, 0, 0}, {0, 0, 0}};
+    const GemmArgs* walk = &list[0];
+    for (int i = 1; i < n; ++i)
+        if (list[i].h2_walk != list[0].h2_walk || list[i].h2_walk_sig != list[0].h2_walk_sig) walk = nullptr;
     for (int i = 0; i < n; ++i) {
         H2Problem q;
         if (!list[i].Wp3 || !list[i].x3_h2 || !h2_from_args(list[i], &q)) return hipErrorInvalidValue;
@@ -92,7 +164,7 @@
     if (cnt[1][0] && e == hipSuccess) e = h2_launch<2>(cls[1][0], cnt[1][0], s);
     if (cnt[1][1] && e == hipSuccess) e = h2_launch<2, true, false>(cls[1][1], cnt[1][1], s);
     if (cnt[1][2] && e == hipSuccess) e = h2_launch<2, false, true>(cls[1][2], cnt[1][2], s);
-    if (cnt[0][0] && e == hipSuccess) e = h2_launch<1>(cls[0][0], cnt[0][0], s);
+    if (cnt[0][0] && e == hipSuccess) e = h2_launch<1>(cls[0][0], cnt[0][0], s, walk);
     if (cnt[0][1] && e == hipSuccess) e = h2_launch<1, true, false>(cls[0][1], cnt[0][1], s);
     if (cnt[0][2] && e == hipSuccess) e = h2_launch<1, false, true>(cls[0][2], cnt[0][2], s);
     return e;
diff --git a/contextaware-poseformer_amd/csrc/igemm_f32h2_ws_tile.h b/contextaware-poseformer_amd/csrc/igemm_f32h2_ws_tile.h
--- a/contextaware-poseformer_amd/csrc/igemm_f32h2_ws_tile.h
+++ b/contextaware-poseformer_amd/csrc/igemm_f32h2_ws_tile.h
@@ -3,6 +3,9 @@
 #define H2_EXPERIMENT 0
 #endif
 #include <algorithm>
+#include <queue>
+#include <utility>
+#include <vector>
 
 #include "igemm_bf16_ws_tile.h"
 
@@ -66,7 +69,63 @@
     return sb < 64 ? 64 : (sb > 190 ? 190 : sb);
 }
 
+static constexpr int H2_WALK_SLOTS = 768;
+inline unsigned h2_walk_build(const int* tiles, const int* ncc, int n, int slots, std::vector<int>* out, int* wgs) {
+    unsigned sig = 2166136261u;
+    auto mix = [&](unsigned v) { sig = (sig ^ v) * 16777619u; };
+    mix((unsigned)n); mix((unsigned)slots);
+    for (int i = 0; i < n; ++i) { mix((unsigned)tiles[i]); mix((unsigned)ncc[i]); }
+    if (sig == 0) sig = 1;
+    const int per = slots / 8;
+    if (n <= 0 || n > 8 || per <= 0) return 0;
+    for (int i = 0; i < n; ++i)
+        if (tiles[i] <= 0 || tiles[i] >= (1 << 28)) return 0;
+    auto share = [&](int i, int x, int* first) {
+        const int per_xcd = ((tiles[i] + 7) & ~7) >> 3;
+        *first = x * per_xcd;
+        return std::max(0, std::min(tiles[i], (x + 1) * per_xcd) - x * per_xcd);
+    };
+    int L = 0;
+    for (int x = 0; x < 8; ++x) {
+        int t = 0, f;
+        for (int i = 0; i < n; ++i) t += share(i, x, &f);
+        L = std::max(L, std::min(per, t));
+    }
+    if (wgs) *wgs = 8 * L;
+    if (!out) return sig;
+    std::vector<std::vector<int>> lists((size_t)8 * L);
+    for (int x = 0; x < 8; ++x) {
+        typedef std::pair<long, int> Slot;
+        std::priority_queue<Slot, std::vector<Slot>, std::greater<Slot>> heap;
+        for (int l = 0; l < L; ++l) heap.push(Slot(0, l));
+        for (int i = 0; i < n; ++i) {
+            int first;
+            const int cnt = share(i, x, &first);
+            for (int b = first; b < first + cnt; ++b) {
+                Slot s = heap.top();
+                heap.pop();
+                lists[(size_t)8 * s.second + x].push_back((int)(((unsigned)i << 28) | (unsigned)b));
+                s.first += 2 * ncc[i] + 5;
+                heap.push(s);
+            }
+        }
+    }
+    out->clear();
+    int at = 8 * L + 1;
+    for (const std::vector<int>& l : lists) { out->push_back(at); at += (int)l.size(); }
+    out->push_back(at);
+    for (const std::vector<int>& l : lists) out->insert(out->end(), l.begin(), l.end());
+    return sig;
+}
+
 #if defined(__HIP_DEVICE_COMPILE__)
+
+struct H2OneTile {
+    static constexpr bool walk = false;
+    const H2Problem& q;
+    __device__ __forceinline__ bool operator()(int&, int&) { return false; }
+    __device__ __forceinline__ const H2Problem& problem(int) const { return q; }
+};
 
 typedef _Float16 ws_f16x8 __attribute__((ext_vector_type(8)));
 typedef unsigned ws_u32x2 __attribute__((ext_vector_type(2)));
@@ -98,8 +157,10 @@
                max(__builtin_amdgcn_readlane(x, 32), __builtin_amdgcn_readlane(x, 48)));
 }
 
-template <int TN, bool PIN = false, bool POUT = false>
-__device__ __forceinline__ void igemm_f32h2_ws_tile(const H2Problem& q, const int bid, unsigned char* __restrict__ lds) {
+template <int TN, bool PIN, bool POUT, class Next>
+__device__ __forceinline__ void igemm_f32h2_ws_tiles(const int pi_first, const int bid_first, unsigned char* __restrict__ lds, Next next) {
+    constexpr bool WALK = Next::walk;
+    static_assert(!WALK || (!PIN && !POUT), "the walking form takes plain fp32 tensors");
     constexpr int NS = 32 * TN;
     constexpr int WP_BYTES = 9 * 32 * 32;
     constexpr int WS_BYTES = 2 * WP_BYTES;
@@ -108,18 +169,19 @@
     constexpr int NWS = (NWI + 3) / 4;
     constexpr int NAU = H2_NAU;
     constexpr unsigned OOB = 0x80000000u;
-    const WsProblem& p = q.g;
     const int tid = threadIdx.x, lane = tid & 63;
     const int wave = __builtin_amdgcn_readfirstlane(tid >> 6);
-    const int frow = lane & 31, fhalf = lane >> 5;
-    const int NCC = p.C >> 4;
-    const int tm = bid / p.NSL, slice = bid - tm * p.NSL;
-
+    int pi = pi_first;
+    int bid = bid_first;
+    ws_rsrc_t rs_x;
+    constexpr int HP = H2_HP;
+    unsigned a_voff[NAU];
+    [[maybe_unused]] unsigned a_cls = 0;
+    auto stage_geometry = [&](const H2Problem& q, const int bid) __attribute__((always_inline)) {
+    const WsProblem& p = q.g;
+    const int tm = bid / p.NSL;
     const int b_first = ws_div(tm * p.G, p.d_rgpi);
-    const ws_rsrc_t rs_x = __builtin_amdgcn_make_buffer_rsrc((void*)(q.x + (size_t)b_first * p.H * p.W * p.C), 0, 0x7FFFFF00u, 0x00020000);
-    constexpr int HP = H2_HP;
-    unsigned a_voff[NAU], a_lds[NAU];
-    [[maybe_unused]] unsigned a_cls = 0;
+    rs_x = __builtin_amdgcn_make_buffer_rsrc((void*)(q.x + (size_t)b_first * p.H * p.W * p.C), 0, 0x7FFFFF00u, 0x00020000);
     const int n_units = 4 * p.PP;
     const bool tab_ok = !(H2_EXPERIMENT & 128) && !PIN && q.utab != nullptr && (p.G == 1 || (p.RGPI == 1 && (tm + 1) * p.G <= p.RG));
     if (tab_ok) {
@@ -129,9 +191,6 @@
 #pragma unroll
         for (int j = 0; j < NAU; ++j) {
             const unsigned t = q.utab[j * 256 + tid];
-            const int qi = min(j * 256 + tid, n_units - 1);
-            const int px = qi >> 2, qt = qi & 3;
-            a_lds[j] = (unsigned)((qt >> 1) * HP + px * 16 + (qt & 1) * 8);
             a_voff[j] = ((t & 1u) && !(t & kill)) ? (unsigned)((int)(t & ~15u) + base) : OOB;
         }
     } else {
@@ -140,8 +199,6 @@
         for (int j = 0; j < NAU; ++j) {
             const int qi = min(j * 256 + tid, n_units - 1);
             const int px = qi >> 2, qt = qi & 3;
-            a_lds[j] = PIN ? (unsigned)((2 * (qt >> 1) + (qt & 1)) * HP + px * 16)
-                           : (unsigned)((qt >> 1) * HP + px * 16 + (qt & 1) * 8);
 #if (H2_EXPERIMENT & 64)
             a_voff[j] = (unsigned)(qi * 16 + q0);
             continue;
@@ -156,12 +213,53 @@
             a_voff[j] = ok ? (unsigned)(((((b - b_first) * p.H + h) * p.W + col) * p.C + qt * 4) * 4) : OOB;
         }
     }
+    };
     ws_f32x4 ar[NAU];
     auto load_a = [&](int cc) {
 #pragma unroll
         for (int j = 0; j < NAU; ++j)
             ar[j] = __builtin_bit_cast(ws_f32x4, __builtin_amdgcn_raw_buffer_load_b128(rs_x, a_voff[j], (unsigned)cc * 64u, 0));
     };
+    ws_rsrc_t rs_w;
+    int ncc_w = 0;
+    const unsigned w_voff = (unsigned)lane * 16u;
+    auto set_w = [&](const H2Problem& q, const int bid) __attribute__((always_inline)) {
+        const WsProblem& p = q.g;
+        const int slice = bid - (bid / p.NSL) * p.NSL;
+        const int nsl32 = (p.N + 31) >> 5;
+        ncc_w = p.C >> 4;
+        rs_w = __builtin_amdgcn_make_buffer_rsrc((void*)(p.wp + (size_t)slice * TN * ncc_w * (WS_BYTES / 2)), 0,
+                                                 (unsigned)(nsl32 - slice * TN) * (unsigned)ncc_w * (unsigned)WS_BYTES, 0x00020000);
+    };
+    auto fire_w = [&](int cc) {
+#pragma unroll
+        for (int i = 0; i < NWS; ++i) {
+            const int k = min(i * 4 + wave, NWI - 1);
+            const int j = k / 18, rem = k - j * 18;
+            __builtin_amdgcn_raw_ptr_buffer_load_lds(rs_w, (ws_lptr_t)(lds + H2_A_BYTES + k * 1024), 16, w_voff,
+                                                     (unsigned)(j * ncc_w + cc) * (unsigned)WS_BYTES + (unsigned)rem * 1024u, 0, 0);
+        }
+    };
+    stage_geometry(next.problem(pi), bid);
+    set_w(next.problem(pi), bid);
+    bool ahead = false;
+    for (;;) {
+    int tid_tile = threadIdx.x;
+    if constexpr (WALK) asm volatile("" : "+v"(tid_tile));
+    const int tid = tid_tile, lane = tid & 63;
+    const int frow = lane & 31, fhalf = lane >> 5;
+    const H2Problem& q = next.problem(pi);
+    const WsProblem& p = q.g;
+    const int NCC = p.C >> 4;
+    const int tm = bid / p.NSL, slice = bid - tm * p.NSL;
+    unsigned a_lds[NAU];
+#pragma unroll
+    for (int j = 0; j < NAU; ++j) {
+        const int qi = min(j * 256 + tid, 4 * p.PP - 1);
+        const int px = qi >> 2, qt = qi & 3;
+        a_lds[j] = PIN ? (unsigned)((2 * (qt >> 1) + (qt & 1)) * HP + px * 16)
+                       : (unsigned)((qt >> 1) * HP + px * 16 + (qt & 1) * 8);
+    }
     int* const aux = reinterpret_cast<int*>(lds + H2_A_BYTES + W2_BYTES);
     float* const aux_w = reinterpret_cast<float*>(aux + 4);
     float* const aux_b = aux_w + 64;
@@ -264,20 +362,7 @@
             *reinterpret_cast<ws_u32x2*>(lds + 2 * HP + a_lds[j]) = u2;
         }
     };
-    const unsigned w_voff = (unsigned)lane * 16u;
-    const int nsl32 = (p.N + 31) >> 5;
-    const ws_rsrc_t rs_w = __builtin_amdgcn_make_buffer_rsrc((void*)(p.wp + (size_t)slice * TN * NCC * (WS_BYTES / 2)), 0,
-                                                             (unsigned)(nsl32 - slice * TN) * (unsigned)NCC * (unsigned)WS_BYTES, 0x00020000);
-    auto fire_w = [&](int cc) {
-#pragma unroll
-        for (int i = 0; i < NWS; ++i) {
-            const int k = min(i * 4 + wave, NWI - 1);
-            const int j = k / 18, rem = k - j * 18;
-            __builtin_amdgcn_raw_ptr_buffer_load_lds(rs_w, (ws_lptr_t)(lds + H2_A_BYTES + k * 1024), 16, w_voff,
-                                                     (unsigned)(j * NCC + cc) * (unsigned)WS_BYTES + (unsigned)rem * 1024u, 0, 0);
-        }
-    };
-    load_a(0);
+    if (!ahead) load_a(0);
     load_e(0);
     if (POUT && tid < 4) aux_o[tid] = 0;
     if (tid < NS) {
@@ -323,7 +408,7 @@
             __builtin_amdgcn_s_barrier();
         }
     }
-    fire_w(0);
+    if (!ahead) fire_w(0);
     unsigned a_addr[2][3];
 #pragma unroll
     for (int i = 0; i < 2; ++i) {
@@ -448,6 +533,18 @@
         }
     }
 
+    int pi_next = 0, bid_next = 0;
+    bool more = false;
+    if constexpr (WALK) {
+        more = next(pi_next, bid_next);
+    }
+    auto advance = [&]() {
+        pi = pi_next;
+        bid = bid_next;
+        ahead = true;
+        asm volatile("s_waitcnt lgkmcnt(0)" ::: "memory");
+        __builtin_amdgcn_s_barrier();
+    };
     if (H2_EXPERIMENT & 32) {
         float t = 0.f;
 #pragma unroll
@@ -457,7 +554,15 @@
 #pragma unroll
                 for (int e = 0; e < 16; ++e) t += acc[i][j][e];
         if (t == 1234.5678f) q.y[tid] = t;
-        return;
+        if (!more) return;
+        asm volatile("s_waitcnt lgkmcnt(0)" ::: "memory");
+        __builtin_amdgcn_s_barrier();
+        set_w(next.problem(pi_next), bid_next);
+        fire_w(0);
+        stage_geometry(next.problem(pi_next), bid_next);
+        load_a(0);
+        advance();
+        continue;
     }
     const float inv_s = __int_as_float((254 - sb) << 23);
     if constexpr (POUT) {
@@ -482,6 +587,10 @@
     }
     asm volatile("s_waitcnt lgkmcnt(0)" ::: "memory");
     __builtin_amdgcn_s_barrier();
+    if (WALK && more) {
+        set_w(next.problem(pi_next), bid_next);
+        fire_w(0);
+    }
     constexpr int EPS = 36;
     float* ep = reinterpret_cast<float*>(lds) + wave * (32 * EPS);
     [[maybe_unused]] const int hi_chunk = (lane >> 1) & 1;
@@ -542,8 +651,20 @@
                     __builtin_amdgcn_raw_buffer_store_b128(p1, rs_out, ok ? off + 32u : OOB, 0, 0);
                 }
             }
-        }
-    }
+            if (WALK && more && j == TN - 1 && i == 0) {
+                stage_geometry(next.problem(pi_next), bid_next);
+                load_a(0);
+            }
+        }
+    }
+    if (!more) return;
+    advance();
+    }
+}
+
+template <int TN, bool PIN = false, bool POUT = false>
+__device__ __forceinline__ void igemm_f32h2_ws_tile(const H2Problem& q, const int bid, unsigned char* __restrict__ lds) {
+    igemm_f32h2_ws_tiles<TN, PIN, POUT, H2OneTile>(0, bid, lds, H2OneTile{q});
 }
 
 #endif
diff --git a/contextaware-poseformer_amd/csrc/kernels.h b/contextaware-poseformer_amd/csrc/kernels.h
--- a/contextaware-poseformer_amd/csrc/kernels.h
+++ b/contextaware-poseformer_amd/csrc/kernels.h
@@ -3,6 +3,8 @@
 #include <stdint.h>
 
 #include <stdlib.h>
+
+#include <vector>
 
 namespace capf {
 
@@ -111,6 +113,9 @@
     const int* h2_ein;
     int* h2_eout;
     const unsigned* h2_utab;
+    const int* h2_walk;
+    int h2_walk_words;
+    unsigned h2_walk_sig;
     int f32s;
     int out_f32;
     void* out_sh;
@@ -270,8 +275,10 @@
 hipError_t launch_gemm_f32h2_group(const GemmArgs* list, int n, hipStream_t s);
 bool gemm_f32h2_ok(const GemmArgs& a);
 static constexpr int F32H2_UNIT_TABLE_WORDS = 7 * 256;
+static constexpr int F32H2_WALK_MIN_TILES = 768;
 bool f32h2_unit_table(int H, int W, int Cin, unsigned* out);
 bool f32h2_shape_ok(int B, int H, int W, int Cin, int Cout);
+unsigned f32h2_walk_lists(const int (*geo)[5], int n, std::vector<int>* out, int* wgs, int* total_tiles);
 const char* gemm_f32h2_kernel_name(const GemmArgs& a);
 hipError_t launch_pack_conv_f32h2(const float* w, const float* gamma, const float* beta, const float* mean, const float* var, float eps,
                                   void* Wp_f16, float* bias, int Cout, int Cin, hipStream_t s);
diff --git a/contextaware-poseformer_amd/csrc/plan.cpp b/contextaware-poseformer_amd/csrc/plan.cpp
--- a/contextaware-poseformer_amd/csrc/plan.cpp
+++ b/contextaware-poseformer_amd/csrc/plan.cpp
@@ -973,6 +973,7 @@
     if (cfg.plan_flags & CAPF_PLAN_NO_BNECK) p.use_bneck = false;
     if (cfg.plan_flags & CAPF_PLAN_NO_BATCHED_REDUCE) p.batch_reduce = false;
     if (cfg.plan_flags & CAPF_PLAN_H2_PLANES) p.use_h2_planes = true;
+    if (cfg.plan_flags & CAPF_PLAN_H2_PER_TILE_GRID) p.h2_walk = false;
     if (cfg.plan_flags & CAPF_PLAN_NO_WS) p.use_ws = false;
     if (cfg.plan_flags & CAPF_PLAN_NO_F32X3) p.use_x3 = false;
     if (cfg.plan_flags & CAPF_PLAN_F32X3_EXACT) p.x3_h2 = false;
@@ -1154,8 +1155,46 @@
     off += round64(t_h2_specs.size() * (sizeof(H2TrainW) / sizeof(float)) + 16);
     utab_off = off;
     off += round64(utab_host.size() + 16);
+    walk_off = off;
+    if (plan.x3_h2 && plan.use_x3 && plan.h2_walk && !plan.use_h2_planes) off += round64(WALK_WORDS);
     pack_elems = off;
     return true;
 }
 
-}
+void Engine::walk_plan(int batch, std::vector<int>& img_all, std::vector<WalkRef>& refs) const {
+    img_all.clear();
+    refs.assign(ops.size(), WalkRef{});
+    if (!(plan.x3_h2 && plan.use_x3 && plan.h2_walk && !plan.use_h2_planes)) return;
+    std::map<std::vector<int>, WalkRef> seen;
+    for (const auto& levels : region_levels)
+        for (const std::vector<int>& level : levels) {
+            int geo[MAXG][5], members[MAXG], n = 0;
+            std::vector<int> key;
+            for (int oi : level) {
+                const Op& op = ops[oi];
+                if (op.kind != OP_GEMM || !op.wino || !packs[op.pack].x3 || batch < op.x3_lo || batch > op.x3_hi) continue;
+                if (n == MAXG) { n = 0; break; }
+                const int g[5] = {batch, op.H, op.W, op.Cin, op.N};
+                for (int k = 0; k < 5; ++k) geo[n][k] = g[k];
+                key.insert(key.end(), g, g + 5);
+                members[n++] = oi;
+            }
+            if (n < 2) continue;
+            auto it = seen.find(key);
+            if (it == seen.end()) {
+                std::vector<int> img;
+                int wgs = 0, total = 0;
+                WalkRef r;
+                r.sig = f32h2_walk_lists(geo, n, &img, &wgs, &total);
+                if (r.sig && total > F32H2_WALK_MIN_TILES) {
+                    r.at = (long)img_all.size();
+                    r.words = (int)img.size();
+                    img_all.insert(img_all.end(), img.begin(), img.end());
+                }
+                it = seen.emplace(key, r).first;
+            }
+            for (int k = 0; k < n; ++k) refs[members[k]] = it->second;
+        }
+}
+
+}
diff --git a/include/capf.h b/include/capf.h
--- a/include/capf.h
+++ b/include/capf.h
@@ -66,6 +66,7 @@
     CAPF_PLAN_NO_BNECK = 4096,
     CAPF_PLAN_NO_BATCHED_REDUCE = 8192,
     CAPF_PLAN_BF16_F32_STREAM = 32768,
+    CAPF_PLAN_H2_PER_TILE_GRID = 65536,
     CAPF_PLAN_F32X3_EXACT = 256
 };
 
@@ -178,6 +179,8 @@
 
 int capf_op_conv_f32h2_tiles(int B, int H, int W, int* tile_pixels);
 int capf_op_conv_f32h2_planes(void* stream, const capf_conv_desc* conv, const int32_t* exps_in, int32_t* exps_out);
+int64_t capf_op_conv_f32h2_walk_lists(int n, const capf_conv_desc* convs, int32_t* out, int64_t capacity, int32_t* blocks);
+int capf_op_conv_f32h2_walk_group(void* stream, int n, const capf_conv_desc* convs, const int32_t* lists_dev, int64_t words);
 
 int64_t capf_op_f32h2_gemm_pack_elems(int N, int K);
 int capf_op_pack_f32h2_gemm(void* stream, const float* w, const float* gamma, const float* beta, const float* mean, const float* var,
@@ -255,6 +258,7 @@
 int capf_op_describe_sized(const capf_handle* h, int index, void* desc, size_t desc_bytes);
 int capf_op_tensor(const capf_handle* h, int index, int slot, const void** dev_ptr);
 int capf_op_h2_planes(const capf_handle* h, int index, int batch, const void** exps, int32_t* tile_pixels);
+int capf_op_h2_walk(const capf_handle* h, int index, int batch);
 
 int capf_forward_profile(capf_handle* h, void* stream, const float* images_nhwc, const float* k2d,
                          float* kcrop_inout, int batch, float* out, float* op_ms, int n_ops);
```

After: 9741 frames/s. -1.2%, worse.
